# joesound212985/Deepfake-Detection-using-CLIP-Based-SigLIP-2-Vision-Transformers

Measured on AMD Instinct MI355X. Metric: images/sec (train fwd+bwd) SigLIP-2-so400m@384 bf16, higher is better.
Workload: dtype bf16; 1 GPU; so400m-patch14-384 encoder+pool-head train fwd+bwd, 384x384, per-GPU batch 128, seeded random weights; global_batch=128, parallelism=dp1

## Files before the change

### deepfake-detection-using-clip-based-siglip-2-vision-transformers_amd/csrc/encoder.hip

```cpp
#include <hip/hip_runtime.h>
#include <string.h>

#include <algorithm>
#include <new>
#include <vector>

#include "kernels.h"
#include "siglip_hip.h"

using namespace sgl;

namespace {

inline size_t align256(size_t x) { return (x + 255) & ~(size_t)255; }
inline char* at(void* base, size_t off) { return reinterpret_cast<char*>(base) + off; }
inline const char* at(const void* base, size_t off) { return reinterpret_cast<const char*>(base) + off; }
inline bool mfma16(int dt) { return dt == DT_BF16 || dt == DT_F16; }
inline int round_up(int x, int m) { return (x + m - 1) / m * m; }

struct Bump {
  size_t off = 0;
  size_t take(size_t bytes) {
    const size_t o = off;
    off += align256(bytes);
// ... 148 lines not shown

#define CK(expr)                        \
  do {                                  \
    hipError_t e_ = (expr);             \
    if (e_ != hipSuccess) {             \
      ctx->last_hip = (int)e_;          \
      return SGL_ERR_HIP;               \
    }                                   \
  } while (0)

#define RET(expr)                 \
  do {                            \
    int r_ = (expr);              \
    if (r_ != SGL_OK) return r_;  \
  } while (0)

EpiParams epi_store(void* out, int ldo) {
  EpiParams p;
  p.out = out;
  p.ldo = ldo;
  return p;
}
EpiParams epi_f32(float* out, int ldo, const float* bias = nullptr) {
  EpiParams p;
  p.out = out;
  p.ldo = ldo;
  p.bias = bias;
  return p;
}
EpiParams epi_f32_acc(float* out, int ldo, int accumulate) {
  EpiParams p;
  p.out = out;
  p.ldo = ldo;
  p.accumulate = accumulate;
  return p;
}
EpiParams epi_res_f32(float* out, const float* bias, const float* res, int ld) {
  EpiParams p;
  p.out = out;
  p.ldo = ld;
  p.bias = bias;
  p.res = res;
  p.ldr = ld;
  return p;
}
EpiParams epi_pos_f32(float* out, int ldo, const float* bias, const float* pos, int pos_rows) {
  EpiParams p;
  p.out = out;
  p.ldo = ldo;
  p.bias = bias;
  p.pos = pos;
  p.pos_rows = pos_rows;
  return p;
}
EpiParams epi_bias_gelu(void* u, void* a, int ld, const float* bias, int grad_form) {
  EpiParams p;
  p.out = u;
  p.gelu_grad_form = grad_form;
  p.ldo = ld;
  p.out2 = a;
  p.ldo2 = ld;
  p.bias = bias;
  return p;
}
EpiParams epi_bias_gelu_mx(void* out, int ldo, const float* bias) {
  EpiParams p;
  p.out = out;
  p.ldo = ldo;
  p.bias = bias;
  return p;
}
EpiParams epi_gelu_bwd(void* out, const void* aux, int ld, int grad_form, float* colsum = nullptr) {
  EpiParams p;
  p.out = out;
  p.ldo = ld;
  p.aux = aux;
  p.ldaux = ld;
  p.gelu_grad_form = grad_form;
  if (colsum) {
    p.colsum = colsum;
    p.colsum_ld = ld;
  }
  return p;
}

int tn_splits(int N1, int N2, int rows) {
  const int tiles = ((N1 + 127) / 128) * ((N2 + 127) / 128);
  return std::min({(512 + tiles - 1) / tiles, std::max(rows / 512, 1), 16});
}

struct Call {
  sgl_ctx* ctx = nullptr;
  Layout lay;
  hipStream_t s = nullptr;
  const void* shadow = nullptr;
  char* act = nullptr;
  void* ws = nullptr;
  void* sp_a = nullptr;
  void* sp_b = nullptr;

  char* wsp(size_t off) const { return at(ws, off); }
  float* wsf(size_t off) const { return reinterpret_cast<float*>(at(ws, off)); }
  float* actf(size_t off) const { return reinterpret_cast<float*>(act + off); }
  const char* sh(size_t off) const { return at(shadow, off); }
  const float* shf(size_t off) const { return reinterpret_cast<const float*>(at(shadow, off)); }
  size_t head_bytes() const { return ::head_bytes(ctx, lay.B, lay.N); }
  char* block(int l) const { return lay.rc ? wsp(lay.w_blk) : act + lay.layer_base(l); }

  EpiParams epi_qkv(void* out, const float* bias) const {
    EpiParams p;
    p.out = out;
    p.bias = bias;
    p.tokens = lay.N;
    p.heads = ctx->H;
    p.head_dim = ctx->dh;
    p.head_dim_pad = ctx->DP;
    p.batch = lay.B;
    return p;
  }

  hipError_t gemm_nt(const void* A, int lda, const void* B, int ldb, int M, int N, int K, int epi, int out_dt,
                     const EpiParams& p) const {
    if (ctx->dt == DT_BF16) return gemm_nt_bf16(A, lda, B, ldb, M, N, K, epi, out_dt, p, s);
    if (ctx->dt == DT_F16) return gemm_nt_f16(A, lda, B, ldb, M, N, K, epi, out_dt, p, s);
    if (ctx->split && M > 0 && N > 0) {
      const int Ks = round_up(K, 8);
      hipError_t e = split3_rows((const float*)A, M, K, lda, sp_a, Ks, 0, s);
      if (e != hipSuccess) return e;
      e = split3_rows((const float*)B, N, K, ldb, sp_b, Ks, 1, s);
      if (e != hipSuccess) return e;
      return gemm_nt_bf16(sp_a, 3 * Ks, sp_b, 3 * Ks, M, N, 3 * Ks, epi, out_dt, p, s);
    }
    return gemm_f32_generic((const float*)A, lda, 1, (const float*)B, ldb, 1, M, N, K, epi, out_dt, p, s);
  }

  hipError_t gemm_tn(const void* A, int lda, const void* B, int ldb, int Mred, int N1, int N2, float* out, int ldo,
                     int accumulate, bool split_slabs) const {
    const EpiParams p = epi_f32_acc(out, ldo, accumulate);
    float* slabs = split_slabs ? wsf(lay.w_splitws) : nullptr;
    const size_t slab_bytes = split_slabs ? kSplitWsBytes : 0;
    if (ctx->dt == DT_F16)
      return gemm_tn_f16(A, lda, B, ldb, Mred, N1, N2, tn_splits(N1, N2, Mred), p, s, slabs, slab_bytes);
    if (ctx->dt == DT_BF16)
      return gemm_tn_bf16(A, lda, B, ldb, Mred, N1, N2, tn_splits(N1, N2, Mred), p, s, slabs, slab_bytes);
    if (ctx->split && Mred > 0 && N1 > 0 && N2 > 0) {
      const int l1 = round_up(N1, 8), l2 = round_up(N2, 8);
      hipError_t e = split3_stack((const float*)A, Mred, N1, lda, sp_a, l1, 0, s);
      if (e != hipSuccess) return e;
      e = split3_stack((const float*)B, Mred, N2, ldb, sp_b, l2, 1, s);
      if (e != hipSuccess) return e;
      return gemm_tn_bf16(sp_a, l1, sp_b, l2, 3 * Mred, N1, N2, tn_splits(N1, N2, 3 * Mred), p, s, slabs, slab_bytes);
    }
    return gemm_f32_generic((const float*)A, 1, lda, (const float*)B, 1, ldb, N1, N2, Mred, EPI_F32, DT_F32, p, s);
  }

  int bias_grad(const void* in, int ld, int M, int N, int n_out, float* out, int accumulate) const {
    if (!out) return SGL_OK;
    CK(colsum(in, ctx->dt, ld, M, N, n_out, wsf(lay.w_cspart), out, accumulate, s));
    return SGL_OK;
  }

  int ln_backward(const void* dy, int dy_dt, const float* x, const float* stats, int rows, const float* gamma,
                  const float* dres, float* dx, void* dx_lp, float* dgamma, float* dbeta, int accumulate,
                  float* colsum_out = nullptr) const {
    const int D = ctx->D;
    const bool want = dgamma || dbeta || colsum_out;
    const int nblk = layernorm_bwd_blocks(rows);
    float* part = wsf(lay.w_lnpart);
    CK(layernorm_bwd(dy, dy_dt, D, x, stats, stats + rows, gamma, dres, dx, dx_lp, ctx->dt, want ? part : nullptr, nblk,
                     rows, D, s));
    CK(reduce_partials3(part, nblk, 3 * D, dgamma, dbeta, colsum_out, D, accumulate, accumulate, 0, s));
    return SGL_OK;
  }
};

int mx_block(const Call& c, const sgl_layer_weights& lw, const ShadowLayer& sl, char* lb, const float* x, float* xo) {
  sgl_ctx* ctx = c.ctx;
  const Layout& lay = c.lay;
  hipStream_t s = c.s;
  const int D = ctx->D, Ip = ctx->Ip, Dp = ctx->Dp, M = lay.M;
  const float eps = ctx->cfg.layer_norm_eps;
  const size_t Mz = (size_t)M;
  char* h1 = lb + lay.r_h1;
  char* q = lb + lay.r_qkv;
  char* aq = lb + lay.r_attq;
  float* xmid = reinterpret_cast<float*>(lb + lay.r_xmid);
  char* h2 = lb + lay.r_h2;
  char* ua = lb + lay.r_a;
  CK(layernorm_fwd_mx(x, lw.ln1_w, lw.ln1_b, h1, h1 + Mz * Dp, M, D, Dp, eps, s));
  CK(gemm_nt_mx(h1, h1 + Mz * Dp, c.sh(sl.wqkv), c.sh(sl.wqkv_s), M, 3 * D, Dp, EPI_QKV, c.epi_qkv(q, c.shf(sl.bqkv)),
                nullptr, s));
  CK(attn_fwd(q, q + c.head_bytes(), q + 2 * c.head_bytes(), DT_BF16, lb + lay.r_attn,
              reinterpret_cast<float*>(lb + lay.r_lse), lay.B, ctx->H, lay.N, ctx->dh, ctx->DP, 0, s));
  CK(quantize_mx(lb + lay.r_attn, DT_BF16, D, M, D, Dp, aq, aq + Mz * Dp, s));
  CK(gemm_nt_mx(aq, aq + Mz * Dp, c.sh(sl.wo), c.sh(sl.wo_s), M, D, Dp, EPI_RES_F32, epi_res_f32(xmid, lw.o_b, x, D),
                nullptr, s));
  CK(layernorm_fwd_mx(xmid, lw.ln2_w, lw.ln2_b, h2, h2 + Mz * Dp, M, D, Dp, eps, s));
  CK(gemm_nt_mx(h2, h2 + Mz * Dp, c.sh(sl.w1), c.sh(sl.w1_s), M, Ip, Dp, EPI_BIAS_GELU,
                epi_bias_gelu_mx(ua, Ip, c.shf(sl.b1)), ua + Mz * Ip, s));
  CK(gemm_nt_mx(ua, ua + Mz * Ip, c.sh(sl.w2), c.sh(sl.w2_s), M, D, Ip, EPI_RES_F32, epi_res_f32(xo, lw.fc2_b, xmid, D),
                nullptr, s));
  return SGL_OK;
}

int block_to_fc1(const Call& c, const sgl_layer_weights& lw, const ShadowLayer& sl, char* lb, const float* x, bool want_u) {
  sgl_ctx* ctx = c.ctx;
  const Layout& lay = c.lay;
  hipStream_t s = c.s;
  const int D = ctx->D, Ip = ctx->Ip, M = lay.M, dt = ctx->dt;
  const float eps = ctx->cfg.layer_norm_eps;
  float* st1 = reinterpret_cast<float*>(lb + lay.r_stats1);
  float* st2 = reinterpret_cast<float*>(lb + lay.r_stats2);
  char* q = lb + lay.r_qkv;
  float* xmid = reinterpret_cast<float*>(lb + lay.r_xmid);
  CK(layernorm_fwd(x, lw.ln1_w, lw.ln1_b, lb + lay.r_h1, dt, D, st1, st1 + M, M, D, eps, s));
  CK(c.gemm_nt(lb + lay.r_h1, D, c.sh(sl.wqkv), D, M, 3 * D, D, EPI_QKV, dt, c.epi_qkv(q, c.shf(sl.bqkv))));
  CK(attn_fwd(q, q + c.head_bytes(), q + 2 * c.head_bytes(), ctx->split ? DT_F32_MFMA : dt, lb + lay.r_attn,
              reinterpret_cast<float*>(lb + lay.r_lse), lay.B, ctx->H, lay.N, ctx->dh, ctx->DP, 0, s));
  CK(c.gemm_nt(lb + lay.r_attn, D, c.sh(sl.wo), D, M, D, D, EPI_RES_F32, DT_F32, epi_res_f32(xmid, lw.o_b, x, D)));
  CK(layernorm_fwd(xmid, lw.ln2_w, lw.ln2_b, lb + lay.r_h2, dt, D, st2, st2 + M, M, D, eps, s));
  CK(c.gemm_nt(lb + lay.r_h2, D, c.sh(sl.w1), D, M, Ip, D, EPI_BIAS_GELU, dt,
               epi_bias_gelu(want_u ? lb + lay.r_u : nullptr, lb + lay.r_a, Ip, c.shf(sl.b1), mfma16(dt))));
  return SGL_OK;
}

int embed_forward(const Call& c, const sgl_weights* w, const float* pixels, int channels_last, int H, int W, float* out) {
  sgl_ctx* ctx = c.ctx;
  const Layout& lay = c.lay;
  hipStream_t s = c.s;
  const int D = ctx->D, Kp = ctx->Kp, M = lay.M;
  char* cols = c.act + lay.a_im2col;
  if (channels_last == 2) {
    CK(hipMemcpyAsync(cols, pixels, (size_t)M * Kp * ctx->es, hipMemcpyDeviceToDevice, s));
  } else {
    CK(im2col(pixels, channels_last, cols, ctx->dt, lay.B, H, W, ctx->P, Kp, s));
  }
  const float* pos = w->pos;
  if (!(lay.gh == ctx->g0 && lay.gw == ctx->g0)) {
    float* pr = c.actf(lay.a_pos);
    CK(pos_resize(w->pos, ctx->g0, pr, lay.gh, lay.gw, D, s));
    pos = pr;
  }
  CK(c.gemm_nt(cols, Kp, c.sh(ctx->sh_wpatch), Kp, M, D, Kp, EPI_POS_F32, DT_F32,
               epi_pos_f32(out, D, w->patch_b, pos, lay.N)));
  return SGL_OK;
}

int head_forward(const Call& c, const sgl_weights* w, const float* last_hidden, float* pooled) {
  sgl_ctx* ctx = c.ctx;
  const Layout& lay = c.lay;
  hipStream_t s = c.s;
  const int D = ctx->D, Ip = ctx->Ip, M = lay.M, B = lay.B, dt = ctx->dt;
  char* act = c.act;
  char* kv = act + lay.a_kvh;
  float* qp = c.actf(lay.a_qp);
  float* h0 = c.actf(lay.a_h0);
  float* hst = c.actf(lay.a_hstats);
  CK(cast_f32(last_hidden, act + lay.a_lastlp, dt, (size_t)M * D, s));
  CK(c.gemm_nt(act + lay.a_lastlp, D, c.sh(ctx->sh_hwkv), D, M, 2 * D, D, EPI_QKV, dt, c.epi_qkv(kv, w->in_proj_b + D)));
  CK(gemm_f32_generic(w->probe, D, 1, w->in_proj_w, D, 1, 1, D, D, EPI_F32, DT_F32, epi_f32(qp, D, w->in_proj_b), s));
  CK(pool_attn_fwd(qp, kv, kv + c.head_bytes(), dt, act + lay.a_ao, c.actf(lay.a_probs), B, ctx->H, lay.N, ctx->dh,
                   ctx->DP, s));
  CK(c.gemm_nt(act + lay.a_ao, D, c.sh(ctx->sh_hwo), D, B, D, D, EPI_F32, DT_F32, epi_f32(h0, D, w->out_proj_b)));
  CK(layernorm_fwd(h0, w->head_ln_w, w->head_ln_b, act + lay.a_hl, dt, D, hst, hst + B, B, D, ctx->cfg.layer_norm_eps, s));
  CK(c.gemm_nt(act + lay.a_hl, D, c.sh(ctx->sh_hw1), D, B, Ip, D, EPI_BIAS_GELU, dt,
               epi_bias_gelu(act + lay.a_hu, act + lay.a_ha, Ip, c.shf(ctx->sh_hb1), 0)));
  CK(c.gemm_nt(act + lay.a_ha, Ip, c.sh(ctx->sh_hw2), Ip, B, D, Ip, EPI_RES_F32, DT_F32,
               epi_res_f32(pooled, w->head_fc2_b, h0, D)));
  return SGL_OK;
}

long rc_max_tokens(const sgl_ctx* c) {
  long w = c->Ip;
  if (3l * c->D > w) w = 3l * c->D;
  if ((long)c->Kp > w) w = c->Kp;
  const long row_bytes = c->split ? 3 * (long)round_up((int)w, 8) * 2 : w * (long)c->es;
  const long m = ((1l << 32) - 1) / row_bytes;
  return m < (1l << 22) - 1 ? m : (1l << 22) - 1;
}

bool shape_ok(const sgl_ctx* c, int B, int H, int W) {
  if (B <= 0 || H <= 0 || W <= 0) return false;
  if (H < c->P || W < c->P) return false;
  const long N = (long)(H / c->P) * (W / c->P);
  if ((long)B * N > (1l << 24)) return false;
  if (c->cfg.use_head && N > pool_attn_max_tokens(c->DP, 0)) return false;
  return true;
}

bool train_shape_ok(const sgl_ctx* c, int B, int H, int W) {
  if (!shape_ok(c, B, H, W)) return false;
  const long N = (long)(H / c->P) * (W / c->P);
  if (c->cfg.use_head && N > pool_attn_max_tokens(c->DP, 1)) return false;
  return !c->recompute || (long)B * N <= rc_max_tokens(c);
}

enum Pass { FORWARD, BACKWARD };
int begin_call(Call& c, Pass pass, sgl_ctx* ctx, const void* shadow, int B, int H, int W, const void* saved,
               size_t saved_bytes, void* ws, size_t ws_bytes, sgl_stream stream) {
  const bool train = pass == BACKWARD || saved != nullptr;
  if (!(train ? train_shape_ok(ctx, B, H, W) : shape_ok(ctx, B, H, W))) return SGL_ERR_BAD_SHAPE;
  if (train && ctx->mx) return SGL_ERR_UNSUPPORTED;
  c.lay = Layout(ctx, B, H, W, train);
  const Layout& lay = c.lay;
  if (pass == BACKWARD) {
    if (!saved || !ws) return SGL_ERR_NULL;
// ... 295 lines not shown
  float* slots[kMaxLayers + 1];
  for (int l = 0; l <= ctx->L; ++l) slots[l] = hidden_states + (size_t)(l % hs_slots) * hs_stride;
  return sgl_forward_slots(ctx, w, shadow, pixels, channels_last, B, H, W, interpolate_pos, slots, last_hidden,
                           pooled, saved, saved_bytes, ws, ws_bytes, first_trainable_block, stream);
}

int sgl_forward_slots(sgl_ctx* ctx, const sgl_weights* w, const void* shadow, const float* pixels, int channels_last,
                      int B, int H, int W, int interpolate_pos, float* const* hs_slots, float* last_hidden,
                      float* pooled, void* saved, size_t saved_bytes, void* ws, size_t ws_bytes,
                      int first_trainable_block, sgl_stream stream) {
  if (!ctx || !w || !shadow || !pixels || !hs_slots || !last_hidden || (ctx->L > 0 && !w->layers))
    return SGL_ERR_NULL;
  if (!shape_ok(ctx, B, H, W)) return SGL_ERR_BAD_SHAPE;
  for (int l = 0; l <= ctx->L; ++l)
    if (!hs_slots[l]) return SGL_ERR_NULL;
  const bool train = saved != nullptr;
  if (train && ctx->mx) return SGL_ERR_UNSUPPORTED;
  if (train)
    for (int l = 0; l < ctx->L; ++l)
      for (int k = l + 1; k <= ctx->L; ++k)
        if (hs_slots[l] == hs_slots[k]) return SGL_ERR_BAD_SHAPE;
  Call c;
  RET(begin_call(c, FORWARD, ctx, shadow, B, H, W, saved, saved_bytes, ws, ws_bytes, stream));
  const Layout& lay = c.lay;
  if (!(lay.gh == ctx->g0 && lay.gw == ctx->g0) && !interpolate_pos) return SGL_ERR_BAD_SHAPE;

  RET(embed_forward(c, w, pixels, channels_last, H, W, hs_slots[0]));
  for (int l = 0; l < ctx->L; ++l) {
    const sgl_layer_weights& lw = w->layers[l];
    const ShadowLayer& sl = ctx->sh_layers[l];
    char* lb = c.block(l);
    if (ctx->mx) {
      RET(mx_block(c, lw, sl, lb, hs_slots[l], hs_slots[l + 1]));
      continue;
    }
    RET(block_to_fc1(c, lw, sl, lb, hs_slots[l], train && !lay.rc && l >= first_trainable_block));
    CK(c.gemm_nt(lb + lay.r_a, ctx->Ip, c.sh(sl.w2), ctx->Ip, lay.M, ctx->D, ctx->Ip, EPI_RES_F32, DT_F32,
                 epi_res_f32(hs_slots[l + 1], lw.fc2_b, reinterpret_cast<const float*>(lb + lay.r_xmid), ctx->D)));
  }
  float* pst = c.actf(lay.a_pstats);
  CK(layernorm_fwd(hs_slots[ctx->L], w->post_ln_w, w->post_ln_b, last_hidden, DT_F32, ctx->D, pst, pst + lay.M, lay.M,
                   ctx->D, ctx->cfg.layer_norm_eps, c.s));
  if (ctx->cfg.use_head && pooled) RET(head_forward(c, w, last_hidden, pooled));
  return SGL_OK;
}

namespace {

int head_backward(const Call& c, const sgl_weights* w, const sgl_grads* g, const float* d_pooled,
                  const float* d_last_hidden, float* dlast) {
  sgl_ctx* ctx = c.ctx;
  const Layout& lay = c.lay;
  hipStream_t s = c.s;
  const int D = ctx->D, I = ctx->I, Ip = ctx->Ip, M = lay.M, B = lay.B, dt = ctx->dt;
  const int acc = g->accumulate;
  const char* act = c.act;
  const char* kv = act + lay.a_kvh;
  const float* qp = c.actf(lay.a_qp);
  void* hg = c.wsp(lay.w_hg);
  void* hdu = c.wsp(lay.w_hdu);
  void* hdh = c.wsp(lay.w_hdh);
  float* hdao = c.wsf(lay.w_hdao);
  CK(cast_f32(d_pooled, hg, dt, (size_t)B * D, s));
  CK(c.gemm_nt(hg, D, c.sh(ctx->sh_hw2_t), D, B, Ip, D, EPI_GELU_BWD, dt, epi_gelu_bwd(hdu, act + lay.a_hu, Ip, 0)));
  if (g->head_fc2_w) CK(c.gemm_tn(hg, D, act + lay.a_ha, Ip, B, D, I, g->head_fc2_w, I, acc, false));
  RET(c.bias_grad(hg, D, B, D, D, g->head_fc2_b, acc));
  CK(c.gemm_nt(hdu, Ip, c.sh(ctx->sh_hw1_t), Ip, B, D, Ip, EPI_STORE, dt, epi_store(hdh, D)));
  if (g->head_fc1_w) CK(c.gemm_tn(hdu, Ip, act + lay.a_hl, D, B, I, D, g->head_fc1_w, D, acc, false));
  RET(c.bias_grad(hdu, Ip, B, Ip, I, g->head_fc1_b, acc));
  RET(c.ln_backward(hdh, dt, c.actf(lay.a_h0), c.actf(lay.a_hstats), B, w->head_ln_w, d_pooled, c.wsf(lay.w_hdh0), hg,
                    g->head_ln_w, g->head_ln_b, acc));
  CK(c.gemm_nt(hg, D, c.sh(ctx->sh_hwo_t), D, B, D, D, EPI_F32, DT_F32, epi_f32(hdao, D)));
  if (g->out_proj_w) CK(c.gemm_tn(hg, D, act + lay.a_ao, D, B, D, D, g->out_proj_w, D, acc, false));
  RET(c.bias_grad(hg, D, B, D, D, g->out_proj_b, acc));
  void* dkv = c.wsp(lay.w_dqkv);
  float* dqpart = c.wsf(lay.w_hdqpart);
  float* dqp = c.wsf(lay.w_hdqp);
  CK(pool_attn_bwd(qp, kv, kv + c.head_bytes(), dt, c.actf(lay.a_probs), hdao, dkv, dqpart, B, ctx->H, lay.N, ctx->dh,
                   ctx->DP, s));
  if (g->probe || g->in_proj_w || g->in_proj_b) {
    CK(batch_sum(dqpart, B, (size_t)D, dqp, 0, s));
    if (g->in_proj_w)
      CK(gemm_f32_generic(dqp, 1, 1, w->probe, 1, 1, D, D, 1, EPI_F32, DT_F32, epi_f32_acc(g->in_proj_w, D, acc), s));
    if (g->in_proj_b) CK(batch_sum(dqp, 1, (size_t)D, g->in_proj_b, acc, s));
    if (g->probe)
      CK(gemm_f32_generic(dqp, D, 1, w->in_proj_w, 1, D, 1, D, D, EPI_F32, DT_F32, epi_f32_acc(g->probe, D, acc), s));
  }
  if (d_last_hidden) CK(copy_f32(d_last_hidden, dlast, (size_t)M * D, s));
  CK(c.gemm_nt(dkv, 2 * D, c.sh(ctx->sh_hwkv_t), 2 * D, M, D, 2 * D, EPI_F32, DT_F32,
               epi_f32_acc(dlast, D, d_last_hidden ? 1 : 0)));
  if (g->in_proj_w)
    CK(c.gemm_tn(dkv, 2 * D, act + lay.a_lastlp, D, M, 2 * D, D, g->in_proj_w + (size_t)D * D, D, acc, true));
  if (g->in_proj_b) RET(c.bias_grad(dkv, 2 * D, M, 2 * D, 2 * D, g->in_proj_b + D, acc));
  return SGL_OK;
}

int zero_dead_grads(const Call& c, const sgl_grads* g, bool no_head_grad, bool no_post_ln_grad) {
  sgl_ctx* ctx = c.ctx;
  hipStream_t s = c.s;
  if (g->accumulate) return SGL_OK;
  auto zero = [&](float* p, size_t n) { return p ? hipMemsetAsync(p, 0, n * 4, s) : hipSuccess; };
  const size_t Dz = (size_t)ctx->D, Iz = (size_t)ctx->I;
  if (ctx->cfg.use_head && no_head_grad) {
    CK(zero(g->probe, Dz));
    CK(zero(g->in_proj_w, 3 * Dz * Dz));
    CK(zero(g->in_proj_b, 3 * Dz));
    CK(zero(g->out_proj_w, Dz * Dz));
    CK(zero(g->out_proj_b, Dz));
    CK(zero(g->head_ln_w, Dz));
    CK(zero(g->head_ln_b, Dz));
    CK(zero(g->head_fc1_w, Iz * Dz));
    CK(zero(g->head_fc1_b, Iz));
    CK(zero(g->head_fc2_w, Dz * Iz));
    CK(zero(g->head_fc2_b, Dz));
  }
  if (no_post_ln_grad) {
    CK(zero(g->post_ln_w, Dz));
    CK(zero(g->post_ln_b, Dz));
  }
  return SGL_OK;
}

int mlp_backward(const Call& c, const sgl_layer_weights& lw, const sgl_layer_grads& lg, const ShadowLayer& sl,
                 const char* lb, int acc) {
  sgl_ctx* ctx = c.ctx;
  const Layout& lay = c.lay;
  hipStream_t s = c.s;
  const int D = ctx->D, I = ctx->I, Ip = ctx->Ip, M = lay.M, dt = ctx->dt;
  float* dx = c.wsf(lay.w_dx);
  void* gbuf = c.wsp(lay.w_g);
  void* du = c.wsp(lay.w_du);
  void* dhb = c.wsp(lay.w_dh);
  float* gsum = c.wsf(lay.w_gsum);
  float* csum = c.wsf(lay.w_csum);
  const bool fuse_cs = mfma16(dt) && lg.fc1_b;
  if (fuse_cs) CK(hipMemsetAsync(csum, 0, (size_t)((M + 127) / 128) * Ip * 4, s));
  CK(c.gemm_nt(gbuf, D, c.sh(sl.w2_t), D, M, Ip, D, EPI_GELU_BWD, dt,
               epi_gelu_bwd(du, lb + lay.r_u, Ip, mfma16(dt), fuse_cs ? csum : nullptr)));
  if (lg.fc2_w) CK(c.gemm_tn(gbuf, D, lb + lay.r_a, Ip, M, D, I, lg.fc2_w, I, acc, true));
  if (lg.fc2_b) CK(batch_sum(gsum, 1, (size_t)D, lg.fc2_b, acc, s));
  CK(c.gemm_nt(du, Ip, c.sh(sl.w1_t), Ip, M, D, Ip, EPI_STORE, dt, epi_store(dhb, D)));
  if (lg.fc1_w) CK(c.gemm_tn(du, Ip, lb + lay.r_h2, D, M, I, D, lg.fc1_w, D, acc, true));
  if (fuse_cs)
    CK(reduce_partials(csum, (M + 127) / 128, Ip, lg.fc1_b, I, acc, s));
  else
    RET(c.bias_grad(du, Ip, M, Ip, I, lg.fc1_b, acc));
  RET(c.ln_backward(dhb, dt, reinterpret_cast<const float*>(lb + lay.r_xmid),
                    reinterpret_cast<const float*>(lb + lay.r_stats2), M, lw.ln2_w, dx, dx, gbuf, lg.ln2_w, lg.ln2_b, acc,
                    (lg.o_b || lg.v_b) ? gsum : nullptr));
  if (lg.o_b) CK(batch_sum(gsum, 1, (size_t)D, lg.o_b, acc, s));
  return SGL_OK;
}

int attn_backward(const Call& c, const sgl_layer_weights& lw, const sgl_layer_grads& lg, const ShadowLayer& sl,
                  const char* lb, int acc) {
  sgl_ctx* ctx = c.ctx;
  const Layout& lay = c.lay;
  hipStream_t s = c.s;
  const int D = ctx->D, M = lay.M, dt = ctx->dt;
  void* gbuf = c.wsp(lay.w_g);
  void* dattn = c.wsp(lay.w_dh);
  void* dqkv = c.wsp(lay.w_dqkv);
  float* gsum = c.wsf(lay.w_gsum);
  const char* q = lb + lay.r_qkv;
  CK(c.gemm_nt(gbuf, D, c.sh(sl.wo_t), D, M, D, D, EPI_STORE, dt, epi_store(dattn, D)));
  if (lg.o_w) CK(c.gemm_tn(gbuf, D, lb + lay.r_attn, D, M, D, D, lg.o_w, D, acc, true));
  CK(attn_bwd(q, q + c.head_bytes(), q + 2 * c.head_bytes(), lb + lay.r_attn, dattn,
              reinterpret_cast<const float*>(lb + lay.r_lse), ctx->split ? DT_F32_MFMA : dt, dqkv, c.wsf(lay.w_delta),
              nullptr, lay.B, ctx->H, lay.N, ctx->dh, ctx->DP, 0, s));
  float* gw[3] = {lg.q_w, lg.k_w, lg.v_w};
  float* gb[3] = {lg.q_b, lg.k_b, lg.v_b};
  const bool w_adj = gw[0] && gw[1] == gw[0] + (size_t)D * D && gw[2] == gw[1] + (size_t)D * D;
  if (w_adj) CK(c.gemm_tn(dqkv, 3 * D, lb + lay.r_h1, D, M, 3 * D, D, gw[0], D, acc, true));
  for (int j = 0; j < 3; ++j) {
    const char* aj = reinterpret_cast<const char*>(dqkv) + (size_t)j * D * ctx->es;
    if (!w_adj && gw[j]) CK(c.gemm_tn(aj, 3 * D, lb + lay.r_h1, D, M, D, D, gw[j], D, acc, true));
  }
  if (gb[0]) RET(c.bias_grad(dqkv, 3 * D, M, D, D, gb[0], acc));
  if (gb[1] && !acc) CK(hipMemsetAsync(gb[1], 0, (size_t)D * 4, s));
  if (gb[2]) CK(vecmat_f32(gsum, lw.o_w, D, D, c.wsf(lay.w_cspart), gb[2], acc, s));
  return SGL_OK;
}

int ln1_backward(const Call& c, const sgl_layer_weights& lw, const sgl_layer_grads& lg, const ShadowLayer& sl,
                 const char* lb, const float* x_in, int acc) {
  sgl_ctx* ctx = c.ctx;
  const Layout& lay = c.lay;
  const int D = ctx->D, M = lay.M, dt = ctx->dt;
  float* dx = c.wsf(lay.w_dx);
  void* dh1 = c.wsp(lay.w_dh);
  CK(c.gemm_nt(c.wsp(lay.w_dqkv), 3 * D, c.sh(sl.wqkv_t), 3 * D, M, D, 3 * D, EPI_STORE, dt, epi_store(dh1, D)));
  RET(c.ln_backward(dh1, dt, x_in, reinterpret_cast<const float*>(lb + lay.r_stats1), M, lw.ln1_w, dx, dx,
                    c.wsp(lay.w_g), lg.ln1_w, lg.ln1_b, acc, c.wsf(lay.w_gsum)));
  return SGL_OK;
}

}

int sgl_backward_begin(sgl_ctx* ctx, const sgl_weights* w, const void* shadow, const sgl_grads* g, int B, int H, int W,
                       const float* hidden_states, const float* d_last_hidden, const float* d_pooled,
                       const float* d_tap_last, const void* saved, size_t saved_bytes, void* ws, size_t ws_bytes,
                       sgl_stream stream) {
  if (!ctx || !hidden_states) return SGL_ERR_NULL;
  if (!train_shape_ok(ctx, B, H, W)) return SGL_ERR_BAD_SHAPE;
  const size_t stride = (size_t)B * (H / ctx->P) * (W / ctx->P) * ctx->D;
  return sgl_backward_begin_p(ctx, w, shadow, g, B, H, W, hidden_states + (size_t)ctx->L * stride, d_last_hidden, d_pooled,
                              d_tap_last, saved, saved_bytes, ws, ws_bytes, stream);
}

int sgl_backward_begin_p(sgl_ctx* ctx, const sgl_weights* w, const void* shadow, const sgl_grads* g, int B, int H, int W,
                         const float* hs_last, const float* d_last_hidden, const float* d_pooled,
                         const float* d_tap_last, const void* saved, size_t saved_bytes, void* ws, size_t ws_bytes,
                         sgl_stream stream) {
  if (!ctx || !w || !shadow || !g || !hs_last) return SGL_ERR_NULL;
  Call c;
  RET(begin_call(c, BACKWARD, ctx, shadow, B, H, W, saved, saved_bytes, ws, ws_bytes, stream));
  const Layout& lay = c.lay;
  hipStream_t s = c.s;
  const int D = ctx->D, M = lay.M;
  float* dx = c.wsf(lay.w_dx);
  void* gbuf = c.wsp(lay.w_g);
  float* gsum = c.wsf(lay.w_gsum);
  const float* dlast = d_last_hidden;
  if (ctx->cfg.use_head && d_pooled) {
    float* dlast_buf = c.wsf(lay.w_dlast);
    RET(head_backward(c, w, g, d_pooled, d_last_hidden, dlast_buf));
    dlast = dlast_buf;
  }
  RET(zero_dead_grads(c, g, !d_pooled, !dlast));
  if (dlast) {
    RET(c.ln_backward(dlast, DT_F32, hs_last, c.actf(lay.a_pstats), M, w->post_ln_w, d_tap_last, dx, gbuf, g->post_ln_w,
                      g->post_ln_b, g->accumulate, gsum));
  } else if (d_tap_last) {
    CK(copy_f32(d_tap_last, dx, (size_t)M * D, s));
    CK(cast_f32(d_tap_last, gbuf, ctx->dt, (size_t)M * D, s));
    CK(colsum(gbuf, ctx->dt, D, M, D, D, c.wsf(lay.w_cspart), gsum, 0, s));
  } else {
    CK(hipMemsetAsync(dx, 0, (size_t)M * D * 4, s));
    CK(hipMemsetAsync(gbuf, 0, (size_t)M * D * ctx->es, s));
    CK(hipMemsetAsync(gsum, 0, (size_t)D * 4, s));
  }
  return SGL_OK;
}

int sgl_backward_layer(sgl_ctx* ctx, const sgl_weights* w, const void* shadow, const sgl_grads* g, int layer, int B,
                       int H, int W, const float* hidden_states, const float* d_tap, int need_dx, const void* saved,
                       size_t saved_bytes, void* ws, size_t ws_bytes, sgl_stream stream) {
  if (!ctx || !hidden_states) return SGL_ERR_NULL;
  if (layer < 0 || layer >= ctx->L || !train_shape_ok(ctx, B, H, W)) return SGL_ERR_BAD_SHAPE;
  const size_t stride = (size_t)B * (H / ctx->P) * (W / ctx->P) * ctx->D;
  return sgl_backward_layer_p(ctx, w, shadow, g, layer, B, H, W, hidden_states + (size_t)layer * stride, d_tap, need_dx,
                              saved, saved_bytes, ws, ws_bytes, stream);
}

int sgl_backward_layer_p(sgl_ctx* ctx, const sgl_weights* w, const void* shadow, const sgl_grads* g, int layer, int B,
                         int H, int W, const float* hs_in, const float* d_tap, int need_dx, const void* saved,
                         size_t saved_bytes, void* ws, size_t ws_bytes, sgl_stream stream) {
  if (!ctx || !w || !shadow || !g || !hs_in || !g->layers || !w->layers) return SGL_ERR_NULL;
  if (layer < 0 || layer >= ctx->L) return SGL_ERR_BAD_SHAPE;
  Call c;
  RET(begin_call(c, BACKWARD, ctx, shadow, B, H, W, saved, saved_bytes, ws, ws_bytes, stream));
  const int acc = g->accumulate;
  const sgl_layer_weights& lw = w->layers[layer];
  const sgl_layer_grads& lg = g->layers[layer];
  const ShadowLayer& sl = ctx->sh_layers[layer];
  char* lb = c.block(layer);
  if (c.lay.rc) RET(block_to_fc1(c, lw, sl, lb, hs_in, true));
  RET(mlp_backward(c, lw, lg, sl, lb, acc));
  RET(attn_backward(c, lw, lg, sl, lb, acc));
  float* dx = c.wsf(c.lay.w_dx);
  if (d_tap) CK(add_f32(dx, d_tap, dx, (size_t)c.lay.M * ctx->D, c.s));
  if (need_dx || lg.ln1_w || lg.ln1_b) RET(ln1_backward(c, lw, lg, sl, lb, hs_in, acc));
  return SGL_OK;
}

namespace {

int embed_param_backward(const Call& c, const sgl_grads* g) {
  sgl_ctx* ctx = c.ctx;
  const Layout& lay = c.lay;
  hipStream_t s = c.s;
  const int D = ctx->D, M = lay.M, N = lay.N;
  const int acc = g->accumulate;
  float* dx = c.wsf(lay.w_dx);
  void* gbuf = c.wsp(lay.w_g);
  if (g->patch_w)
    CK(c.gemm_tn(gbuf, D, c.act + lay.a_im2col, ctx->Kp, M, D, ctx->K0, g->patch_w, ctx->K0, acc, true));
  if (g->patch_b) CK(batch_sum(c.wsf(lay.w_gsum), 1, (size_t)D, g->patch_b, acc, s));
  if (g->pos) {
    if (lay.gh == ctx->g0 && lay.gw == ctx->g0) {
      CK(batch_sum(dx, lay.B, (size_t)N * D, g->pos, acc, s));
    } else {
      float* dpos = c.wsf(lay.w_dlast);
      CK(batch_sum(dx, lay.B, (size_t)N * D, dpos, 0, s));
      if (!acc) CK(hipMemsetAsync(g->pos, 0, (size_t)ctx->g0 * ctx->g0 * D * 4, s));
      CK(pos_resize_bwd(dpos, lay.gh, lay.gw, g->pos, ctx->g0, D, s));
    }
  }
  return SGL_OK;
}

struct PxLayout {
  size_t dcols = 0, wpt = 0, total = 0;
  PxLayout(const sgl_ctx* c, int M) {
    Bump b;
    dcols = b.take((size_t)M * c->Kp * 4);
    wpt = b.take((size_t)c->Kp * c->D * c->es);
    total = b.off;
  }
};

}

int sgl_backward_embed(sgl_ctx* ctx, const sgl_weights* w, const sgl_grads* g, int B, int H, int W, int interpolate_pos,
                       const void* saved, size_t saved_bytes, void* ws, size_t ws_bytes, sgl_stream stream) {
  if (!ctx || !w || !g) return SGL_ERR_NULL;
  Call c;
  RET(begin_call(c, BACKWARD, ctx, nullptr, B, H, W, saved, saved_bytes, ws, ws_bytes, stream));
  (void)interpolate_pos;
  return embed_param_backward(c, g);
}

int sgl_query_input_grad_bytes(const sgl_ctx* ctx, int B, int H, int W, size_t* scratch_bytes) {
  if (!ctx || !scratch_bytes) return SGL_ERR_NULL;
  if (!train_shape_ok(ctx, B, H, W)) return SGL_ERR_BAD_SHAPE;
  if (ctx->mx) return SGL_ERR_UNSUPPORTED;
  *scratch_bytes = PxLayout(ctx, B * (H / ctx->P) * (W / ctx->P)).total;
  return SGL_OK;
}

int sgl_backward_embed_px(sgl_ctx* ctx, const sgl_weights* w, const sgl_grads* g, int B, int H, int W,
                          int interpolate_pos, float* d_pixels, int channels_last, void* px_scratch,
                          size_t px_scratch_bytes, const void* saved, size_t saved_bytes, void* ws, size_t ws_bytes,
                          sgl_stream stream) {
  if (!ctx || !w || !g || !w->patch_w) return SGL_ERR_NULL;
  if (!d_pixels || !px_scratch) return SGL_ERR_NULL;
  if (channels_last != 0 && channels_last != 1) return SGL_ERR_UNSUPPORTED;
  Call c;
  RET(begin_call(c, BACKWARD, ctx, nullptr, B, H, W, saved, saved_bytes, ws, ws_bytes, stream));
  const Layout& lay = c.lay;
  const PxLayout px(ctx, lay.M);
  if (px_scratch_bytes < px.total) return SGL_ERR_WORKSPACE;
  (void)interpolate_pos;
  RET(embed_param_backward(c, g));
  const int D = ctx->D, Kp = ctx->Kp;
  float* dcols = reinterpret_cast<float*>(at(px_scratch, px.dcols));
  void* wpt = at(px_scratch, px.wpt);
  CastJob job;
  cast_job_add(job, w->patch_w, D, ctx->K0, ctx->K0, nullptr, D, Kp, Kp, wpt, D);
  CK(cast_job_run(job, ctx->dt, c.s));
  CK(c.gemm_nt(c.wsp(lay.w_g), D, wpt, D, lay.M, Kp, D, EPI_F32, DT_F32, epi_f32(dcols, Kp)));
  CK(col2im(dcols, lay.B, H, W, ctx->P, Kp, d_pixels, channels_last, c.s));
  return SGL_OK;
}

int sgl_backward(sgl_ctx* ctx, const sgl_weights* w, const void* shadow, const sgl_grads* g, int B, int H, int W,
                 int interpolate_pos, const float* hidden_states, const float* const* d_taps,
                 const float* d_last_hidden, const float* d_pooled, int first_trainable_block, int train_embeddings,
                 const void* saved, size_t saved_bytes, void* ws, size_t ws_bytes, sgl_stream stream) {
  if (!ctx) return SGL_ERR_NULL;
  const int L = ctx->L;
  int stop = train_embeddings ? 0 : first_trainable_block;
  if (stop < 0) stop = 0;
  if (stop < L && w && g && (!w->layers || !g->layers)) return SGL_ERR_NULL;
  RET(sgl_backward_begin(ctx, w, shadow, g, B, H, W, hidden_states, d_last_hidden, d_pooled,
                         d_taps ? d_taps[L] : nullptr, saved, saved_bytes, ws, ws_bytes, stream));
  for (int l = L - 1; l >= stop; --l) {
    const int need_dx = (l > stop) || train_embeddings;
    RET(sgl_backward_layer(ctx, w, shadow, g, l, B, H, W, hidden_states, d_taps ? d_taps[l] : nullptr, need_dx, saved,
                           saved_bytes, ws, ws_bytes, stream));
  }
  if (train_embeddings)
    RET(sgl_backward_embed(ctx, w, g, B, H, W, interpolate_pos, saved, saved_bytes, ws, ws_bytes, stream));
  return SGL_OK;
}

#define CKV(expr)                                   \
  do {                                              \
    hipError_t e_ = (expr);                         \
    if (e_ == hipErrorInvalidValue) return SGL_ERR_UNSUPPORTED; \
    if (e_ != hipSuccess) return SGL_ERR_HIP;       \
  } while (0)

int sgl_op_layernorm_fwd(const float* x, const float* gamma, const float* beta, void* y, int y_dtype, float* mean,
                         float* rstd, int M, int D, float eps, sgl_stream stream) {
  CKV(layernorm_fwd(x, gamma, beta, y, y_dtype, D, mean, rstd, M, D, eps, (hipStream_t)stream));
  return SGL_OK;
}

int sgl_op_quantize_mxfp8(const void* x, int x_dtype, int ldx, int M, int K, int Kp, void* q, void* scales,
                          sgl_stream stream) {
  if (!x || !q || !scales) return SGL_ERR_NULL;
  CKV(quantize_mx(x, x_dtype, ldx, M, K, Kp, q, scales, (hipStream_t)stream));
  return SGL_OK;
}

int sgl_op_layernorm_fwd_mx(const float* x, const float* gamma, const float* beta, void* q, void* scales, int M, int D,
                            int Kp, float eps, sgl_stream stream) {
  if (!x || !gamma || !beta || !q || !scales) return SGL_ERR_NULL;
  CKV(layernorm_fwd_mx(x, gamma, beta, q, scales, M, D, Kp, eps, (hipStream_t)stream));
  return SGL_OK;
}

int sgl_op_gemm_nt_mx(const void* A, const void* As, const void* B, const void* Bs, int M, int N, int Kp, int epi,
                      void* out, int ldo, void* out_scales, const float* bias, const float* res, int ldr, int tokens,
                      int heads, int head_dim, int head_dim_pad, int batch, sgl_stream stream) {
  if (!A || !As || !B || !Bs || !out || !bias) return SGL_ERR_NULL;
  EpiParams p;
  p.out = out; p.ldo = ldo; p.bias = bias; p.res = res; p.ldr = ldr;
  p.tokens = tokens > 0 ? tokens : 1; p.heads = heads > 0 ? heads : 1; p.head_dim = head_dim > 0 ? head_dim : 8;
  p.head_dim_pad = head_dim_pad > 0 ? head_dim_pad : 8; p.batch = batch > 0 ? batch : 1;
  CKV(gemm_nt_mx(A, As, B, Bs, M, N, Kp, epi, p, out_scales, (hipStream_t)stream));
  return SGL_OK;
}

int sgl_op_layernorm_bwd(const void* dy, int dy_dtype, const float* x, const float* mean, const float* rstd,
                         const float* gamma, const float* dres, float* dx, void* dx_lp, int lp_dtype, float* dgamma,
                         float* dbeta, float* scratch, size_t scratch_bytes, int M, int D, sgl_stream stream) {
  const int nblk = layernorm_bwd_blocks(M);
  if (scratch_bytes < (size_t)nblk * 3 * D * 4) return SGL_ERR_WORKSPACE;
  hipStream_t s = (hipStream_t)stream;
  CKV(layernorm_bwd(dy, dy_dtype, D, x, mean, rstd, gamma, dres, dx, dx_lp, lp_dtype, scratch, nblk, M, D, s));
  if (dgamma) CKV(reduce_partials(scratch, nblk, 3 * D, dgamma, D, 0, s));
  if (dbeta) CKV(reduce_partials(scratch + D, nblk, 3 * D, dbeta, D, 0, s));
  return SGL_OK;
}

int sgl_op_gemm_nt(int dtype, const void* A, int lda, const void* B, int ldb, int M, int N, int K, int epi, void* out,
                   int ldo, void* out2, int ldo2, const float* bias, const float* res, int ldr, const void* aux,
                   int ldaux, const float* pos, int pos_rows, int tokens, int heads, int head_dim, int head_dim_pad,
                   int batch, sgl_stream stream) {
  EpiParams p;
  p.out = out; p.ldo = ldo; p.out2 = out2; p.ldo2 = ldo2; p.bias = bias; p.res = res; p.ldr = ldr;
  p.aux = aux; p.ldaux = ldaux; p.pos = pos; p.pos_rows = pos_rows > 0 ? pos_rows : 1;
  p.tokens = tokens > 0 ? tokens : 1; p.heads = heads > 0 ? heads : 1; p.head_dim = head_dim > 0 ? head_dim : 8;
  p.head_dim_pad = head_dim_pad > 0 ? head_dim_pad : 8; p.batch = batch > 0 ? batch : 1;
  const bool f32_out = (epi == EPI_RES_F32 || epi == EPI_POS_F32 || epi == EPI_F32);
  const int out_dt = f32_out ? DT_F32 : dtype;
  if (dtype == DT_BF16)
    CKV(gemm_nt_bf16(A, lda, B, ldb, M, N, K, epi, out_dt, p, (hipStream_t)stream));
  else if (dtype == DT_F16)
    CKV(gemm_nt_f16(A, lda, B, ldb, M, N, K, epi, out_dt, p, (hipStream_t)stream));
  else
    CKV(gemm_f32_generic((const float*)A, lda, 1, (const float*)B, ldb, 1, M, N, K, epi, out_dt, p,
                         (hipStream_t)stream));
  return SGL_OK;
}

int sgl_op_gemm_tn(int dtype, const void* A, int lda, const void* B, int ldb, int Mred, int N1, int N2, int splits,
                   float* out, int ldo, int accumulate, sgl_stream stream) {
  return sgl_op_gemm_tn_ws(dtype, A, lda, B, ldb, Mred, N1, N2, splits, out, ldo, accumulate, nullptr, 0, stream);
}

int sgl_op_gemm_tn_ws(int dtype, const void* A, int lda, const void* B, int ldb, int Mred, int N1, int N2, int splits,
                      float* out, int ldo, int accumulate, float* scratch, size_t scratch_bytes, sgl_stream stream) {
  EpiParams p;
  p.out = out; p.ldo = ldo; p.accumulate = accumulate;
  if (dtype == DT_BF16)
    CKV(gemm_tn_bf16(A, lda, B, ldb, Mred, N1, N2, splits, p, (hipStream_t)stream, scratch, scratch_bytes));
  else if (dtype == DT_F16)
    CKV(gemm_tn_f16(A, lda, B, ldb, Mred, N1, N2, splits, p, (hipStream_t)stream, scratch, scratch_bytes));
  else
    CKV(gemm_f32_generic((const float*)A, 1, lda, (const float*)B, 1, ldb, N1, N2, Mred, EPI_F32, DT_F32, p,
                         (hipStream_t)stream));
  return SGL_OK;
}

int sgl_op_attn_fwd(int dtype, const void* q, const void* k, const void* v, void* out, float* lse, int B, int H, int N,
                    int head_dim, int head_dim_pad, int ld_qkv, sgl_stream stream) {
  CKV(attn_fwd(q, k, v, dtype, out, lse, B, H, N, head_dim, head_dim_pad, ld_qkv, (hipStream_t)stream));
  return SGL_OK;
}

int sgl_op_attn_bwd(int dtype, const void* q, const void* k, const void* v, const void* out, const void* dout,
                    const float* lse, void* dqkv, float* delta_scratch, int B, int H, int N, int head_dim,
                    int head_dim_pad, int ld_qkv, sgl_stream stream) {
  CKV(attn_bwd(q, k, v, out, dout, lse, dtype, dqkv, delta_scratch, nullptr, B, H, N, head_dim, head_dim_pad, ld_qkv,
               (hipStream_t)stream));
  return SGL_OK;
}

int sgl_op_colsum(int dtype, const void* in, int ld, int M, int N, float* out, int accumulate, float* scratch,
                  size_t scratch_bytes, sgl_stream stream) {
  if (scratch_bytes < (size_t)colsum_chunks(M) * N * 4) return SGL_ERR_WORKSPACE;
  CKV(colsum(in, dtype, ld, M, N, N, scratch, out, accumulate, (hipStream_t)stream));
  return SGL_OK;
}

int sgl_op_im2col(const float* pixels, int channels_last, void* out, int out_dtype, int B, int H, int W, int P, int Kp,
                  sgl_stream stream) {
  CKV(im2col(pixels, channels_last, out, out_dtype, B, H, W, P, Kp, (hipStream_t)stream));
  return SGL_OK;
}

int sgl_op_col2im(const float* d_cols, int B, int H, int W, int P, int Kp, float* d_pixels, int channels_last,
                  sgl_stream stream) {
  if (!d_cols || !d_pixels) return SGL_ERR_NULL;
  CKV(col2im(d_cols, B, H, W, P, Kp, d_pixels, channels_last, (hipStream_t)stream));
  return SGL_OK;
}

int sgl_op_pos_resize(const float* table, int native_grid, float* out, int gh, int gw, int D, sgl_stream stream) {
  CKV(pos_resize(table, native_grid, out, gh, gw, D, (hipStream_t)stream));
  return SGL_OK;
}

static bool lo_dtype_ok(int dt) { return dt == DT_F32 || dt == DT_BF16 || dt == DT_F16; }
static bool aligned16(const void* p) { return (((uintptr_t)p) & 15) == 0; }

int sgl_op_pool_attn_fwd(int dtype, const float* q, const void* K, const void* V, void* out, float* probs, int B, int H,
                         int N, int head_dim, int head_dim_pad, sgl_stream stream) {
  if (!q || !K || !V || !out || !probs) return SGL_ERR_NULL;
  if (B <= 0 || H <= 0 || N <= 0 || head_dim <= 0 || head_dim % 8 || head_dim_pad % 8 || head_dim > head_dim_pad)
    return SGL_ERR_BAD_SHAPE;
  if (!lo_dtype_ok(dtype) || !aligned16(K) || !aligned16(V)) return SGL_ERR_UNSUPPORTED;
  CKV(pool_attn_fwd(q, K, V, dtype, out, probs, B, H, N, head_dim, head_dim_pad, (hipStream_t)stream));
  return SGL_OK;
}

int sgl_op_pool_attn_bwd(int dtype, const float* q, const void* K, const void* V, const float* probs, const float* dout,
                         void* dkv, float* dq_partial, int B, int H, int N, int head_dim, int head_dim_pad,
                         sgl_stream stream) {
  if (!q || !K || !V || !probs || !dout || !dkv || !dq_partial) return SGL_ERR_NULL;
  if (B <= 0 || H <= 0 || N <= 0 || head_dim <= 0 || head_dim % 8 || head_dim_pad % 8 || head_dim > head_dim_pad)
    return SGL_ERR_BAD_SHAPE;
  if (!lo_dtype_ok(dtype) || !aligned16(K) || !aligned16(V) || !aligned16(dkv)) return SGL_ERR_UNSUPPORTED;
  CKV(pool_attn_bwd(q, K, V, dtype, probs, dout, dkv, dq_partial, B, H, N, head_dim, head_dim_pad, (hipStream_t)stream));
  return SGL_OK;
}

int sgl_op_pos_resize_bwd(const float* dout, int gh, int gw, float* dtable, int native_grid, int D, sgl_stream stream) {
  if (!dout || !dtable) return SGL_ERR_NULL;
  if (gh <= 0 || gw <= 0 || native_grid <= 0 || D <= 0) return SGL_ERR_BAD_SHAPE;
  CKV(pos_resize_bwd(dout, gh, gw, dtable, native_grid, D, (hipStream_t)stream));
  return SGL_OK;
}

int sgl_op_cast_pad(const float* src, int R, int C, int lds, void* dst, int dst_dtype, int Rp, int Cp, int ldd,
                    sgl_stream stream) {
  if (!src || !dst) return SGL_ERR_NULL;
  if (R < 0 || C < 0 || Rp < R || Cp < C || lds < C || ldd < Cp) return SGL_ERR_BAD_SHAPE;
  if (!lo_dtype_ok(dst_dtype)) return SGL_ERR_UNSUPPORTED;
  CKV(cast_pad(src, R, C, lds, dst, dst_dtype, Rp, Cp, ldd, (hipStream_t)stream));
  return SGL_OK;
}

int sgl_op_cast_job(const sgl_cast_mat* mats, int nmat, const sgl_cast_vec* vecs, int nvec, int dst_dtype,
                    sgl_stream stream) {
  if ((nmat > 0 && !mats) || (nvec > 0 && !vecs)) return SGL_ERR_NULL;
  if (nmat < 0 || nmat > 6 || nvec < 0 || nvec > 4) return SGL_ERR_BAD_SHAPE;
  for (int k = 0; k < nmat; ++k)
    if (!mats[k].src || (!mats[k].dst && !mats[k].dst_t)) return SGL_ERR_NULL;
  for (int k = 0; k < nvec; ++k)
    if (!vecs[k].src || !vecs[k].dst) return SGL_ERR_NULL;
  for (int k = 0; k < nmat; ++k) {
    const sgl_cast_mat& m = mats[k];
    if (m.R <= 0 || m.C <= 0 || m.Rp < m.R || m.Cp < m.C || m.lds < m.C || (m.dst && m.ldd < m.Cp) ||
        (m.dst_t && m.ldt < m.Rp))
      return SGL_ERR_BAD_SHAPE;
  }
  for (int k = 0; k < nvec; ++k)
    if (vecs[k].n < 0 || vecs[k].np < vecs[k].n) return SGL_ERR_BAD_SHAPE;
  if (!lo_dtype_ok(dst_dtype)) return SGL_ERR_UNSUPPORTED;
  CastJob job;
  for (int k = 0; k < nmat; ++k) {
    const sgl_cast_mat& m = mats[k];
    cast_job_add(job, m.src, m.R, m.C, m.lds, m.dst, m.Rp, m.Cp, m.ldd, m.dst_t, m.ldt);
  }
  for (int k = 0; k < nvec; ++k) cast_job_add_vec(job, vecs[k].src, vecs[k].n, vecs[k].dst, vecs[k].np);
  CKV(cast_job_run(job, dst_dtype, (hipStream_t)stream));
  return SGL_OK;
}

int sgl_op_split3(const float* src, int R, int C, int ld, void* dst, int Cs, int b_side, int stacked, sgl_stream stream) {
  if (!src || !dst) return SGL_ERR_NULL;
  if (R <= 0 || C <= 0 || ld < C || Cs != round_up(C, 8)) return SGL_ERR_BAD_SHAPE;
  if (!aligned16(dst)) return SGL_ERR_UNSUPPORTED;
  if (stacked)
    CKV(split3_stack(src, R, C, ld, dst, Cs, b_side ? 1 : 0, (hipStream_t)stream));
  else
    CKV(split3_rows(src, R, C, ld, dst, Cs, b_side ? 1 : 0, (hipStream_t)stream));
  return SGL_OK;
}

int sgl_op_batch_sum(const float* in, int B, size_t n, float* out, int accumulate, sgl_stream stream) {
  if (!in || !out) return SGL_ERR_NULL;
  if (B <= 0 || n >= ((size_t)1 << 31) * 256) return SGL_ERR_BAD_SHAPE;
  CKV(batch_sum(in, B, n, out, accumulate, (hipStream_t)stream));
  return SGL_OK;
}

int sgl_op_vecmat(const float* v, const float* W, int rows, int cols, float* scratch, size_t scratch_bytes, float* out,
                  int accumulate, sgl_stream stream) {
  if (!v || !W || !scratch || !out) return SGL_ERR_NULL;
  if (rows <= 0 || cols <= 0) return SGL_ERR_BAD_SHAPE;
  if (scratch_bytes < (size_t)16 * cols * 4) return SGL_ERR_WORKSPACE;
  CKV(vecmat_f32(v, W, rows, cols, scratch, out, accumulate, (hipStream_t)stream));
  return SGL_OK;
}

int sgl_op_reduce_partials(const float* partial, int nblk, int stride, float* out, int n, int accumulate,
                           sgl_stream stream) {
  if (!partial || !out) return SGL_ERR_NULL;
  if (nblk <= 0 || n <= 0 || stride < n) return SGL_ERR_BAD_SHAPE;
  CKV(reduce_partials(partial, nblk, stride, out, n, accumulate, (hipStream_t)stream));
  return SGL_OK;
}

int sgl_op_reduce_partials3(const float* partial, int nblk, int stride, float* out0, float* out1, float* out2, int n,
                            int accumulate0, int accumulate1, int accumulate2, sgl_stream stream) {
  if (!partial) return SGL_ERR_NULL;
  if (nblk <= 0 || n <= 0 || stride < 3 * (long)n) return SGL_ERR_BAD_SHAPE;
  CKV(reduce_partials3(partial, nblk, stride, out0, out1, out2, n, accumulate0, accumulate1, accumulate2,
                       (hipStream_t)stream));
  return SGL_OK;
}

int sgl_op_reduce_splits(const float* ws, int splits, size_t stride, int N1, int N2, float* out, int ldo, int accumulate,
                         sgl_stream stream) {
  if (!ws || !out) return SGL_ERR_NULL;
// ... 21 lines not shown
```

### deepfake-detection-using-clip-based-siglip-2-vision-transformers_amd/csrc/gemm_bf16.hip

```cpp
#include <stdlib.h>

#include "common.hip.h"
#include "epilogue.hip.h"
#include "kernels.h"

namespace sgl {

constexpr int G_BM = 128, G_BN = 128, G_BK = 64;
constexpr int G_STAGE = (G_BM + G_BN) * G_BK * 2;
constexpr int G_CT_LD = 132;
constexpr int G_LDS = (2 * G_STAGE > G_BM * G_CT_LD * 4) ? 2 * G_STAGE : G_BM * G_CT_LD * 4;

__device__ __forceinline__ u32x4 ldg128(__amdgpu_buffer_rsrc_t r, uint32_t voff) {
  return __builtin_amdgcn_raw_buffer_load_b128(r, voff, 0, 0);
}

template <int EPI, typename TOut>
__device__ __forceinline__ void store_tile(char* smem, f32x4 (&acc)[4][4], int wr, int wc, int lane, int t, int m0,
                                           int n0, int M, int N, const EpiParams& p) {
  float* ct = reinterpret_cast<float*>(smem);
  __syncthreads();
  const int g = lane >> 4, c16 = lane & 15;
#pragma unroll
  for (int i = 0; i < 4; ++i)
// ... 193 lines not shown
    }
  };

  load_tile(0);
  store_stage(0);
  __syncthreads();
  for (int kt = 0; kt < nk; ++kt) {
    const int cur = kt & 1;
    if (kt + 1 < nk) load_tile(kt + 1);
    const char* base = smem + cur * G_STAGE;
#pragma unroll
    for (int s = 0; s < 2; ++s) {
      const char* ba = base + s * 32 * 256 + frow;
      const char* bb = ba + OPB;
      lo_x8<TIn> af[4], bfr[4];
#pragma unroll
      for (int i = 0; i < 4; ++i) {
        const lo_x4<TIn> alo = lds_read_tr16<TIn>(ba + fa_col[i]);
        const lo_x4<TIn> ahi = lds_read_tr16<TIn>(ba + 4 * 256 + fa_col[i]);
        const lo_x4<TIn> blo = lds_read_tr16<TIn>(bb + fb_col[i]);
        const lo_x4<TIn> bhi = lds_read_tr16<TIn>(bb + 4 * 256 + fb_col[i]);
        af[i] = __builtin_shufflevector(alo, ahi, 0, 1, 2, 3, 4, 5, 6, 7);
        bfr[i] = __builtin_shufflevector(blo, bhi, 0, 1, 2, 3, 4, 5, 6, 7);
      }
#pragma unroll
      for (int i = 0; i < 4; ++i)
#pragma unroll
        for (int j = 0; j < 4; ++j)
          acc[i][j] = mfma_16x16x32(af[i], bfr[j], acc[i][j]);
    }
    if (kt + 1 < nk) store_stage(cur ^ 1);
    __syncthreads();
  }
  EpiParams pq = p;
  if (p.split_stride) pq.out = reinterpret_cast<float*>(p.out) + (size_t)blockIdx.y * p.split_stride;
  store_tile<EPI_F32, float>(smem, acc, wr, wc, lane, t, n1_0, n2_0, N1, N2, pq);
}

template <int EPI, typename TOut, typename TIn>
static hipError_t launch_nt(const TIn* A, int lda, const TIn* B, int ldb, int M, int N, int K, const EpiParams& p,
                            hipStream_t s) {
  const hipError_t e = set_max_dynamic_lds_once<&gemm_nt_kernel<EPI, TOut, TIn>>(G_LDS);
  if (e != hipSuccess) return e;
  const int tiles = ((M + G_BM - 1) / G_BM) * ((N + G_BN - 1) / G_BN);
  hipLaunchKernelGGL((gemm_nt_kernel<EPI, TOut, TIn>), dim3(tiles), dim3(256), G_LDS, s, A, lda, B, ldb, M, N, K, p);
  return hipGetLastError();
}

template <typename TIn>
static hipError_t gemm_nt_mfma(const void* A, int lda, const void* B, int ldb, int M, int N, int K, int epi,
                               int out_dtype, const EpiParams& p, hipStream_t s) {
  if (M == 0 || N == 0) return hipSuccess;
  if ((lda % 8) || (ldb % 8) || (K % 8) || K <= 0) return hipErrorInvalidValue;
  if (epi != EPI_F32 && (N % 8)) return hipErrorInvalidValue;
  if ((size_t)M * lda * 2 >= (1ull << 32) || (size_t)N * ldb * 2 >= (1ull << 32)) return hipErrorInvalidValue;
  if (M >= 2048 && N >= 256) {
    static const int tile_env = getenv("SGL_NT_TILE") ? atoi(getenv("SGL_NT_TILE")) : 0;
    const bool can384 = epi == EPI_STORE || epi == EPI_RES_F32;
    const bool pays384 = N % 192 == 0 && N % 256 != 0 && (epi == EPI_STORE || K >= 2048);
    const bool want384 = tile_env == 384 || (tile_env != 256 && pays384);
    if (can384 && want384) return gemm_nt384<TIn>(A, lda, B, ldb, M, N, K, epi, out_dtype, p, s);
    return gemm_nt256<TIn>(A, lda, B, ldb, M, N, K, epi, out_dtype, p, s);
  }
  return dispatch_epilogue<TIn>(epi, out_dtype, [&](auto tag) {
    using T = decltype(tag);
    return launch_nt<T::epi, typename T::out, TIn>((const TIn*)A, lda, (const TIn*)B, ldb, M, N, K, p, s);
  });
}
hipError_t gemm_nt_bf16(const void* A, int lda, const void* B, int ldb, int M, int N, int K, int epi, int out_dtype,
                        const EpiParams& p, hipStream_t s) {
  return gemm_nt_mfma<bf16>(A, lda, B, ldb, M, N, K, epi, out_dtype, p, s);
}
hipError_t gemm_nt_f16(const void* A, int lda, const void* B, int ldb, int M, int N, int K, int epi, int out_dtype,
                       const EpiParams& p, hipStream_t s) {
  return gemm_nt_mfma<f16>(A, lda, B, ldb, M, N, K, epi, out_dtype, p, s);
}

static bool tn_slabs_ok(const EpiParams& p, int N2, const float* split_ws) {
  return p.alpha == 1.0f && !p.bias && (N2 % 4 == 0) && (p.ldo % 4 == 0) &&
         ((((uintptr_t)p.out) | ((uintptr_t)split_ws)) & 15) == 0;
}

template <typename Launch>
static hipError_t tn_split_k(int Mred, int N1, int N2, int splits, const EpiParams& p_, hipStream_t s, float* split_ws,
                             size_t split_ws_bytes, Launch&& launch) {
  EpiParams p = p_;
  float* out = reinterpret_cast<float*>(p.out);
  if (splits < 1) splits = 1;
  int m_per = (Mred + splits - 1) / splits;
  m_per = ((m_per + G_BK - 1) / G_BK) * G_BK;
  splits = (Mred + m_per - 1) / m_per;
  if (splits > 1) {
    const size_t slab = (size_t)N1 * N2;
    if (split_ws && (size_t)splits * slab * sizeof(float) <= split_ws_bytes && tn_slabs_ok(p, N2, split_ws)) {
      EpiParams q = p;
      q.out = split_ws;
      q.ldo = N2;
      q.accumulate = 0;
      q.atomic = 0;
      q.split_stride = slab;
      const hipError_t e = launch(m_per, splits, q);
      if (e != hipSuccess) return e;
      return reduce_splits(split_ws, splits, slab, N1, N2, out, p.ldo, p.accumulate, s);
    }
    if (!p.accumulate) {
      const hipError_t e = hipMemset2DAsync(out, (size_t)p.ldo * sizeof(float), 0, (size_t)N2 * sizeof(float), N1, s);
      if (e != hipSuccess) return e;
    }
    p.atomic = 1;
  }
  return launch(m_per, splits, p);
}

template <typename TIn>
static hipError_t gemm_tn_mfma(const void* A, int lda, const void* B, int ldb, int Mred, int N1, int N2, int splits,
                               const EpiParams& p, hipStream_t s, float* split_ws, size_t split_ws_bytes) {
  if (N1 == 0 || N2 == 0) return hipSuccess;
  if ((lda % 8) || (ldb % 8)) return hipErrorInvalidValue;
  if ((size_t)Mred * lda * 2 >= (1ull << 32) || (size_t)Mred * ldb * 2 >= (1ull << 32)) return hipErrorInvalidValue;
  if (Mred <= 0) {
    if (!p.accumulate)
      return hipMemset2DAsync(p.out, (size_t)p.ldo * sizeof(float), 0, (size_t)N2 * sizeof(float), N1, s);
    return hipSuccess;
  }
  if (N1 >= 512 && N2 >= 512 && Mred >= 2048) {
    static const int tile_env = getenv("SGL_TN_TILE") ? atoi(getenv("SGL_TN_TILE")) : 0;
    const int tile = (tile_env == 256 || tile_env == 384) ? tile_env : 0;
    const bool slabs_ok = split_ws && tn_slabs_ok(p, N2, split_ws);
    TnPlan plan = tn_plan(Mred, N1, N2, slabs_ok ? split_ws_bytes : 0, tile);
    if (plan.splits == 1) plan = tn_plan(Mred, N1, N2, ~(size_t)0, tile);
    return tn_split_k(Mred, N1, N2, plan.splits, p, s, split_ws, split_ws_bytes, [&](int m_per, int nsplit, const EpiParams& q) {
      if (plan.tile == 384) return gemm_tn384<TIn>(A, lda, B, ldb, Mred, N1, N2, m_per, nsplit, q, s);
      return gemm_tn256<TIn>(A, lda, B, ldb, Mred, N1, N2, m_per, nsplit, q, s);
    });
  }
  return tn_split_k(Mred, N1, N2, splits, p, s, split_ws, split_ws_bytes, [&](int m_per, int nsplit, const EpiParams& q) {
    const hipError_t e = set_max_dynamic_lds_once<&gemm_tn_kernel<TIn>>(G_LDS);
    if (e != hipSuccess) return e;
    const int tiles = ((N1 + G_BM - 1) / G_BM) * ((N2 + G_BN - 1) / G_BN);
    hipLaunchKernelGGL(gemm_tn_kernel<TIn>, dim3(tiles, nsplit), dim3(256), G_LDS, s, (const TIn*)A, lda, (const TIn*)B,
                       ldb, Mred, N1, N2, m_per, q);
    return hipGetLastError();
  });
}
hipError_t gemm_tn_bf16(const void* A, int lda, const void* B, int ldb, int Mred, int N1, int N2, int splits,
                        const EpiParams& p, hipStream_t s, float* split_ws, size_t split_ws_bytes) {
  return gemm_tn_mfma<bf16>(A, lda, B, ldb, Mred, N1, N2, splits, p, s, split_ws, split_ws_bytes);
}
hipError_t gemm_tn_f16(const void* A, int lda, const void* B, int ldb, int Mred, int N1, int N2, int splits,
                       const EpiParams& p, hipStream_t s, float* split_ws, size_t split_ws_bytes) {
  return gemm_tn_mfma<f16>(A, lda, B, ldb, Mred, N1, N2, splits, p, s, split_ws, split_ws_bytes);
}

}
```

### deepfake-detection-using-clip-based-siglip-2-vision-transformers_amd/csrc/gemm_bf16_v2.hip

```cpp
#include <stdlib.h>
#ifdef SGL_TIMELINE
#include <stdio.h>
#include <string.h>
#endif

#include "common.hip.h"
#include "epilogue.hip.h"
#include "kernels.h"

namespace sgl {

constexpr int T_BK = 64;

template <int BM_, int BN_, int MI_, int MJ_>
struct NtTileShape {
  static constexpr int BM = BM_, BN = BN_, MI = MI_, MJ = MJ_;
  static constexpr int WM = 16 * MI, WN = 16 * MJ;
  static constexpr int NWR = BM / WM, NWC = BN / WN;
  static constexpr int OPA = BM * T_BK * 2;
  static constexpr int STAGE = (BM + BN) * T_BK * 2;
  static constexpr int LDS = 2 * STAGE;
  static constexpr int PA = BM / 128, PB = BN / 64, NI = 2 * PA + PB;
  static constexpr int CT_LD = BN + 4;
  static_assert(NWR * WM == BM && NWC * WN == BN && NWR * NWC == 8, "8 waves = 512 threads cover the tile");
  static_assert(MI % 2 == 0 && BM % 128 == 0 && BN % 64 == 0 && 64 % NWR == 0 && (64 / NWR) % 16 == 0, "halves, pieces, passes");
  static_assert(LDS <= 160 * 1024 && 64 * CT_LD * 4 <= LDS, "two stages, and the epilogue image, in 160 KiB of LDS");
};

struct NtTile256 : NtTileShape<256, 256, 8, 4> {
  static __device__ __forceinline__ int wr(int w) { return (w >> 1) & 1; }
  static __device__ __forceinline__ int wc(int w) { return (w & 1) + 2 * (w >> 2); }
  static __device__ __forceinline__ int b_row(int w, int q) {
    const int ul = 16 * w + 8 * (q & 1);
    return (ul >> 5) * 64 + (ul & 31) + 32 * (q >> 1);
  }
  static constexpr bool takes(int epi) { return true; }
};

struct NtTile384 : NtTileShape<384, 192, 6, 6> {
  static __device__ __forceinline__ int wr(int w) { return w & 3; }
  static __device__ __forceinline__ int wc(int w) { return w >> 2; }
  static __device__ __forceinline__ int b_row(int w, int q) { return 8 * (3 * w + q); }
  static constexpr bool takes(int epi) { return epi == EPI_STORE || epi == EPI_RES_F32 || epi == EPI_F32; }
};

constexpr int gcd_of(int a, int b) { return b == 0 ? a : gcd_of(b, a % b); }

template <typename G, int EPI, typename TOut>
__device__ __forceinline__ void store_tile_pp(char* smem, f32x4 (&acc)[G::MI][G::MJ], int wr, int wc, int lane, int t,
                                              int m0, int n0, int M, int N, const EpiParams& p) {
  static_assert(G::takes(EPI), "this tile geometry is not dispatched with this epilogue");
  float* ct = reinterpret_cast<float*>(smem);
  const int g = lane >> 4, c16 = lane & 15;
  constexpr int NV = (sizeof(TOut) == 4) ? 4 : 8;
  constexpr int CT_LD = G::CT_LD;
  constexpr int CPR = G::BN / NV;
  constexpr int WR_ROWS = 64 / G::NWR;
  constexpr int BLK = WR_ROWS / 16;
  constexpr int NPASS = G::BM / 64;
  constexpr int QN = (64 * CPR) / 512;
  constexpr int P = CPR / gcd_of(CPR, 512);
  static_assert(NPASS * BLK == G::MI && (64 * CPR) % 512 == 0 && (512 * P) % CPR == 0, "staging image and chunk walk");
  auto grow_of = [&](int pass, int row) { return m0 + (row / WR_ROWS) * G::WM + pass * WR_ROWS + row % WR_ROWS; };
  constexpr bool HAS_BIAS = (EPI == EPI_BIAS_GELU || EPI == EPI_RES_F32 || EPI == EPI_QKV);
  int tcol[P], gcol[P];
  bool col_ok[P];
  float bias[P][NV];
  size_t qkv_c0[P];
  int qkv_pad[P];
#pragma unroll
  for (int h = 0; h < P; ++h) {
    tcol[h] = ((t + 512 * h) % CPR) * NV;
    gcol[h] = n0 + tcol[h];
    col_ok[h] = gcol[h] < N;
#pragma unroll
    for (int j = 0; j < NV; ++j) bias[h][j] = 0.f;
    if constexpr (HAS_BIAS) {
      if (col_ok[h]) Vec<float, NV>::ld(p.bias + gcol[h], bias[h]);
    }
    qkv_c0[h] = 0;
    qkv_pad[h] = 0;
    if constexpr (EPI == EPI_QKV) {
      const int dm = p.heads * p.head_dim;
      const int which = gcol[h] / dm;
      const int hc = gcol[h] - which * dm;
      const int hd = hc / p.head_dim;
      const int d = hc - hd * p.head_dim;
      qkv_c0[h] = ((size_t)which * p.batch * p.heads + hd) * (size_t)p.tokens * p.head_dim_pad + d;
      qkv_pad[h] = (d + NV == p.head_dim) ? (p.head_dim_pad - p.head_dim) / NV : 0;
    }
  }
  float csum[NV];
#pragma unroll
  for (int j = 0; j < NV; ++j) csum[j] = 0.f;
  using PreT = u32x4;
  constexpr bool HAS_PRE = (EPI == EPI_RES_F32 || EPI == EPI_GELU_BWD);
  PreT pre[2][QN];
  auto load_pre = [&](int pass, PreT (&dst)[QN]) {
    if constexpr (HAS_PRE) {
#pragma unroll
      for (int q = 0; q < QN; ++q) {
        const int h = q % P;
        const int grow = grow_of(pass, (t + 512 * q) / CPR);
        const void* src = (EPI == EPI_RES_F32)
                              ? (const void*)(p.res + (size_t)grow * p.ldr + gcol[h])
                              : (const void*)(reinterpret_cast<const TOut*>(p.aux) + (size_t)grow * p.ldaux + gcol[h]);
        dst[q] = (grow < M && col_ok[h]) ? *reinterpret_cast<const PreT*>(src) : PreT{0u, 0u, 0u, 0u};
      }
    }
  };
  load_pre(0, pre[0]);
#pragma unroll
  for (int pass = 0; pass < NPASS; ++pass) {
    if (pass + 1 < NPASS) load_pre(pass + 1, pre[(pass + 1) & 1]);
    lds_barrier();
#pragma unroll
    for (int i2 = 0; i2 < BLK; ++i2)
#pragma unroll
      for (int j = 0; j < G::MJ; ++j)
#pragma unroll
        for (int r = 0; r < 4; ++r)
          ct[(wr * WR_ROWS + i2 * 16 + g * 4 + r) * CT_LD + wc * G::WN + j * 16 + c16] = acc[BLK * pass + i2][j][r];
    lds_barrier();
    if constexpr (EPI == EPI_F32) {
      if (p.atomic) {
        float* outp = reinterpret_cast<float*>(p.out);
        const int w = t >> 6;
#pragma unroll 2
        for (int rr = 0; rr < 8; ++rr) {
          const int row = w + rr * 8;
          const int grow = grow_of(pass, row);
          if (grow >= M) continue;
#pragma unroll
          for (int h = 0; h < G::BN / 64; ++h) {
            const int col = lane + 64 * h;
            if (n0 + col < N) atomicAdd(outp + (size_t)grow * p.ldo + n0 + col, ct[row * CT_LD + col] * p.alpha);
          }
        }
        continue;
      }
    }
#pragma unroll
    for (int q = 0; q < QN; ++q) {
      const int h = q % P;
      const int row = (t + 512 * q) / CPR;
      const int grow = grow_of(pass, row);
      if (grow < M && col_ok[h]) {
        float v[NV];
        Vec<float, NV>::ld(ct + row * CT_LD + tcol[h], v);
        if constexpr (EPI == EPI_RES_F32) {
          const f32x4 r = __builtin_bit_cast(f32x4, pre[pass & 1][q]);
          float rf[NV];
#pragma unroll
          for (int j = 0; j < NV; ++j) rf[j] = r[j];
          epi_res_f32<NV>(v, bias[h], rf, reinterpret_cast<float*>(p.out) + (size_t)grow * p.ldo + gcol[h]);
        } else if constexpr (EPI == EPI_BIAS_GELU) {
          epi_bias_gelu<TOut, NV>(p, v, bias[h], reinterpret_cast<TOut*>(p.out) + (size_t)grow * p.ldo + gcol[h],
                                  reinterpret_cast<TOut*>(p.out2) + (size_t)grow * p.ldo2 + gcol[h]);
        } else if constexpr (EPI == EPI_QKV) {
          int b, n;
          qkv_split_row(grow, p.tokens, b, n);
// ... 63 lines not shown
               (uint32_t)__builtin_amdgcn_readfirstlane((int)d[2]), (uint32_t)__builtin_amdgcn_readfirstlane((int)d[3])};
}
template <int NI>
__device__ __forceinline__ void pp_end_read() {
  asm volatile("s_waitcnt vmcnt(%0) lgkmcnt(0)" :: "n"(NI) : "memory");
  __builtin_amdgcn_sched_barrier(0);
  __builtin_amdgcn_s_barrier();
  __builtin_amdgcn_sched_barrier(0);
}
#define SGL_PP_END_MFMA()                 \
  do {                                    \
    __builtin_amdgcn_sched_barrier(0);    \
    __builtin_amdgcn_s_barrier();         \
    __builtin_amdgcn_sched_barrier(0);    \
  } while (0)

#ifdef SGL_TIMELINE
__device__ unsigned long long g_nt6_tl[4];
__device__ unsigned long long g_tn6_tl[12];
#define SGL_TL_STAMP(v) const unsigned long long v = __builtin_readcyclecounter()
#else
#define SGL_TL_STAMP(v)
#endif

template <typename G, int EPI, typename TOut, typename TIn>
__global__ __launch_bounds__(512, 2) void gemm_nt6_kernel(const TIn* __restrict__ A, int lda,
                                                          const TIn* __restrict__ B, int ldb, int M, int N, int K,
                                                          int tiles_m, int tiles_n, int band_h, EpiParams p) {
  extern __shared__ __attribute__((aligned(16))) char smem[];
  SGL_TL_STAMP(tl0);
  const int ntiles = tiles_m * tiles_n;
  int tile_m, tile_n;
  if (band_h < 0) {
    if (!tile_of_local(blockIdx.x & 7, blockIdx.x >> 3, tiles_m, tiles_n, -band_h, tile_m, tile_n)) return;
  } else {
    const int unit = unit_of_block(blockIdx.x, (ntiles + 7) >> 3);
    if (unit >= ntiles) return;
    tile_of_unit(unit, tiles_m, tiles_n, tile_m, tile_n, band_h);
  }
  constexpr int MI = G::MI, MJ = G::MJ, HI = MI / 2, PA = G::PA, PB = G::PB, NI = G::NI;
  const int t = threadIdx.x, lane = t & 63;
  const int w = __builtin_amdgcn_readfirstlane(t >> 6);
  const int wr = G::wr(w), wc = G::wc(w), grp = w >> 2;
  const int m0 = tile_m * G::BM, n0 = tile_n * G::BN;
  const int rows_a = (M - m0 < G::BM) ? M - m0 : G::BM;
  const int rows_b = (N - n0 < G::BN) ? N - n0 : G::BN;
  const u32x4 da = pp_desc(A + (size_t)m0 * lda, (uint32_t)(((size_t)(rows_a - 1) * lda + K) * 2));
  const u32x4 db = pp_desc(B + (size_t)n0 * ldb, (uint32_t)(((size_t)(rows_b - 1) * ldb + K) * 2));
  const uint32_t lds0 = (uint32_t)(size_t)((SGL_LDS char*)smem);

  enum { U_A0 = 0, U_B = 1, U_A1 = 2 };
  constexpr int PMAX = PA > PB ? PA : PB;
  const int drow = lane >> 3, dchunk = (lane & 7) ^ drow;
  uint32_t voff[3][PMAX], ldst[3][PMAX];
#pragma unroll
  for (int u = 0; u < 3; ++u)
#pragma unroll
    for (int q = 0; q < (u == U_B ? PB : PA); ++q) {
      const bool isA = u != U_B;
      constexpr int ppw = G::WM / 16;
      const int piece = PA * w + q;
      const int r0 = isA ? G::WM * (piece / ppw) + 8 * (piece % ppw) + (u == U_A1 ? G::WM / 2 : 0) : G::b_row(w, q);
      const int row = r0 + drow;
      voff[u][q] = (row < (isA ? rows_a : rows_b)) ? (uint32_t)(row * (isA ? lda : ldb) + dchunk * 8) * 2u : SGL_OOB;
      ldst[u][q] = lds0 + (isA ? 0 : G::OPA) + (uint32_t)r0 * 128u;
    }
  const int nk = (K + T_BK - 1) / T_BK;
  auto issue = [&](int u, int kt) {
    const int k0 = kt * T_BK;
    const bool kok = (kt < nk) && (k0 + dchunk * 8 < K);
    const uint32_t sb = (uint32_t)((kt & 1) * G::STAGE);
#pragma unroll
    for (int q = 0; q < (u == U_B ? PB : PA); ++q)
      pp_dma16(u == U_B ? db : da, ldst[u][q] + sb, (kok && voff[u][q] != SGL_OOB) ? voff[u][q] + (uint32_t)k0 * 2u : SGL_OOB);
  };

  const int frow = lane & 15, fg = lane >> 4, fsw = frow & 7;
  const uint32_t fa_base = (uint32_t)((wr * G::WM + frow) * 128);
  const uint32_t fb_base = (uint32_t)(G::OPA + (wc * G::WN + frow) * 128);
  const uint32_t c0 = (uint32_t)(((0 + fg) ^ fsw) << 4), c1 = (uint32_t)(((4 + fg) ^ fsw) << 4);
  const bool active = (n0 + wc * G::WN < N) && (m0 + wr * G::WM < M);

  f32x4 acc[MI][MJ];
#pragma unroll
  for (int i = 0; i < MI; ++i)
#pragma unroll
    for (int j = 0; j < MJ; ++j) acc[i][j] = f32x4{0.f, 0.f, 0.f, 0.f};

  issue(U_A0, 0); issue(U_B, 0); issue(U_A1, 0);
  issue(U_A0, 1); issue(U_B, 1);
  pp_end_read<NI>();
  if (grp == 1) SGL_PP_END_MFMA();

  lo_x8<TIn> fa[2 * HI], fb[2 * MJ];
  auto mfma_slot = [&](int i0) {
    if (active) {
      __builtin_amdgcn_s_setprio(1);
#pragma unroll
      for (int h = 0; h < 2; ++h)
#pragma unroll
        for (int i = 0; i < HI; ++i)
#pragma unroll
          for (int j = 0; j < MJ; ++j)
            acc[i0 + i][j] = mfma_16x16x32(fa[HI * h + i], fb[MJ * h + j], acc[i0 + i][j]);
      __builtin_amdgcn_s_setprio(0);
    }
    SGL_PP_END_MFMA();
  };
  for (int kt = 0; kt < nk; ++kt) {
    const char* base = smem + (kt & 1) * G::STAGE;
    const char* pa = base + fa_base;
    const char* pb = base + fb_base;
    if (active) {
#pragma unroll
      for (int f = 0; f < 2 * MJ; ++f) fb[f] = *reinterpret_cast<const lo_x8<TIn>*>(pb + (f % MJ) * 2048 + ((f / MJ) ? c1 : c0));
#pragma unroll
      for (int f = 0; f < 2 * HI; ++f) fa[f] = *reinterpret_cast<const lo_x8<TIn>*>(pa + (f % HI) * 2048 + ((f / HI) ? c1 : c0));
    }
    issue(U_A1, kt + 1);
    pp_end_read<NI>();
    mfma_slot(0);
    if (active) {
#pragma unroll
      for (int f = 0; f < 2 * HI; ++f) fa[f] = *reinterpret_cast<const lo_x8<TIn>*>(pa + (HI + f % HI) * 2048 + ((f / HI) ? c1 : c0));
    }
    issue(U_A0, kt + 2); issue(U_B, kt + 2);
    pp_end_read<NI>();
    mfma_slot(HI);
  }
  if (grp == 0) SGL_PP_END_MFMA();
  asm volatile("s_waitcnt vmcnt(0)" ::: "memory");
#ifdef SGL_TIMELINE
  if (p.atomic == 77) return;
#endif
  SGL_TL_STAMP(tl1);
  store_tile_pp<G, EPI, TOut>(smem, acc, wr, wc, lane, t, m0, n0, M, N, p);
#ifdef SGL_TIMELINE
  SGL_TL_STAMP(tl2);
  if (t == 0) {
    atomicAdd(&g_nt6_tl[0], tl1 - tl0);
    atomicAdd(&g_nt6_tl[1], tl2 - tl1);
    atomicAdd(&g_nt6_tl[2], 1ull);
  }
#endif
}

template <int ROWB>
__device__ __forceinline__ int tn_swz(int m) {
  static_assert(ROWB % 128 == 0, "the patterns are closed inside 256 / 128 bytes of a row");
  if constexpr (ROWB % 256 == 0) return 2 * (m & 3) + 8 * ((m >> 3) & 1);
  else return 2 * ((m >> 1) & 1) + 4 * ((m >> 3) & 1);
}

template <typename G, typename TIn>
__global__ __launch_bounds__(512, 2) void gemm_tn6_kernel(const TIn* __restrict__ A, int lda,
                                                          const TIn* __restrict__ B, int ldb, int Mred, int N1, int N2,
                                                          int m_per_split, int nsplits, int tiles_1, int tiles_2,
                                                          EpiParams p) {
  extern __shared__ __attribute__((aligned(16))) char smem[];
  constexpr int MI = G::MI, MJ = G::MJ;
  constexpr int RA = 2 * G::BM, RB = 2 * G::BN;
  constexpr int HA = G::BM / 16, HB = G::BN / 16;
  constexpr int PA = HA / 8, PB = HB / 8;
  constexpr bool BX = (HB % 8) != 0;
  constexpr int NI = 2 * PA + 2 * PB + (BX ? 1 : 0);
  static_assert(HA % 8 == 0 && (HB % 8 == 0 || HB % 8 == 4), "pieces of a k-half over 8 waves (+ one wave group)");
  const int ntiles = tiles_1 * tiles_2;
  const int nunits = ntiles * nsplits;
  const int unit = unit_of_block(blockIdx.x, (nunits + 7) >> 3);
  if (unit >= nunits) return;
  const int split = unit / ntiles, trem = unit - split * ntiles;
  const int tile1 = trem / tiles_2, tile2 = trem - tile1 * tiles_2;
  const int t = threadIdx.x, lane = t & 63;
  const int w = __builtin_amdgcn_readfirstlane(t >> 6);
  const int wr = G::wr(w), wc = G::wc(w), grp = w >> 2;
  const int n1_0 = tile1 * G::BM, n2_0 = tile2 * G::BN;
  const int m_begin = split * m_per_split;
  const int m_end = (m_begin + m_per_split < Mred) ? m_begin + m_per_split : Mred;
  const int rows = m_end - m_begin;
  const u32x4 da = pp_desc_sgpr(pp_desc(A + (size_t)m_begin * lda, (uint32_t)((size_t)rows * lda * 2)));
  const u32x4 db = pp_desc_sgpr(pp_desc(B + (size_t)m_begin * ldb, (uint32_t)((size_t)rows * ldb * 2)));
  const uint32_t lds0 = (uint32_t)(size_t)((SGL_LDS char*)smem);

  uint32_t voffA[2][PA], ldsA[2][PA], voffB[2][PB + 1], ldsB[2][PB + 1];
#pragma unroll
  for (int h = 0; h < 2; ++h) {
#pragma unroll
    for (int q = 0; q < PA; ++q) {
      const int piece = PA * w + q, pos = 1024 * piece + 16 * lane;
      const int row = 32 * h + pos / RA, chunk = ((pos % RA) >> 4) ^ tn_swz<RA>(row);
      const int col = n1_0 + chunk * 8;
      voffA[h][q] = (col < N1) ? (uint32_t)(row * lda + col) * 2u : SGL_OOB;
      ldsA[h][q] = lds0 + (uint32_t)(h * 32 * RA + 1024 * piece);
    }
#pragma unroll
    for (int q = 0; q < PB + 1; ++q) {
      const int piece = (q < PB) ? PB * w + q : 8 * PB + (w & 3), pos = 1024 * piece + 16 * lane;
      const int row = 32 * h + pos / RB, chunk = ((pos % RB) >> 4) ^ tn_swz<RB>(row);
      const int col = n2_0 + chunk * 8;
      voffB[h][q] = (col < N2) ? (uint32_t)(row * ldb + col) * 2u : SGL_OOB;
      ldsB[h][q] = lds0 + (uint32_t)(G::OPA + h * 32 * RB + 1024 * piece);
    }
  }
  auto issue = [&](int h, int kt) {
    const uint32_t r0 = (uint32_t)kt * T_BK;
    const uint32_t sb = (uint32_t)((kt & 1) * G::STAGE);
    const uint32_t adva = r0 * (uint32_t)lda * 2u, advb = r0 * (uint32_t)ldb * 2u;
#pragma unroll
    for (int q = 0; q < PA; ++q) pp_dma16(da, ldsA[h][q] + sb, voffA[h][q] == SGL_OOB ? SGL_OOB : voffA[h][q] + adva);
#pragma unroll
    for (int q = 0; q < PB; ++q) pp_dma16(db, ldsB[h][q] + sb, voffB[h][q] == SGL_OOB ? SGL_OOB : voffB[h][q] + advb);
    if constexpr (BX) {
      if (grp == h) pp_dma16(db, ldsB[h][PB] + sb, voffB[h][PB] == SGL_OOB ? SGL_OOB : voffB[h][PB] + advb);
    }
  };

  const int fg = lane >> 4, fq = (lane >> 2) & 3, fp = lane & 3;
  const int fm = 8 * fg + fq;
  uint32_t fa_off[MI], fb_off[MJ];
#pragma unroll
  for (int i = 0; i < MI; ++i)
    fa_off[i] = (uint32_t)(fm * RA) + ((uint32_t)(wr * G::WM * 2 + i * 32 + 8 * fp) ^ (uint32_t)(16 * tn_swz<RA>(fm)));
#pragma unroll
  for (int j = 0; j < MJ; ++j)
    fb_off[j] = (uint32_t)(G::OPA + fm * RB) + ((uint32_t)(wc * G::WN * 2 + j * 32 + 8 * fp) ^ (uint32_t)(16 * tn_swz<RB>(fm)));
  const bool active = (n2_0 + wc * G::WN < N2) && (n1_0 + wr * G::WM < N1);

  f32x4 acc[MI][MJ];
#pragma unroll
  for (int i = 0; i < MI; ++i)
#pragma unroll
    for (int j = 0; j < MJ; ++j) acc[i][j] = f32x4{0.f, 0.f, 0.f, 0.f};

  const int nk = (rows + T_BK - 1) / T_BK;
  issue(0, 0); issue(1, 0);
  issue(0, 1);
  pp_end_read<NI>();
  if (grp == 1) SGL_PP_END_MFMA();

#define SGL_TR6(ptr, rowb) \
  __builtin_shufflevector(lds_read_tr16<TIn>(ptr), lds_read_tr16<TIn>((ptr) + 4 * (rowb)), 0, 1, 2, 3, 4, 5, 6, 7)
  lo_x8<TIn> fa[MI], fb[MJ];
#ifdef SGL_TIMELINE
  unsigned long long tlp[5] = {0, 0, 0, 0, 0};
#define SGL_TLP(i) do { const unsigned long long n_ = __builtin_readcyclecounter(); tlp[i] += n_ - tl_last; tl_last = n_; } while (0)
  unsigned long long tl_last = __builtin_readcyclecounter();
#else
#define SGL_TLP(i)
#endif
  for (int kt = 0; kt < nk; ++kt) {
    const char* base = smem + (kt & 1) * G::STAGE;
#pragma unroll
    for (int h = 0; h < 2; ++h) {
      if (active) {
#pragma unroll
        for (int j = 0; j < MJ; ++j) fb[j] = SGL_TR6(base + h * 32 * RB + fb_off[j], RB);
#pragma unroll
        for (int i = 0; i < MI; ++i) fa[i] = SGL_TR6(base + h * 32 * RA + fa_off[i], RA);
      }
      if (h == 0) issue(1, kt + 1);
      else issue(0, kt + 2);
#ifdef SGL_TIMELINE
      SGL_TLP(0);
      asm volatile("s_waitcnt vmcnt(%0) lgkmcnt(0)" :: "n"(NI) : "memory");
      SGL_TLP(1);
      __builtin_amdgcn_sched_barrier(0);
      __builtin_amdgcn_s_barrier();
      __builtin_amdgcn_sched_barrier(0);
      SGL_TLP(2);
#else
      pp_end_read<NI>();
#endif
      if (active) {
        __builtin_amdgcn_s_setprio(1);
#pragma unroll
        for (int i = 0; i < MI; ++i)
#pragma unroll
          for (int j = 0; j < MJ; ++j)
            acc[i][j] = mfma_16x16x32(fa[i], fb[j], acc[i][j]);
        __builtin_amdgcn_s_setprio(0);
      }
#ifdef SGL_TIMELINE
      asm volatile("s_nop 0" ::"v"(acc[0][0]), "v"(acc[MI - 1][MJ - 1]));
      SGL_TLP(3);
#endif
      SGL_PP_END_MFMA();
      SGL_TLP(4);
    }
  }
#ifdef SGL_TIMELINE
  if (lane == 0 && active && (w == 0 || w == 4)) {
    for (int i = 0; i < 5; ++i) atomicAdd(&g_tn6_tl[(w >> 2) * 6 + i], tlp[i]);
    atomicAdd(&g_tn6_tl[(w >> 2) * 6 + 5], (unsigned long long)(2 * nk));
  }
#endif
#undef SGL_TR6
  if (grp == 0) SGL_PP_END_MFMA();
  asm volatile("s_waitcnt vmcnt(0)" ::: "memory");
  EpiParams pq = p;
  if (p.split_stride) pq.out = reinterpret_cast<float*>(p.out) + (size_t)split * p.split_stride;
  store_tile_pp<G, EPI_F32, float>(smem, acc, wr, wc, lane, t, n1_0, n2_0, N1, N2, pq);
}

#ifdef SGL_TIMELINE
template <int NC, typename Print>
static void timeline_report(hipStream_t s, unsigned long long (&counters)[NC], Print&& print) {
  if (!getenv("SGL_TIMELINE")) return;
  unsigned long long h[NC];
  (void)hipStreamSynchronize(s);
  (void)hipMemcpyFromSymbol(h, HIP_SYMBOL(counters), sizeof(h));
  print(h);
  memset(h, 0, sizeof(h));
  (void)hipMemcpyToSymbol(HIP_SYMBOL(counters), h, sizeof(h));
}
#endif

template <typename G, int EPI, typename TOut, typename TIn>
static hipError_t launch_nt_pp(const TIn* A, int lda, const TIn* B, int ldb, int M, int N, int K, const EpiParams& p,
                               hipStream_t s) {
  const hipError_t e = set_max_dynamic_lds_once<&gemm_nt6_kernel<G, EPI, TOut, TIn>>(G::LDS);
  if (e != hipSuccess) return e;
  const int tiles_m = (M + G::BM - 1) / G::BM, tiles_n = (N + G::BN - 1) / G::BN;
  static const int band_env = getenv("SGL_BAND") ? atoi(getenv("SGL_BAND")) : 0;
  const int band_h = band_env != 0 ? band_env : -8;
  const int grid = band_h < 0 ? 8 * (((tiles_m + 7) / 8) * tiles_n)
                              : ((tiles_m * tiles_n + 7) / 8) * 8;
  EpiParams pp = p;
#ifdef SGL_TIMELINE
  static const bool skip_epi = getenv("SGL_NT6_SKIP_EPI") != nullptr;
  if (skip_epi && EPI != EPI_F32) pp.atomic = 77;
#endif
  hipLaunchKernelGGL((gemm_nt6_kernel<G, EPI, TOut, TIn>), dim3(grid), dim3(512), G::LDS, s, A, lda, B, ldb, M, N, K,
                     tiles_m, tiles_n, band_h, pp);
#ifdef SGL_TIMELINE
  timeline_report(s, g_nt6_tl, [&](const unsigned long long* h) {
    if (h[2])
      fprintf(stderr, "[timeline] gemm_nt6 %dx%d EPI %d M=%d N=%d K=%d: %llu tiles, main loop %.0f, epilogue %.0f cycles per tile\n",
              G::BM, G::BN, EPI, M, N, K, h[2], (double)h[0] / h[2], (double)h[1] / h[2]);
  });
#endif
  return hipGetLastError();
}

template <typename G, typename TIn>
static hipError_t gemm_nt_pp(const void* A, int lda, const void* B, int ldb, int M, int N, int K, int epi, int out_dtype,
                             const EpiParams& p, hipStream_t s) {
  return dispatch_epilogue<TIn>(epi, out_dtype, [&](auto tag) {
    using T = decltype(tag);
    if constexpr (G::takes(T::epi))
      return launch_nt_pp<G, T::epi, typename T::out, TIn>((const TIn*)A, lda, (const TIn*)B, ldb, M, N, K, p, s);
    else
      return hipErrorInvalidValue;
  });
}
template <typename TIn>
hipError_t gemm_nt256(const void* A, int lda, const void* B, int ldb, int M, int N, int K, int epi, int out_dtype,
                      const EpiParams& p, hipStream_t s) {
  return gemm_nt_pp<NtTile256, TIn>(A, lda, B, ldb, M, N, K, epi, out_dtype, p, s);
}
template <typename TIn>
hipError_t gemm_nt384(const void* A, int lda, const void* B, int ldb, int M, int N, int K, int epi, int out_dtype,
                      const EpiParams& p, hipStream_t s) {
  return gemm_nt_pp<NtTile384, TIn>(A, lda, B, ldb, M, N, K, epi, out_dtype, p, s);
}

template <typename G, typename TIn>
static hipError_t launch_tn_pp(const void* A, int lda, const void* B, int ldb, int Mred, int N1, int N2, int m_per,
                               int splits, const EpiParams& p, hipStream_t s) {
  const hipError_t e = set_max_dynamic_lds_once<&gemm_tn6_kernel<G, TIn>>(G::LDS);
  if (e != hipSuccess) return e;
  const int tiles_1 = (N1 + G::BM - 1) / G::BM, tiles_2 = (N2 + G::BN - 1) / G::BN;
  const int grid = ((tiles_1 * tiles_2 * splits + 7) / 8) * 8;
  hipLaunchKernelGGL((gemm_tn6_kernel<G, TIn>), dim3(grid), dim3(512), G::LDS, s, (const TIn*)A, lda, (const TIn*)B, ldb,
                     Mred, N1, N2, m_per, splits, tiles_1, tiles_2, p);
#ifdef SGL_TIMELINE
  timeline_report(s, g_tn6_tl, [&](const unsigned long long* h) {
    for (int g = 0; g < 2; ++g)
      if (h[g * 6 + 5])
        fprintf(stderr, "[timeline] gemm_tn6 %dx%d N1=%d N2=%d Mred=%d splits=%d group %d, cycles per slot pair (read slot + MFMA slot): "
                "issue reads+DMA %.0f, wait %.0f, barrier %.0f, %d MFMAs %.0f, barrier %.0f\n", G::BM, G::BN, N1, N2, Mred, splits, g,
                (double)h[g * 6 + 0] / h[g * 6 + 5], (double)h[g * 6 + 1] / h[g * 6 + 5], (double)h[g * 6 + 2] / h[g * 6 + 5],
                G::MI * G::MJ, (double)h[g * 6 + 3] / h[g * 6 + 5], (double)h[g * 6 + 4] / h[g * 6 + 5]);
  });
#endif
  return hipGetLastError();
}
template <typename TIn>
hipError_t gemm_tn256(const void* A, int lda, const void* B, int ldb, int Mred, int N1, int N2, int m_per, int splits,
                      const EpiParams& p, hipStream_t s) {
  return launch_tn_pp<NtTile256, TIn>(A, lda, B, ldb, Mred, N1, N2, m_per, splits, p, s);
}
template <typename TIn>
hipError_t gemm_tn384(const void* A, int lda, const void* B, int ldb, int Mred, int N1, int N2, int m_per, int splits,
                      const EpiParams& p, hipStream_t s) {
  return launch_tn_pp<NtTile384, TIn>(A, lda, B, ldb, Mred, N1, N2, m_per, splits, p, s);
}

#define SGL_INSTANTIATE_PP(TIn)                                                                                        \
  template hipError_t gemm_nt256<TIn>(const void*, int, const void*, int, int, int, int, int, int, const EpiParams&,   \
                                      hipStream_t);                                                                    \
  template hipError_t gemm_nt384<TIn>(const void*, int, const void*, int, int, int, int, int, int, const EpiParams&,   \
                                      hipStream_t);                                                                    \
  template hipError_t gemm_tn256<TIn>(const void*, int, const void*, int, int, int, int, int, int, const EpiParams&,   \
                                      hipStream_t);                                                                    \
  template hipError_t gemm_tn384<TIn>(const void*, int, const void*, int, int, int, int, int, int, const EpiParams&,   \
                                      hipStream_t);
SGL_INSTANTIATE_PP(bf16)
SGL_INSTANTIATE_PP(f16)
#undef SGL_INSTANTIATE_PP

}
```

### deepfake-detection-using-clip-based-siglip-2-vision-transformers_amd/csrc/kernels.h

```cpp
#pragma once
#include <hip/hip_runtime.h>
#include <stddef.h>
#include <stdint.h>

#include "siglip_hip.h"

namespace sgl {

enum DType : int {
  DT_F32 = 0,
  DT_BF16 = 1,
  DT_F32_MFMA = 2,
  DT_F16 = 3,
};
static inline size_t dtype_size(int dt) { return (dt == DT_BF16 || dt == DT_F16) ? 2 : 4; }

template <auto Kernel>
hipError_t set_max_dynamic_lds_once(int bytes) {
  static bool done = false;
  if (done) return hipSuccess;
  const hipError_t e =
      hipFuncSetAttribute(reinterpret_cast<const void*>(Kernel), hipFuncAttributeMaxDynamicSharedMemorySize, bytes);
  done = e == hipSuccess;
  return e;
}

static inline bool view_box_ok(const sgl_view& r, int B, int Hs, int Ws) {
  return r.src >= 0 && r.src < B && r.x0 >= 0 && r.x0 < r.x1 && r.x1 <= Ws && r.y0 >= 0 && r.y0 < r.y1 && r.y1 <= Hs;
}

enum Epi : int {
  EPI_STORE = 0,
  EPI_BIAS_GELU = 1,
  EPI_RES_F32 = 2,
  EPI_QKV = 3,
  EPI_GELU_BWD = 4,
  EPI_POS_F32 = 5,
  EPI_F32 = 6,
};

struct EpiParams {
  void* out = nullptr;   int ldo = 0;
  void* out2 = nullptr;  int ldo2 = 0;
  const float* bias = nullptr;
  const float* res = nullptr;  int ldr = 0;
  const void* aux = nullptr;   int ldaux = 0;
  const float* pos = nullptr;  int pos_rows = 1;
  int tokens = 1, heads = 1, head_dim = 8, head_dim_pad = 8, batch = 1;
  float alpha = 1.0f;
  int accumulate = 0;
  int atomic = 0;
  float* colsum = nullptr;
  int colsum_ld = 0;
  int gelu_grad_form = 0;
  size_t split_stride = 0;
};

hipError_t quantize_mx(const void* x, int x_dtype, int ldx, int M, int K, int Kp, void* q, void* sc, hipStream_t s);
hipError_t layernorm_fwd_mx(const float* x, const float* gamma, const float* beta, void* q, void* sc, int M, int D, int Kp,
                            float eps, hipStream_t s);
hipError_t gemm_nt_mx(const void* A, const void* As, const void* B, const void* Bs, int M, int N, int Kp, int epi,
                      const EpiParams& p, void* out_sc, hipStream_t s);

hipError_t layernorm_fwd(const float* x, const float* gamma, const float* beta, void* y, int y_dtype, int ldy,
                         float* mean, float* rstd, int M, int D, float eps, hipStream_t s);
int layernorm_bwd_blocks(int M);
hipError_t layernorm_bwd(const void* dy, int dy_dtype, int lddy, const float* x, const float* mean,
                         const float* rstd, const float* gamma, const float* dres, float* dx, void* dx_lp,
                         int lp_dtype, float* partial, int nblk, int M, int D, hipStream_t s);
hipError_t reduce_partials(const float* partial, int nblk, int stride, float* out, int n, int accumulate,
                           hipStream_t s);
hipError_t reduce_partials3(const float* partial, int nblk, int stride, float* o0, float* o1, float* o2, int n, int a0,
                            int a1, int a2, hipStream_t s);

hipError_t im2col(const float* pix, int channels_last, void* out, int out_dtype, int B, int H, int W, int P,
                  int Kp, hipStream_t s);
hipError_t col2im(const float* d_cols, int B, int H, int W, int P, int Kp, float* d_pixels, int channels_last,
                  hipStream_t s);
hipError_t cast_pad(const float* src, int R, int C, int lds_, void* dst, int dst_dtype, int Rp, int Cp, int ldd,
                    hipStream_t s);
struct CastMat {
  const float* src;
  void* dst;
  void* dst_t;
  int R, C, lds, Rp, Cp, ldd, ldt, tiles_c, tile0;
};
struct CastJob {
  CastMat m[6];
  const float* vsrc[4];
  float* vdst[4];
  int vn[4], vnp[4];
  int nmat = 0, nvec = 0, ntiles = 0;
};
void cast_job_add(CastJob& job, const float* src, int R, int C, int lds_, void* dst, int Rp, int Cp, int ldd, void* dst_t,
                  int ldt);
void cast_job_add_vec(CastJob& job, const float* src, int n, float* dst, int np);
hipError_t cast_job_run(const CastJob& job, int dst_dtype, hipStream_t s);
hipError_t split3_rows(const float* src, int R, int C, int ld, void* dst, int Cs, int b_side, hipStream_t s);
hipError_t split3_stack(const float* src, int R, int C, int ld, void* dst, int Cs, int b_side, hipStream_t s);
int colsum_chunks(int M);
hipError_t colsum(const void* in, int dtype, int ld, int M, int N, int n_out, float* partial ,
                  float* out, int accumulate, hipStream_t s);
hipError_t batch_sum(const float* in, int B, size_t n, float* out, int accumulate, hipStream_t s);
hipError_t vecmat_f32(const float* v, const float* W, int rows, int cols, float* scratch, float* out, int accumulate,
                      hipStream_t s);
hipError_t pos_resize(const float* table, int g0, float* out, int gh, int gw, int D, hipStream_t s);
hipError_t pos_resize_bwd(const float* dout, int gh, int gw, float* dtable, int g0, int D, hipStream_t s);
hipError_t copy_f32(const float* src, float* dst, size_t n, hipStream_t s);
hipError_t cast_f32(const float* src, void* dst, int dst_dtype, size_t n, hipStream_t s);
hipError_t add_f32(const float* a, const float* b, float* out, size_t n, hipStream_t s);
static inline size_t pool_attn_lds_floats(int N, int DP, int backward) {
  const size_t part = (size_t)N * (DP / 8) > (size_t)256 * 8 ? (size_t)N * (DP / 8) : (size_t)256 * 8;
  return part + (backward ? 2 : 1) * (size_t)N + 8;
}
static inline int pool_attn_max_tokens(int DP, int backward) {
  return (int)((64 * 1024 / sizeof(float) - 8) / (size_t)(DP / 8 + (backward ? 2 : 1)));
}
hipError_t pool_attn_fwd(const float* q, const void* K, const void* V, int dtype, void* out ,
                         float* probs , int B, int H, int N, int dh, int DP, hipStream_t s);
hipError_t pool_attn_bwd(const float* q, const void* K, const void* V, int dtype, const float* probs,
                         const float* dout , void* dkv ,
                         float* dq_partial , int B, int H, int N, int dh, int DP, hipStream_t s);

hipError_t gemm_f32_generic(const float* A, long sam, long sak, const float* B, long sbn, long sbk, int M, int N,
                            int K, int epi, int out_dtype, const EpiParams& p, hipStream_t s);

hipError_t gemm_nt_bf16(const void* A, int lda, const void* B, int ldb, int M, int N, int K, int epi,
                        int out_dtype, const EpiParams& p, hipStream_t s);
hipError_t reduce_splits(const float* ws, int splits, size_t stride, int N1, int N2, float* out, int ldo, int accumulate,
                         hipStream_t s);
hipError_t gemm_tn_bf16(const void* A, int lda, const void* B, int ldb, int Mred, int N1, int N2, int splits,
                        const EpiParams& p, hipStream_t s, float* split_ws = nullptr, size_t split_ws_bytes = 0);
hipError_t gemm_nt_f16(const void* A, int lda, const void* B, int ldb, int M, int N, int K, int epi, int out_dtype,
                       const EpiParams& p, hipStream_t s);
hipError_t gemm_tn_f16(const void* A, int lda, const void* B, int ldb, int Mred, int N1, int N2, int splits,
                       const EpiParams& p, hipStream_t s, float* split_ws = nullptr, size_t split_ws_bytes = 0);
template <typename TIn>
hipError_t gemm_nt256(const void* A, int lda, const void* B, int ldb, int M, int N, int K, int epi, int out_dtype,
                      const EpiParams& p, hipStream_t s);
template <typename TIn>
hipError_t gemm_nt384(const void* A, int lda, const void* B, int ldb, int M, int N, int K, int epi, int out_dtype,
                      const EpiParams& p, hipStream_t s);
template <typename TIn>
hipError_t gemm_tn256(const void* A, int lda, const void* B, int ldb, int Mred, int N1, int N2, int m_per, int splits,
                      const EpiParams& p, hipStream_t s);
template <typename TIn>
hipError_t gemm_tn384(const void* A, int lda, const void* B, int ldb, int Mred, int N1, int N2, int m_per, int splits,
                      const EpiParams& p, hipStream_t s);

struct TnPlan {
  int tile, splits, m_per;
};
constexpr TnPlan tn_plan(int Mred, int N1, int N2, size_t ws_bytes, int tile = 0) {
  TnPlan best = {0, 0, 0};
  long best_cost = 0;
  for (int g = 0; g < 2; ++g) {
    const int bm = g ? 384 : 256, bn = g ? 192 : 256, area8 = g ? 9 : 8;
    if (tile != 0 && tile != bm) continue;
    const int tiles = ((N1 + bm - 1) / bm) * ((N2 + bn - 1) / bn);
    for (int sp = 1; sp == 1 || (tiles * sp <= 256 && Mred / sp >= 1024); ++sp) {
      if (sp > 1 && (size_t)sp * N1 * N2 * sizeof(float) > ws_bytes) break;
      const int m_per = ((Mred + sp - 1) / sp + 63) / 64 * 64;
      const long cost = (long)area8 * m_per;
      if (best.tile == 0 || cost < best_cost) {
        best = {bm, (Mred + m_per - 1) / m_per, m_per};
        best_cost = cost;
      }
    }
  }
  return best;
}
constexpr bool tn_plan_is(int Mred, int N1, int N2, size_t ws_bytes, int tile, int splits) {
  const TnPlan p = tn_plan(Mred, N1, N2, ws_bytes);
  return (tile == 0 || p.tile == tile) && p.splits == splits;
}
constexpr size_t kTnSlabBytes = (size_t)256 * 384 * 192 * 4;
static_assert(tn_plan_is(93312, 1152, 1152, kTnSlabBytes, 384, 14), "out_proj dW");
static_assert(tn_plan_is(93312, 3456, 1152, kTnSlabBytes, 384, 4), "QKV dW");
static_assert(tn_plan_is(93312, 4304, 1152, kTnSlabBytes, 256, 3), "fc1 dW");
static_assert(tn_plan_is(93312, 1152, 4304, kTnSlabBytes, 256, 3), "fc2 dW");
static_assert(tn_plan_is(4133, 520, 1152, kTnSlabBytes, 0, 4) && tn_plan(4133, 520, 1152, kTnSlabBytes).m_per == 1088, "digest case");
static_assert(tn_plan_is(2048, 512, 512, kTnSlabBytes, 256, 2) && tn_plan(2048, 512, 512, kTnSlabBytes).m_per == 1024, "digest case");

hipError_t attn_fwd(const void* q, const void* k, const void* v, int dtype, void* out, float* lse, int B, int H,
                    int N, int dh, int DP, int ld_qkv, hipStream_t s);
hipError_t attn_bwd(const void* q, const void* k, const void* v, const void* out, const void* dout,
                    const float* lse, int dtype, void* dqkv, float* delta, float* reserved, int B, int H, int N,
                    int dh, int DP, int ld_qkv, hipStream_t s);

}
```

### deepfake-detection-using-clip-based-siglip-2-vision-transformers_amd/csrc/layernorm.hip

```cpp
#include "common.hip.h"
#include "kernels.h"

namespace sgl {

constexpr int LN_MAXV_MAX = 8;

template <typename TOut, int LN_MAXV>
__global__ __launch_bounds__(256) void ln_fwd_kernel(const float* __restrict__ x, const float* __restrict__ gamma,
                                                     const float* __restrict__ beta, TOut* __restrict__ y, int ldy,
                                                     float* __restrict__ mean, float* __restrict__ rstd, int M, int D,
                                                     float eps) {
  const int lane = lane_id();
  const int nv = D >> 2;
  const int stride = gridDim.x * 4;
  int row = blockIdx.x * 4 + wave_id();
  if (row >= M) return;
  f32x4 v[LN_MAXV], nx[LN_MAXV];
#pragma unroll
  for (int i = 0; i < LN_MAXV; ++i) {
    const int c = lane + i * 64;
    const f32x4 z = {0.f, 0.f, 0.f, 0.f};
    v[i] = (c < nv) ? __builtin_nontemporal_load(reinterpret_cast<const f32x4*>(x + (size_t)row * D) + c) : z;
    nx[i] = z;
  }
  const float invD = 1.0f / (float)D;
  for (; row < M; row += stride) {
    const int nrow = row + stride;
    if (nrow < M) {
#pragma unroll
      for (int i = 0; i < LN_MAXV; ++i) {
        const int c = lane + i * 64;
        if (c < nv) nx[i] = __builtin_nontemporal_load(reinterpret_cast<const f32x4*>(x + (size_t)nrow * D) + c);
      }
    }
    float s = 0.f;
#pragma unroll
    for (int i = 0; i < LN_MAXV; ++i) s += (v[i][0] + v[i][1]) + (v[i][2] + v[i][3]);
    const float mu = wave_sum(s) * invD;
    float q = 0.f;
#pragma unroll
    for (int i = 0; i < LN_MAXV; ++i) {
      const int c = lane + i * 64;
      if (c < nv) {
#pragma unroll
        for (int j = 0; j < 4; ++j) {
          const float d = v[i][j] - mu;
          q += d * d;
        }
      }
    }
    const float rs = 1.0f / sqrtf(wave_sum(q) * invD + eps);
    TOut* yr = y + (size_t)row * ldy;
#pragma unroll
    for (int i = 0; i < LN_MAXV; ++i) {
      const int c = lane + i * 64;
      if (c < nv) {
        const f32x4 g = reinterpret_cast<const f32x4*>(gamma)[c];
        const f32x4 b = reinterpret_cast<const f32x4*>(beta)[c];
        float o[4];
#pragma unroll
        for (int j = 0; j < 4; ++j) o[j] = (v[i][j] - mu) * rs * g[j] + b[j];
        Vec<TOut, 4>::st_nt(yr + c * 4, o);
      }
    }
    if (lane == 0) {
      mean[row] = mu;
      rstd[row] = rs;
    }
#pragma unroll
    for (int i = 0; i < LN_MAXV; ++i) v[i] = nx[i];
  }
}

template <typename TOut>
static hipError_t ln_fwd_launch(const float* x, const float* gamma, const float* beta, TOut* y, int ldy, float* mean,
                                float* rstd, int M, int D, float eps, hipStream_t s) {
  int blocks = (M + 3) / 4;
  if (blocks > 16384) blocks = 16384;
  dim3 grid(blocks), block(256);
  if (D <= 512)
    hipLaunchKernelGGL((ln_fwd_kernel<TOut, 2>), grid, block, 0, s, x, gamma, beta, y, ldy, mean, rstd, M, D, eps);
  else if (D <= 1280)
    hipLaunchKernelGGL((ln_fwd_kernel<TOut, 5>), grid, block, 0, s, x, gamma, beta, y, ldy, mean, rstd, M, D, eps);
  else
    hipLaunchKernelGGL((ln_fwd_kernel<TOut, 8>), grid, block, 0, s, x, gamma, beta, y, ldy, mean, rstd, M, D, eps);
  return hipGetLastError();
}

hipError_t layernorm_fwd(const float* x, const float* gamma, const float* beta, void* y, int y_dtype, int ldy,
                         float* mean, float* rstd, int M, int D, float eps, hipStream_t s) {
  if (D % 4 || D > 64 * 4 * LN_MAXV_MAX || ldy % 4) return hipErrorInvalidValue;
  if (M == 0) return hipSuccess;
  if (y_dtype == DT_BF16) return ln_fwd_launch<bf16>(x, gamma, beta, (bf16*)y, ldy, mean, rstd, M, D, eps, s);
  if (y_dtype == DT_F16) return ln_fwd_launch<f16>(x, gamma, beta, (f16*)y, ldy, mean, rstd, M, D, eps, s);
  return ln_fwd_launch<float>(x, gamma, beta, (float*)y, ldy, mean, rstd, M, D, eps, s);
}

template <typename TDy, typename TLp, int LN_MAXV>
__global__ __launch_bounds__(256, (LN_MAXV <= 5 ? 3 : 1)) void ln_bwd_kernel(const TDy* __restrict__ dy, int lddy, const float* __restrict__ x,
                                                     const float* __restrict__ mean, const float* __restrict__ rstd,
                                                     const float* __restrict__ gamma, const float* __restrict__ dres,
                                                     float* __restrict__ dx, TLp* __restrict__ dx_lp,
                                                     float* __restrict__ partial, int M, int D) {
  extern __shared__ __attribute__((aligned(16))) float ln_smem[];
  const int lane = lane_id(), w = wave_id();
  const int nv = D >> 2;
  float* gsm = ln_smem + (size_t)4 * D;
  for (int j = threadIdx.x; j < D; j += 256) gsm[j] = gamma[j];
  __syncthreads();
  using DyVec = __attribute__((ext_vector_type(4))) TDy;
  f32x4 dg[LN_MAXV], db[LN_MAXV], ds[LN_MAXV];
#pragma unroll
  for (int i = 0; i < LN_MAXV; ++i) {
    const f32x4 z = {0.f, 0.f, 0.f, 0.f};
    dg[i] = z;
    db[i] = z;
    ds[i] = z;
  }
  const float invD = 1.0f / (float)D;
  for (int row = blockIdx.x * 4 + w; row < M; row += gridDim.x * 4) {
    const f32x4* xr = reinterpret_cast<const f32x4*>(x + (size_t)row * D);
    const TDy* dyr = dy + (size_t)row * lddy;
    const f32x4* rr = dres ? reinterpret_cast<const f32x4*>(dres + (size_t)row * D) : nullptr;
    f32x4 xv[LN_MAXV], rv[LN_MAXV];
    DyVec dv[LN_MAXV];
#pragma unroll
    for (int i = 0; i < LN_MAXV; ++i) {
      const int c = lane + i * 64;
      if (c < nv) {
        xv[i] = __builtin_nontemporal_load(xr + c);
        dv[i] = __builtin_nontemporal_load(reinterpret_cast<const DyVec*>(dyr + c * 4));
        if (rr) rv[i] = __builtin_nontemporal_load(rr + c);
      }
    }
    const float mu = mean[row], rs = rstd[row];
    float c1 = 0.f, c2 = 0.f;
#pragma unroll
    for (int i = 0; i < LN_MAXV; ++i) {
      const int c = lane + i * 64;
      if (c < nv) {
        const f32x4 gm = reinterpret_cast<const f32x4*>(gsm)[c];
#pragma unroll
        for (int j = 0; j < 4; ++j) {
          const float d = (float)dv[i][j];
          const float h = (xv[i][j] - mu) * rs;
          const float g = d * gm[j];
          c1 += g;
          c2 += g * h;
          dg[i][j] += d * h;
          db[i][j] += d;
        }
      }
    }
    c1 = wave_sum(c1) * invD;
    c2 = wave_sum(c2) * invD;
    float* dxr = dx + (size_t)row * D;
#pragma unroll
    for (int i = 0; i < LN_MAXV; ++i) {
      const int c = lane + i * 64;
      if (c < nv) {
        const f32x4 gm = reinterpret_cast<const f32x4*>(gsm)[c];
        float o[4];
#pragma unroll
        for (int j = 0; j < 4; ++j) {
          const float h = (xv[i][j] - mu) * rs;
          const float g = (float)dv[i][j] * gm[j];
          o[j] = rs * (g - c1 - h * c2);
        }
        if (rr) {
#pragma unroll
          for (int j = 0; j < 4; ++j) o[j] += rv[i][j];
        }
        Vec<float, 4>::st_nt(dxr + c * 4, o);
#pragma unroll
        for (int j = 0; j < 4; ++j) ds[i][j] += o[j];
        if (dx_lp) Vec<TLp, 4>::st_nt(dx_lp + (size_t)row * D + c * 4, o);
      }
    }
  }
  if (!partial) return;
  float* mine = ln_smem + (size_t)w * D;
  float* out = partial + (size_t)blockIdx.x * 3 * D;
#pragma unroll
  for (int ph = 0; ph < 3; ++ph) {
#pragma unroll
    for (int i = 0; i < LN_MAXV; ++i) {
      const int c = lane + i * 64;
      if (c < nv) reinterpret_cast<f32x4*>(mine)[c] = (ph == 0) ? dg[i] : ((ph == 1) ? db[i] : ds[i]);
    }
    __syncthreads();
    for (int j = threadIdx.x; j < D; j += 256)
      out[ph * D + j] = (ln_smem[j] + ln_smem[D + j]) + (ln_smem[2 * D + j] + ln_smem[3 * D + j]);
    __syncthreads();
  }
}

int layernorm_bwd_blocks(int M) {
  int b = (M + 3) / 4;
  return b < 1 ? 1 : (b > 768 ? 768 : b);
}

template <typename TDy, typename TLp>
static hipError_t ln_bwd_launch2(const void* dy, int lddy, const float* x, const float* mean, const float* rstd,
                                 const float* gamma, const float* dres, float* dx, void* dx_lp, float* partial,
                                 int nblk, int M, int D, hipStream_t s) {
  dim3 grid(nblk), block(256);
  const size_t smem = (size_t)5 * D * sizeof(float);
#define SGL_LNB(V)                                                                                                  \
  hipLaunchKernelGGL((ln_bwd_kernel<TDy, TLp, V>), grid, block, smem, s, (const TDy*)dy, lddy, x, mean, rstd, gamma, \
                     dres, dx, (TLp*)dx_lp, partial, M, D)
  if (D <= 512)
    SGL_LNB(2);
  else if (D <= 1280)
    SGL_LNB(5);
  else
    SGL_LNB(8);
#undef SGL_LNB
  return hipGetLastError();
}

template <typename TDy>
static hipError_t ln_bwd_launch(const void* dy, int lddy, const float* x, const float* mean, const float* rstd,
                                const float* gamma, const float* dres, float* dx, void* dx_lp, int lp_dtype,
                                float* partial, int nblk, int M, int D, hipStream_t s) {
  if (lp_dtype == DT_BF16)
    return ln_bwd_launch2<TDy, bf16>(dy, lddy, x, mean, rstd, gamma, dres, dx, dx_lp, partial, nblk, M, D, s);
  if (lp_dtype == DT_F16)
    return ln_bwd_launch2<TDy, f16>(dy, lddy, x, mean, rstd, gamma, dres, dx, dx_lp, partial, nblk, M, D, s);
  return ln_bwd_launch2<TDy, float>(dy, lddy, x, mean, rstd, gamma, dres, dx, dx_lp, partial, nblk, M, D, s);
}

hipError_t layernorm_bwd(const void* dy, int dy_dtype, int lddy, const float* x, const float* mean,
                         const float* rstd, const float* gamma, const float* dres, float* dx, void* dx_lp,
                         int lp_dtype, float* partial, int nblk, int M, int D, hipStream_t s) {
  if (D % 4 || D > 64 * 4 * LN_MAXV_MAX || lddy % 4) return hipErrorInvalidValue;
  if (M == 0) return hipSuccess;
  if (dy_dtype == DT_BF16)
    return ln_bwd_launch<bf16>(dy, lddy, x, mean, rstd, gamma, dres, dx, dx_lp, lp_dtype, partial, nblk, M, D, s);
  if (dy_dtype == DT_F16)
    return ln_bwd_launch<f16>(dy, lddy, x, mean, rstd, gamma, dres, dx, dx_lp, lp_dtype, partial, nblk, M, D, s);
  return ln_bwd_launch<float>(dy, lddy, x, mean, rstd, gamma, dres, dx, dx_lp, lp_dtype, partial, nblk, M, D, s);
}

__global__ __launch_bounds__(256) void reduce_partials_kernel(const float* __restrict__ partial, int nblk, int stride,
                                                              float* __restrict__ out, int n, int accumulate) {
  __shared__ float red[8][33];
  const int c = threadIdx.x & 31, g = threadIdx.x >> 5;
  const int j = blockIdx.x * 32 + c;
  float s0 = 0.f, s1 = 0.f;
  if (j < n) {
    int b = g;
    for (; b + 8 < nblk; b += 16) {
      s0 += partial[(size_t)b * stride + j];
      s1 += partial[(size_t)(b + 8) * stride + j];
    }
    if (b < nblk) s0 += partial[(size_t)b * stride + j];
  }
  red[g][c] = s0 + s1;
  __syncthreads();
  if (g == 0 && j < n) {
    float r = 0.f;
#pragma unroll
    for (int k = 0; k < 8; ++k) r += red[k][c];
    out[j] = accumulate ? out[j] + r : r;
  }
}

__global__ __launch_bounds__(256) void reduce_partials3_kernel(const float* __restrict__ partial, int nblk, int stride,
                                                               float* __restrict__ o0, float* __restrict__ o1,
                                                               float* __restrict__ o2, int n, int a0, int a1, int a2) {
  __shared__ float red[8][33];
  const int c = threadIdx.x & 31, g = threadIdx.x >> 5;
  const int j = blockIdx.x * 32 + c;
  const int which = j / n, jj = j - which * n;
  float* o = which == 0 ? o0 : (which == 1 ? o1 : o2);
  const int acc = which == 0 ? a0 : (which == 1 ? a1 : a2);
  const bool live = (j < 3 * n) && o;
  float s0 = 0.f, s1 = 0.f, s2 = 0.f, s3 = 0.f;
  if (live) {
    int b = g;
    for (; b + 24 < nblk; b += 32) {
      s0 += partial[(size_t)b * stride + j];
      s1 += partial[(size_t)(b + 8) * stride + j];
      s2 += partial[(size_t)(b + 16) * stride + j];
      s3 += partial[(size_t)(b + 24) * stride + j];
    }
    for (; b < nblk; b += 8) s0 += partial[(size_t)b * stride + j];
  }
  red[g][c] = (s0 + s1) + (s2 + s3);
  __syncthreads();
  if (g == 0 && live) {
    float r = 0.f;
#pragma unroll
    for (int k = 0; k < 8; ++k) r += red[k][c];
    o[jj] = acc ? o[jj] + r : r;
  }
}

hipError_t reduce_partials3(const float* partial, int nblk, int stride, float* o0, float* o1, float* o2, int n, int a0,
                            int a1, int a2, hipStream_t s) {
  if (n == 0 || (!o0 && !o1 && !o2)) return hipSuccess;
  hipLaunchKernelGGL(reduce_partials3_kernel, dim3((3 * n + 31) / 32), dim3(256), 0, s, partial, nblk, stride, o0, o1,
                     o2, n, a0, a1, a2);
  return hipGetLastError();
}

hipError_t reduce_partials(const float* partial, int nblk, int stride, float* out, int n, int accumulate,
                           hipStream_t s) {
  if (n == 0) return hipSuccess;
  hipLaunchKernelGGL(reduce_partials_kernel, dim3((n + 31) / 32), dim3(256), 0, s, partial, nblk, stride, out, n,
                     accumulate);
  return hipGetLastError();
}

}
```

### deepfake-detection-using-clip-based-siglip-2-vision-transformers_amd/lib.py

```python
from __future__ import annotations

import ctypes as C
import os
import re

_HERE = os.path.dirname(os.path.abspath(__file__))
LIB_PATH = os.environ.get("SGL_LIB_PATH") or os.path.join(_HERE, "libsiglip_hip.so")
HEADER_PATH = os.path.join(os.path.dirname(_HERE), "include", "siglip_hip.h")

SGL_DTYPE_F32, SGL_DTYPE_BF16, SGL_DTYPE_BF16X3, SGL_DTYPE_F16, SGL_DTYPE_MXFP8 = 0, 1, 2, 3, 5
SGL_DTYPE_U8 = 6
SEG_EVAL_AUC_BINS = 4096
SEG_TERM_FOCAL, SEG_TERM_BOUNDARY, SEG_TERM_TV = 1, 2, 4
SGL_RECOMPUTE_NONE, SGL_RECOMPUTE_BLOCKS = 0, 1
EPI_STORE, EPI_BIAS_GELU, EPI_RES_F32, EPI_QKV, EPI_GELU_BWD, EPI_POS_F32, EPI_F32 = range(7)
STATUS = {0: "ok", -1: "bad shape", -2: "unsupported configuration", -3: "buffer too small", -4: "HIP error",
          -5: "null pointer"}

_fp = C.c_void_p


class SglConfig(C.Structure):
    _fields_ = [("hidden_size", C.c_int), ("intermediate_size", C.c_int), ("num_layers", C.c_int),
                ("num_heads", C.c_int), ("patch_size", C.c_int), ("native_grid", C.c_int),
                ("layer_norm_eps", C.c_float), ("compute_dtype", C.c_int), ("use_head", C.c_int)]


LAYER_FIELDS = ["ln1_w", "ln1_b", "q_w", "q_b", "k_w", "k_b", "v_w", "v_b", "o_w", "o_b", "ln2_w", "ln2_b",
                "fc1_w", "fc1_b", "fc2_w", "fc2_b"]
HEAD_FIELDS = ["probe", "in_proj_w", "in_proj_b", "out_proj_w", "out_proj_b", "head_ln_w", "head_ln_b",
               "head_fc1_w", "head_fc1_b", "head_fc2_w", "head_fc2_b"]


class SglLayerPtrs(C.Structure):
    _fields_ = [(n, _fp) for n in LAYER_FIELDS]


class SglWeights(C.Structure):
    _fields_ = ([("patch_w", _fp), ("patch_b", _fp), ("pos", _fp), ("layers", C.POINTER(SglLayerPtrs)),
                 ("post_ln_w", _fp), ("post_ln_b", _fp)] + [(n, _fp) for n in HEAD_FIELDS])


class SglGrads(C.Structure):
    _fields_ = ([("patch_w", _fp), ("patch_b", _fp), ("pos", _fp), ("layers", C.POINTER(SglLayerPtrs)),
                 ("post_ln_w", _fp), ("post_ln_b", _fp)] + [(n, _fp) for n in HEAD_FIELDS] +
                [("accumulate", C.c_int)])


class SglAdamwTensor(C.Structure):
    _fields_ = [("p", _fp), ("g", _fp), ("m", _fp), ("v", _fp), ("n", C.c_uint64), ("lr", C.c_float),
                ("weight_decay", C.c_float)]


class SglAdamwAux(C.Structure):
    _fields_ = [("dst", _fp), ("dst_t", _fp), ("dst_f32", _fp), ("ema", _fp), ("ld", C.c_int), ("ld_t", C.c_int),
                ("rows", C.c_int), ("cols", C.c_int), ("row0", C.c_int), ("dtype", C.c_int), ("group", C.c_int),
                ("reserved", C.c_int)]


class SglCastMat(C.Structure):
    _fields_ = [("src", _fp), ("dst", _fp), ("dst_t", _fp)] + [(n, C.c_int) for n in ("R", "C", "lds", "Rp", "Cp", "ldd",
                                                                                    "ldt")]


class SglCastVec(C.Structure):
    _fields_ = [("src", _fp), ("dst", _fp), ("n", C.c_int), ("np", C.c_int)]


class SglView(C.Structure):
    _fields_ = [(n, C.c_int32) for n in ("src", "x0", "y0", "x1", "y1", "turns", "keep_canvas", "flip")]


_lib = None


def declared_symbols() -> list[str]:
    with open(HEADER_PATH) as f:
        text = f.read()
    text = re.sub(r"/\*.*?\*/", "", text, flags=re.S)
    return sorted(set(re.findall(r"\b(sgl_[a-z0-9_]+)\s*\(", text)))


def _sig(lib, name, restype, argtypes):
    fn = getattr(lib, name)
    fn.restype = restype
    fn.argtypes = argtypes
    return fn


def load():
    global _lib
    if _lib is not None:
        return _lib
    if not os.path.exists(LIB_PATH):
        raise RuntimeError(
            f"{LIB_PATH} not found: build it with `python -c 'import __graft_entry__ as g; g.build()'` "
            "(hipcc --offload-arch=gfx950).  There is no CPU fallback for the encoder path.")
    lib = C.CDLL(LIB_PATH)
    missing = [s for s in declared_symbols() if not hasattr(lib, s)]
    if missing:
        raise RuntimeError(f"{LIB_PATH} lacks symbols declared in siglip_hip.h: {missing}")
    i, sz, f = C.c_int, C.c_size_t, C.c_float
    psz = C.POINTER(C.c_size_t)
    _sig(lib, "sgl_abi_version", i, [])
    _sig(lib, "sgl_status_string", C.c_char_p, [i])
    _sig(lib, "sgl_create", C.c_void_p, [C.POINTER(SglConfig)])
    _sig(lib, "sgl_create_ex", C.c_void_p, [C.POINTER(SglConfig), i])
    _sig(lib, "sgl_destroy", None, [C.c_void_p])
    _sig(lib, "sgl_last_hip_error", i, [C.c_void_p])
    _sig(lib, "sgl_query_sizes", i, [C.c_void_p, i, i, i, i, psz, psz, psz])
    _sig(lib, "sgl_prepare_weights", i, [C.c_void_p, C.POINTER(SglWeights), _fp, sz, _fp])
    _sig(lib, "sgl_prepare_weights_dirty", i, [C.c_void_p, C.POINTER(SglWeights), _fp, sz, C.c_char_p, i, _fp])
    _sig(lib, "sgl_forward", i, [C.c_void_p, C.POINTER(SglWeights), _fp, _fp, i, i, i, i, i, _fp, i, _fp, _fp, _fp, sz,
                                 _fp, sz, _fp])
    _sig(lib, "sgl_forward_ex", i, [C.c_void_p, C.POINTER(SglWeights), _fp, _fp, i, i, i, i, i, _fp, i, _fp, _fp, _fp, sz,
                                    _fp, sz, i, _fp])
    _sig(lib, "sgl_forward_slots", i, [C.c_void_p, C.POINTER(SglWeights), _fp, _fp, i, i, i, i, i, C.POINTER(_fp), _fp, _fp,
                                       _fp, sz, _fp, sz, i, _fp])
    _sig(lib, "sgl_backward_begin_p", i, [C.c_void_p, C.POINTER(SglWeights), _fp, C.POINTER(SglGrads), i, i, i, _fp, _fp,
                                          _fp, _fp, _fp, sz, _fp, sz, _fp])
    _sig(lib, "sgl_backward_layer_p", i, [C.c_void_p, C.POINTER(SglWeights), _fp, C.POINTER(SglGrads), i, i, i, i, _fp,
                                          _fp, i, _fp, sz, _fp, sz, _fp])
    _sig(lib, "sgl_backward_begin", i, [C.c_void_p, C.POINTER(SglWeights), _fp, C.POINTER(SglGrads), i, i, i, _fp, _fp,
                                        _fp, _fp, _fp, sz, _fp, sz, _fp])
    _sig(lib, "sgl_backward_layer", i, [C.c_void_p, C.POINTER(SglWeights), _fp, C.POINTER(SglGrads), i, i, i, i, _fp,
                                        _fp, i, _fp, sz, _fp, sz, _fp])
    _sig(lib, "sgl_backward_embed", i, [C.c_void_p, C.POINTER(SglWeights), C.POINTER(SglGrads), i, i, i, i, _fp, sz,
                                        _fp, sz, _fp])
    _sig(lib, "sgl_query_input_grad_bytes", i, [C.c_void_p, i, i, i, psz])
    _sig(lib, "sgl_backward_embed_px", i, [C.c_void_p, C.POINTER(SglWeights), C.POINTER(SglGrads), i, i, i, i, _fp, i, _fp,
                                           sz, _fp, sz, _fp, sz, _fp])
    _sig(lib, "sgl_backward", i, [C.c_void_p, C.POINTER(SglWeights), _fp, C.POINTER(SglGrads), i, i, i, i, _fp,
                                  C.POINTER(_fp), _fp, _fp, i, i, _fp, sz, _fp, sz, _fp])
    _sig(lib, "sgl_op_layernorm_fwd", i, [_fp, _fp, _fp, _fp, i, _fp, _fp, i, i, f, _fp])
    _sig(lib, "sgl_op_layernorm_bwd", i, [_fp, i, _fp, _fp, _fp, _fp, _fp, _fp, _fp, i, _fp, _fp, _fp, sz, i, i, _fp])
    _sig(lib, "sgl_op_gemm_nt", i, [i, _fp, i, _fp, i, i, i, i, i, _fp, i, _fp, i, _fp, _fp, i, _fp, i, _fp, i, i, i,
                                    i, i, i, _fp])
    _sig(lib, "sgl_op_quantize_mxfp8", i, [_fp, i, i, i, i, i, _fp, _fp, _fp])
    _sig(lib, "sgl_op_layernorm_fwd_mx", i, [_fp, _fp, _fp, _fp, _fp, i, i, i, f, _fp])
    _sig(lib, "sgl_op_gemm_nt_mx", i, [_fp, _fp, _fp, _fp, i, i, i, i, _fp, i, _fp, _fp, _fp, i, i, i, i, i, i, _fp])
    _sig(lib, "sgl_op_gemm_tn", i, [i, _fp, i, _fp, i, i, i, i, i, _fp, i, i, _fp])
    _sig(lib, "sgl_op_gemm_tn_ws", i, [i, _fp, i, _fp, i, i, i, i, i, _fp, i, i, _fp, sz, _fp])
    _sig(lib, "sgl_op_attn_fwd", i, [i, _fp, _fp, _fp, _fp, _fp, i, i, i, i, i, i, _fp])
    _sig(lib, "sgl_op_attn_bwd", i, [i, _fp, _fp, _fp, _fp, _fp, _fp, _fp, _fp, i, i, i, i, i, i, _fp])
    _sig(lib, "sgl_op_colsum", i, [i, _fp, i, i, i, _fp, i, _fp, sz, _fp])
    _sig(lib, "sgl_op_im2col", i, [_fp, i, _fp, i, i, i, i, i, i, _fp])
    _sig(lib, "sgl_op_col2im", i, [_fp, i, i, i, i, i, _fp, i, _fp])
    _sig(lib, "sgl_op_pos_resize", i, [_fp, i, _fp, i, i, i, _fp])
    _sig(lib, "sgl_op_pool_attn_fwd", i, [i, _fp, _fp, _fp, _fp, _fp, i, i, i, i, i, _fp])
    _sig(lib, "sgl_op_pool_attn_bwd", i, [i, _fp, _fp, _fp, _fp, _fp, _fp, _fp, i, i, i, i, i, _fp])
    _sig(lib, "sgl_op_pos_resize_bwd", i, [_fp, i, i, _fp, i, i, _fp])
    _sig(lib, "sgl_op_cast_pad", i, [_fp, i, i, i, _fp, i, i, i, i, _fp])
    _sig(lib, "sgl_op_cast_job", i, [C.POINTER(SglCastMat), i, C.POINTER(SglCastVec), i, i, _fp])
    _sig(lib, "sgl_op_split3", i, [_fp, i, i, i, _fp, i, i, i, _fp])
    _sig(lib, "sgl_op_batch_sum", i, [_fp, i, sz, _fp, i, _fp])
    _sig(lib, "sgl_op_vecmat", i, [_fp, _fp, i, i, _fp, sz, _fp, i, _fp])
    _sig(lib, "sgl_op_reduce_partials", i, [_fp, i, i, _fp, i, i, _fp])
    _sig(lib, "sgl_op_reduce_partials3", i, [_fp, i, i, _fp, _fp, _fp, i, i, i, i, _fp])
    _sig(lib, "sgl_op_reduce_splits", i, [_fp, i, sz, i, i, _fp, i, i, _fp])
    _sig(lib, "sgl_op_add_f32", i, [_fp, _fp, _fp, sz, _fp])
    _sig(lib, "sgl_op_cast_f32", i, [_fp, _fp, i, sz, _fp])
    i64 = C.c_int64
    _sig(lib, "sgl_adamw_plan", i64, [C.POINTER(C.c_uint64), i, C.POINTER(C.c_int32), i64])
    _sig(lib, "sgl_op_grad_norm", i, [_fp, _fp, i64, f, _fp, _fp, _fp])
    _sig(lib, "sgl_op_adamw", i, [_fp, _fp, i64, C.c_double, C.c_double, C.c_double, i, _fp, _fp])
    _sig(lib, "sgl_op_ema", i, [_fp, _fp, i64, C.c_double, _fp])
    _sig(lib, "sgl_adamw_bind_shadows", i, [C.c_void_p, C.POINTER(SglWeights), _fp, C.POINTER(SglAdamwTensor),
                                            C.POINTER(SglAdamwAux), i])
    _sig(lib, "sgl_op_grad_norm_scaled", i, [_fp, _fp, i64, f, f, _fp, _fp, _fp])
    _sig(lib, "sgl_op_adamw_ex", i, [_fp, _fp, _fp, i64, C.c_double, C.c_double, C.c_double, i, _fp,
                                     C.POINTER(C.c_float), i, C.c_double, _fp])
    _sig(lib, "sgl_op_dwconv3x3", i, [_fp, i, _fp, _fp, _fp, i, i, i, i, i, _fp])
    _sig(lib, "sgl_op_dwconv3x3_wgrad_scratch_bytes", sz, [i, i, i, i])
    _sig(lib, "sgl_op_dwconv3x3_wgrad", i, [_fp, _fp, i, _fp, i, _fp, sz, i, i, i, i, _fp])
    _sig(lib, "sgl_op_preprocess", i, [_fp, i, i, i, i, _fp, i, i, i, i, i, f, f, _fp, f, _fp])
    _sig(lib, "sgl_op_preprocess_bwd_scratch_bytes", sz, [i, i, i, i])
    _sig(lib, "sgl_op_preprocess_bwd", i, [_fp, i, i, i, i, f, _fp, f, _fp, _fp, sz, _fp])
    _sig(lib, "sgl_op_preprocess_aug", i, [_fp, i, i, i, i, _fp, i, i, i, i, i, f, f, _fp, _fp, _fp])
    _sig(lib, "sgl_op_preprocess_aug_bwd_scratch_bytes", sz, [i, i, i, i])
    _sig(lib, "sgl_op_preprocess_aug_bwd", i, [_fp, _fp, i, i, i, i, i, f, _fp, _fp, _fp, sz, _fp])
    _sig(lib, "sgl_op_preprocess_views_scratch_bytes", sz, [i, i])
    _sig(lib, "sgl_op_preprocess_views", i, [_fp, i, i, i, i, C.POINTER(SglView), i, _fp, i, i, i, i, i, f, f, _fp, sz,
                                             _fp])
    _sig(lib, "sgl_op_preprocess_views_bwd_scratch_bytes", sz, [C.POINTER(SglView), i, i])
    _sig(lib, "sgl_op_preprocess_views_bwd", i, [_fp, i, i, i, C.POINTER(SglView), i, i, f, _fp, _fp, sz, _fp])
    _sig(lib, "sgl_op_freq_features_scratch_bytes", sz, [i, i, i])
    _sig(lib, "sgl_op_freq_features", i, [_fp, i, i, i, C.POINTER(SglView), i, _fp, _fp, i, _fp, _fp, sz, _fp])
    _sig(lib, "sgl_op_l2norm_tmean_fwd", i, [_fp, _fp, _fp, i, i, i, _fp])
    _sig(lib, "sgl_op_l2norm_tmean_bwd", i, [_fp, _fp, _fp, _fp, i, i, i, _fp])
    _sig(lib, "sgl_op_gate_mul", i, [_fp, _fp, _fp, sz, i, _fp])
    _sig(lib, "sgl_op_gate_mul_bwd", i, [_fp, _fp, _fp, _fp, _fp, sz, i, _fp])
    _sig(lib, "sgl_op_seg_loss_chunks", i, [i])
    _sig(lib, "sgl_op_seg_loss_fwd", i, [_fp, _fp, _fp, i, i, i, _fp])
    _sig(lib, "sgl_op_seg_loss_bwd", i, [_fp, _fp, _fp, _fp, _fp, i, i, i, f, _fp])
    _sig(lib, "sgl_op_seg_loss_ex_fwd", i, [_fp, _fp, _fp, i, i, i, i, f, _fp])
    _sig(lib, "sgl_op_seg_loss_ex_bwd", i, [_fp, _fp, _fp, _fp, _fp, i, i, i, i, f, f, f, _fp])
    _sig(lib, "sgl_op_seg_eval_auc_bins", i, [])
    _sig(lib, "sgl_op_seg_eval", i, [_fp, _fp, i, _fp, _fp, i, _fp, _fp, i, i, i, _fp])
    _lib = lib
    return lib


class SglError(RuntimeError):
    pass


def check(status: int, what: str, ctx=None):
    if status == 0:
        return
    msg = STATUS.get(status, f"status {status}")
    if status == -4 and ctx is not None and _lib is not None:
        msg += f" (hipError_t {_lib.sgl_last_hip_error(ctx)})"
    raise SglError(f"{what}: {msg}")


def ptr(t) -> int | None:
    return None if t is None else t.data_ptr()


def current_stream_handle(device) -> int:
    import torch
    return torch.cuda.current_stream(device).cuda_stream


def call(symbol: str, device, *args) -> None:
    import torch
    fn = getattr(load(), symbol)
    with torch.cuda.device(device):
        status = fn(*args, current_stream_handle(device))
    check(status, symbol)


def dtype_code(dtype) -> int:
    import torch
    codes = {torch.float32: SGL_DTYPE_F32, torch.bfloat16: SGL_DTYPE_BF16, torch.float16: SGL_DTYPE_F16}
    if dtype not in codes:
        raise ValueError(f"output dtype must be float32, bfloat16 or float16, not {dtype}")
    return codes[dtype]
```

### include/siglip_hip.h

```cpp
#ifndef SIGLIP_HIP_H
#define SIGLIP_HIP_H
#include <stddef.h>
#include <stdint.h>

#ifdef __cplusplus
extern "C" {
#endif

typedef struct sgl_ctx sgl_ctx;
typedef void* sgl_stream;

enum { SGL_DTYPE_F32 = 0, SGL_DTYPE_BF16 = 1, SGL_DTYPE_BF16X3 = 2, SGL_DTYPE_F16 = 3, SGL_DTYPE_MXFP8 = 5 };
enum { SGL_DTYPE_U8 = 6 };

typedef enum {
  SGL_OK = 0,
  SGL_ERR_BAD_SHAPE = -1,
  SGL_ERR_UNSUPPORTED = -2,
  SGL_ERR_WORKSPACE = -3,
  SGL_ERR_HIP = -4,
  SGL_ERR_NULL = -5
} sgl_status;

typedef struct {
  int hidden_size;
  int intermediate_size;
  int num_layers;
  int num_heads;
  int patch_size;
  int native_grid;
  float layer_norm_eps;
  int compute_dtype;
  int use_head;
} sgl_config;

typedef struct {
  const float *ln1_w, *ln1_b;
  const float *q_w, *q_b, *k_w, *k_b, *v_w, *v_b, *o_w, *o_b;
  const float *ln2_w, *ln2_b;
  const float *fc1_w, *fc1_b, *fc2_w, *fc2_b;
} sgl_layer_weights;

typedef struct {
  const float *patch_w, *patch_b;
  const float* pos;
  const sgl_layer_weights* layers;
  const float *post_ln_w, *post_ln_b;
  const float *probe;
  const float *in_proj_w, *in_proj_b;
  const float *out_proj_w, *out_proj_b;
  const float *head_ln_w, *head_ln_b;
  const float *head_fc1_w, *head_fc1_b, *head_fc2_w, *head_fc2_b;
} sgl_weights;

typedef struct {
  float *ln1_w, *ln1_b;
  float *q_w, *q_b, *k_w, *k_b, *v_w, *v_b, *o_w, *o_b;
  float *ln2_w, *ln2_b;
  float *fc1_w, *fc1_b, *fc2_w, *fc2_b;
} sgl_layer_grads;

typedef struct {
  float *patch_w, *patch_b, *pos;
  const sgl_layer_grads* layers;
  float *post_ln_w, *post_ln_b;
  float *probe, *in_proj_w, *in_proj_b, *out_proj_w, *out_proj_b, *head_ln_w, *head_ln_b;
  float *head_fc1_w, *head_fc1_b, *head_fc2_w, *head_fc2_b;
  int accumulate;
} sgl_grads;

sgl_ctx* sgl_create(const sgl_config* cfg);
enum { SGL_RECOMPUTE_NONE = 0, SGL_RECOMPUTE_BLOCKS = 1 };
sgl_ctx* sgl_create_ex(const sgl_config* cfg, int recompute);
void sgl_destroy(sgl_ctx* ctx);
int sgl_last_hip_error(const sgl_ctx* ctx);
const char* sgl_status_string(int status);
int sgl_abi_version(void);

int sgl_query_sizes(const sgl_ctx* ctx, int B, int H, int W, int train, size_t* shadow_bytes, size_t* saved_bytes,
                    size_t* ws_bytes);

int sgl_prepare_weights(sgl_ctx* ctx, const sgl_weights* w, void* shadow, size_t shadow_bytes, sgl_stream stream);
int sgl_prepare_weights_dirty(sgl_ctx* ctx, const sgl_weights* w, void* shadow, size_t shadow_bytes,
                              const unsigned char* layer_dirty, int globals_dirty, sgl_stream stream);

int sgl_forward(sgl_ctx* ctx, const sgl_weights* w, const void* shadow, const float* pixels, int channels_last, int B,
                int H, int W, int interpolate_pos, float* hidden_states, int hs_slots, float* last_hidden,
                float* pooled, void* saved, size_t saved_bytes, void* ws, size_t ws_bytes, sgl_stream stream);
int sgl_forward_ex(sgl_ctx* ctx, const sgl_weights* w, const void* shadow, const float* pixels, int channels_last, int B,
                   int H, int W, int interpolate_pos, float* hidden_states, int hs_slots, float* last_hidden,
                   float* pooled, void* saved, size_t saved_bytes, void* ws, size_t ws_bytes, int first_trainable_block,
                   sgl_stream stream);

int sgl_forward_slots(sgl_ctx* ctx, const sgl_weights* w, const void* shadow, const float* pixels, int channels_last,
                      int B, int H, int W, int interpolate_pos, float* const* hs_slots, float* last_hidden,
                      float* pooled, void* saved, size_t saved_bytes, void* ws, size_t ws_bytes,
                      int first_trainable_block, sgl_stream stream);

int sgl_backward_begin(sgl_ctx* ctx, const sgl_weights* w, const void* shadow, const sgl_grads* g, int B, int H, int W,
                       const float* hidden_states, const float* d_last_hidden, const float* d_pooled,
                       const float* d_tap_last, const void* saved, size_t saved_bytes, void* ws, size_t ws_bytes,
                       sgl_stream stream);
int sgl_backward_layer(sgl_ctx* ctx, const sgl_weights* w, const void* shadow, const sgl_grads* g, int layer, int B,
                       int H, int W, const float* hidden_states, const float* d_tap, int need_dx, const void* saved,
                       size_t saved_bytes, void* ws, size_t ws_bytes, sgl_stream stream);
int sgl_backward_begin_p(sgl_ctx* ctx, const sgl_weights* w, const void* shadow, const sgl_grads* g, int B, int H, int W,
                         const float* hs_last, const float* d_last_hidden, const float* d_pooled,
                         const float* d_tap_last, const void* saved, size_t saved_bytes, void* ws, size_t ws_bytes,
                         sgl_stream stream);
int sgl_backward_layer_p(sgl_ctx* ctx, const sgl_weights* w, const void* shadow, const sgl_grads* g, int layer, int B,
                         int H, int W, const float* hs_in, const float* d_tap, int need_dx, const void* saved,
                         size_t saved_bytes, void* ws, size_t ws_bytes, sgl_stream stream);
int sgl_backward_embed(sgl_ctx* ctx, const sgl_weights* w, const sgl_grads* g, int B, int H, int W, int interpolate_pos,
                       const void* saved, size_t saved_bytes, void* ws, size_t ws_bytes, sgl_stream stream);
int sgl_query_input_grad_bytes(const sgl_ctx* ctx, int B, int H, int W, size_t* scratch_bytes);
int sgl_backward_embed_px(sgl_ctx* ctx, const sgl_weights* w, const sgl_grads* g, int B, int H, int W,
                          int interpolate_pos, float* d_pixels, int channels_last, void* px_scratch,
                          size_t px_scratch_bytes, const void* saved, size_t saved_bytes, void* ws, size_t ws_bytes,
                          sgl_stream stream);
int sgl_backward(sgl_ctx* ctx, const sgl_weights* w, const void* shadow, const sgl_grads* g, int B, int H, int W,
                 int interpolate_pos, const float* hidden_states, const float* const* d_taps,
                 const float* d_last_hidden, const float* d_pooled, int first_trainable_block, int train_embeddings,
                 const void* saved, size_t saved_bytes, void* ws, size_t ws_bytes, sgl_stream stream);

int sgl_op_layernorm_fwd(const float* x, const float* gamma, const float* beta, void* y, int y_dtype, float* mean,
                         float* rstd, int M, int D, float eps, sgl_stream stream);
int sgl_op_layernorm_bwd(const void* dy, int dy_dtype, const float* x, const float* mean, const float* rstd,
                         const float* gamma, const float* dres, float* dx, void* dx_lp, int lp_dtype, float* dgamma,
                         float* dbeta, float* scratch, size_t scratch_bytes, int M, int D, sgl_stream stream);
enum { SGL_EPI_STORE = 0, SGL_EPI_BIAS_GELU = 1, SGL_EPI_RES_F32 = 2, SGL_EPI_QKV = 3, SGL_EPI_GELU_BWD = 4,
       SGL_EPI_POS_F32 = 5, SGL_EPI_F32 = 6 };
int sgl_op_gemm_nt(int dtype, const void* A, int lda, const void* B, int ldb, int M, int N, int K, int epi, void* out,
                   int ldo, void* out2, int ldo2, const float* bias, const float* res, int ldr, const void* aux,
                   int ldaux, const float* pos, int pos_rows, int tokens, int heads, int head_dim, int head_dim_pad,
                   int batch, sgl_stream stream);
int sgl_op_quantize_mxfp8(const void* x, int x_dtype, int ldx, int M, int K, int Kp, void* q, void* scales,
                          sgl_stream stream);
int sgl_op_layernorm_fwd_mx(const float* x, const float* gamma, const float* beta, void* q, void* scales, int M, int D,
                            int Kp, float eps, sgl_stream stream);
int sgl_op_gemm_nt_mx(const void* A, const void* As, const void* B, const void* Bs, int M, int N, int Kp, int epi,
                      void* out, int ldo, void* out_scales, const float* bias, const float* res, int ldr, int tokens,
                      int heads, int head_dim, int head_dim_pad, int batch, sgl_stream stream);
int sgl_op_gemm_tn(int dtype, const void* A, int lda, const void* B, int ldb, int Mred, int N1, int N2, int splits,
                   float* out, int ldo, int accumulate, sgl_stream stream);
int sgl_op_gemm_tn_ws(int dtype, const void* A, int lda, const void* B, int ldb, int Mred, int N1, int N2, int splits,
                      float* out, int ldo, int accumulate, float* scratch, size_t scratch_bytes, sgl_stream stream);
int sgl_op_attn_fwd(int dtype, const void* q, const void* k, const void* v, void* out, float* lse, int B, int H, int N,
                    int head_dim, int head_dim_pad, int ld_qkv, sgl_stream stream);
int sgl_op_attn_bwd(int dtype, const void* q, const void* k, const void* v, const void* out, const void* dout,
                    const float* lse, void* dqkv, float* delta_scratch, int B, int H, int N, int head_dim,
                    int head_dim_pad, int ld_qkv, sgl_stream stream);
int sgl_op_colsum(int dtype, const void* in, int ld, int M, int N, float* out, int accumulate, float* scratch,
                  size_t scratch_bytes, sgl_stream stream);
int sgl_op_im2col(const float* pixels, int channels_last, void* out, int out_dtype, int B, int H, int W, int P, int Kp,
                  sgl_stream stream);
int sgl_op_col2im(const float* d_cols, int B, int H, int W, int P, int Kp, float* d_pixels, int channels_last,
                  sgl_stream stream);
int sgl_op_pos_resize(const float* table, int native_grid, float* out, int gh, int gw, int D, sgl_stream stream);

int sgl_op_pool_attn_fwd(int dtype, const float* q, const void* K, const void* V, void* out, float* probs, int B, int H,
                         int N, int head_dim, int head_dim_pad, sgl_stream stream);
int sgl_op_pool_attn_bwd(int dtype, const float* q, const void* K, const void* V, const float* probs, const float* dout,
                         void* dkv, float* dq_partial, int B, int H, int N, int head_dim, int head_dim_pad,
                         sgl_stream stream);
int sgl_op_pos_resize_bwd(const float* dout, int gh, int gw, float* dtable, int native_grid, int D, sgl_stream stream);
int sgl_op_cast_pad(const float* src, int R, int C, int lds, void* dst, int dst_dtype, int Rp, int Cp, int ldd,
                    sgl_stream stream);
typedef struct {
  const float* src;
  void* dst;
  void* dst_t;
  int R, C, lds, Rp, Cp, ldd, ldt;
} sgl_cast_mat;
typedef struct {
  const float* src;
  float* dst;
  int n, np;
} sgl_cast_vec;
int sgl_op_cast_job(const sgl_cast_mat* mats, int nmat, const sgl_cast_vec* vecs, int nvec, int dst_dtype,
                    sgl_stream stream);
int sgl_op_split3(const float* src, int R, int C, int ld, void* dst, int Cs, int b_side, int stacked, sgl_stream stream);
int sgl_op_batch_sum(const float* in, int B, size_t n, float* out, int accumulate, sgl_stream stream);
int sgl_op_vecmat(const float* v, const float* W, int rows, int cols, float* scratch, size_t scratch_bytes, float* out,
                  int accumulate, sgl_stream stream);
int sgl_op_reduce_partials(const float* partial, int nblk, int stride, float* out, int n, int accumulate,
                           sgl_stream stream);
int sgl_op_reduce_partials3(const float* partial, int nblk, int stride, float* out0, float* out1, float* out2, int n,
                            int accumulate0, int accumulate1, int accumulate2, sgl_stream stream);
int sgl_op_reduce_splits(const float* ws, int splits, size_t stride, int N1, int N2, float* out, int ldo, int accumulate,
                         sgl_stream stream);
int sgl_op_add_f32(const float* a, const float* b, float* out, size_t n, sgl_stream stream);
int sgl_op_cast_f32(const float* src, void* dst, int dst_dtype, size_t n, sgl_stream stream);

int sgl_op_dwconv3x3(const void* x, int dtype, const float* w9, const float* bias, void* y, int B, int gh, int gw, int E,
                     int flip, sgl_stream stream);
size_t sgl_op_dwconv3x3_wgrad_scratch_bytes(int B, int gh, int gw, int E);
int sgl_op_dwconv3x3_wgrad(const void* x, const void* dy, int dtype, float* dw10, int accumulate, float* scratch,
                           size_t scratch_bytes, int B, int gh, int gw, int E, sgl_stream stream);

int sgl_op_preprocess(const void* src, int src_is_u8_nhwc, int B, int Hs, int Ws, void* out, int out_dtype, int S, int P,
                      int Kp, int patch_major, float mean, float std, const int* mix_index, float lam,
                      sgl_stream stream);
size_t sgl_op_preprocess_bwd_scratch_bytes(int B, int Hs, int Ws, int S);
int sgl_op_preprocess_bwd(const float* d_out, int B, int Hs, int Ws, int S, float std, const int* mix_index, float lam,
                          float* d_src, void* scratch, size_t scratch_bytes, sgl_stream stream);

typedef struct sgl_view {
  int32_t src, x0, y0, x1, y1, turns, keep_canvas, flip;
} sgl_view;
size_t sgl_op_preprocess_views_scratch_bytes(int V, int S);
int sgl_op_preprocess_views(const void* src, int src_is_u8_nhwc, int B, int Hs, int Ws, const sgl_view* views, int V,
                            void* out, int out_dtype, int S, int P, int Kp, int patch_major, float mean, float std,
                            void* scratch, size_t scratch_bytes, sgl_stream stream);
size_t sgl_op_preprocess_views_bwd_scratch_bytes(const sgl_view* views, int V, int S);
int sgl_op_preprocess_views_bwd(const float* d_out, int B, int Hs, int Ws, const sgl_view* views, int V, int S, float std,
                                float* d_src, void* scratch, size_t scratch_bytes, sgl_stream stream);

size_t sgl_op_freq_features_scratch_bytes(int V, int Hs, int Ws);
int sgl_op_freq_features(const void* src_u8_nhwc, int B, int Hs, int Ws, const sgl_view* views, int V,
                         const unsigned char* geometry, float* out , int standardize,
                         unsigned char* gray_out , void* scratch, size_t scratch_bytes,
                         sgl_stream stream);

typedef struct sgl_aug_sample {
  float flip, cos_a, sin_a, brightness, contrast, saturation, hue;
  int order[4];
  int reserved;
} sgl_aug_sample;
int sgl_op_preprocess_aug(const void* src, int src_is_u8_nhwc, int B, int Hs, int Ws, void* out, int out_dtype, int S,
                          int P, int Kp, int patch_major, float mean, float std, const sgl_aug_sample* aug,
                          float* grey_mean, sgl_stream stream);
size_t sgl_op_preprocess_aug_bwd_scratch_bytes(int B, int Hs, int Ws, int S);
int sgl_op_preprocess_aug_bwd(const float* d_out, const void* src, int src_is_u8_nhwc, int B, int Hs, int Ws, int S,
                              float std, const sgl_aug_sample* aug, float* d_src, void* scratch, size_t scratch_bytes,
                              sgl_stream stream);

int sgl_op_l2norm_tmean_fwd(const float* f, float* out, float* inv_norm, int B, int T, int D, sgl_stream stream);
int sgl_op_l2norm_tmean_bwd(const float* f, const float* inv_norm, const float* dout, float* df, int B, int T, int D,
                            sgl_stream stream);

int sgl_op_gate_mul(const void* g, const void* x, void* y, size_t n, int dtype, sgl_stream stream);
int sgl_op_gate_mul_bwd(const void* dy, const void* g, const void* x, void* dg, void* dx, size_t n, int dtype,
                        sgl_stream stream);
int sgl_op_seg_loss_chunks(int S);
int sgl_op_seg_loss_fwd(const float* logits_lr, const float* targets, float* partial, int B, int g, int S,
                        sgl_stream stream);
int sgl_op_seg_loss_bwd(const float* logits_lr, const float* targets, const float* sums, const float* coef,
                        float* dlogits_lr, int B, int g, int S, float eps, sgl_stream stream);

#define SGL_SEG_TERM_FOCAL 1
#define SGL_SEG_TERM_BOUNDARY 2
#define SGL_SEG_TERM_TV 4
int sgl_op_seg_loss_ex_fwd(const float* logits_lr, const float* targets, float* partial, int B, int g, int S, int terms,
                           float alpha, sgl_stream stream);
int sgl_op_seg_loss_ex_bwd(const float* logits_lr, const float* targets, const float* sums, const float* coef,
                           float* dlogits_lr, int B, int g, int S, int terms, float alpha, float eps, float smooth,
                           sgl_stream stream);

#define SGL_SEG_EVAL_AUC_BINS 4096
int sgl_op_seg_eval_auc_bins(void);
int sgl_op_seg_eval(const float* logits_lr, const void* targets, int target_dtype, const uint8_t* sel, const float* cuts,
                    int K, int32_t* hist, unsigned long long* auc_hist, int B, int g, int S, sgl_stream stream);

typedef struct {
  float* p;
  const float* g;
  float* m;
  float* v;
  uint64_t n;
  float lr, weight_decay;
} sgl_adamw_tensor;
int64_t sgl_adamw_plan(const uint64_t* numel, int ntensors, int32_t* blockmap, int64_t capacity_pairs);
int sgl_op_grad_norm(const sgl_adamw_tensor* table, const int32_t* blockmap, int64_t nblocks, float max_norm,
                     float* partials, float* norm_and_coef, sgl_stream stream);
int sgl_op_adamw(const sgl_adamw_tensor* table, const int32_t* blockmap, int64_t nblocks, double beta1, double beta2,
                 double eps, int step, const float* norm_and_coef, sgl_stream stream);
typedef struct {
  void* dst;
  void* dst_t;
  float* dst_f32;
  float* ema;
  int ld, ld_t, rows, cols, row0, dtype, group, reserved;
} sgl_adamw_aux;
int sgl_adamw_bind_shadows(const sgl_ctx* ctx, const sgl_weights* w, void* shadow, const sgl_adamw_tensor* table_host,
                           sgl_adamw_aux* aux_host, int ntensors);
int sgl_op_grad_norm_scaled(const sgl_adamw_tensor* table, const int32_t* blockmap, int64_t nblocks, float max_norm,
                            float grad_scale, float* partials, float* norm_and_coef, sgl_stream stream);
int sgl_op_adamw_ex(const sgl_adamw_tensor* table, const sgl_adamw_aux* aux, const int32_t* blockmap, int64_t nblocks,
                    double beta1, double beta2, double eps, int step, const float* norm_and_coef,
                    const float* group_lr_wd_host, int ngroups, double ema_decay, sgl_stream stream);
int sgl_op_ema(const sgl_adamw_tensor* table, const int32_t* blockmap, int64_t nblocks, double decay,
               sgl_stream stream);

#ifdef __cplusplus
}
#endif
#endif
```

Baseline: 438.7 images/sec.

## Run LN1 backward as passenger workgroups inside the QKV weight-grad split-K GEMM

Defers the fused QKV weight-gradient GEMM from attention backward into LN1 backward, and launches it with extra 'passenger' workgroups that run a share of the layernorm backward rows on CUs the split-K GEMM grid leaves idle. The remaining LN rows run in a range-limited layernorm kernel afterwards, followed by the usual partial reduction. This aims to fill under-occupied GPU capacity during the weight-grad GEMM and cut separate LN backward time, at the cost of a larger kernel, shared LDS budgeting, and new scheduling heuristics.

```diff
diff --git a/deepfake-detection-using-clip-based-siglip-2-vision-transformers_amd/csrc/encoder.hip b/deepfake-detection-using-clip-based-siglip-2-vision-transformers_amd/csrc/encoder.hip
--- a/deepfake-detection-using-clip-based-siglip-2-vision-transformers_amd/csrc/encoder.hip
+++ b/deepfake-detection-using-clip-based-siglip-2-vision-transformers_amd/csrc/encoder.hip
@@ -324,6 +324,24 @@
       return gemm_tn_bf16(sp_a, l1, sp_b, l2, 3 * Mred, N1, N2, tn_splits(N1, N2, 3 * Mred), p, s, slabs, slab_bytes);
     }
     return gemm_f32_generic((const float*)A, 1, lda, (const float*)B, 1, ldb, N1, N2, Mred, EPI_F32, DT_F32, p, s);
+  }
+
+  bool tn_carries_ln() const { return ctx->dt == DT_BF16 || ctx->dt == DT_F16; }
+
+  int gemm_tn_ln(const void* A, int lda, const void* B, int ldb, int Mred, int N1, int N2, float* out, int ldo,
+                 int accumulate, const void* dy, const float* x, const float* stats, int rows, const float* gamma,
+                 const float* dres, float* dx, void* dx_lp, float* dgamma, float* dbeta, float* colsum_out) const {
+    const int D = ctx->D;
+    const bool want = dgamma || dbeta || colsum_out;
+    float* part = wsf(lay.w_lnpart);
+    LnBwdArgs ln;
+    ln.dy = dy; ln.lddy = D; ln.x = x; ln.mean = stats; ln.rstd = stats + rows; ln.gamma = gamma; ln.dres = dres;
+    ln.dx = dx; ln.dx_lp = dx_lp; ln.partial = want ? part : nullptr;
+    ln.nblk = layernorm_bwd_blocks(rows); ln.M = rows; ln.D = D; ln.vb_split = -1;
+    CK(gemm_tn_ln_bwd(ctx->dt, A, lda, B, ldb, Mred, N1, N2, tn_splits(N1, N2, Mred), epi_f32_acc(out, ldo, accumulate), s,
+                      wsf(lay.w_splitws), kSplitWsBytes, ln));
+    CK(reduce_partials3(part, ln.nblk, 3 * D, dgamma, dbeta, colsum_out, D, accumulate, accumulate, 0, s));
+    return SGL_OK;
   }
 
   int bias_grad(const void* in, int ld, int M, int N, int n_out, float* out, int accumulate) const {
@@ -925,8 +943,12 @@
   return SGL_OK;
 }
 
+inline bool qkv_grads_adjacent(const sgl_layer_grads& lg, int D) {
+  return lg.q_w && lg.k_w == lg.q_w + (size_t)D * D && lg.v_w == lg.k_w + (size_t)D * D;
+}
+
 int attn_backward(const Call& c, const sgl_layer_weights& lw, const sgl_layer_grads& lg, const ShadowLayer& sl,
-                  const char* lb, int acc) {
+                  const char* lb, int acc, bool defer_qkv_dw) {
   sgl_ctx* ctx = c.ctx;
   const Layout& lay = c.lay;
   hipStream_t s = c.s;
@@ -943,8 +965,8 @@
               nullptr, lay.B, ctx->H, lay.N, ctx->dh, ctx->DP, 0, s));
   float* gw[3] = {lg.q_w, lg.k_w, lg.v_w};
   float* gb[3] = {lg.q_b, lg.k_b, lg.v_b};
-  const bool w_adj = gw[0] && gw[1] == gw[0] + (size_t)D * D && gw[2] == gw[1] + (size_t)D * D;
-  if (w_adj) CK(c.gemm_tn(dqkv, 3 * D, lb + lay.r_h1, D, M, 3 * D, D, gw[0], D, acc, true));
+  const bool w_adj = qkv_grads_adjacent(lg, D);
+  if (w_adj && !defer_qkv_dw) CK(c.gemm_tn(dqkv, 3 * D, lb + lay.r_h1, D, M, 3 * D, D, gw[0], D, acc, true));
   for (int j = 0; j < 3; ++j) {
     const char* aj = reinterpret_cast<const char*>(dqkv) + (size_t)j * D * ctx->es;
     if (!w_adj && gw[j]) CK(c.gemm_tn(aj, 3 * D, lb + lay.r_h1, D, M, D, D, gw[j], D, acc, true));
@@ -956,13 +978,17 @@
 }
 
 int ln1_backward(const Call& c, const sgl_layer_weights& lw, const sgl_layer_grads& lg, const ShadowLayer& sl,
-                 const char* lb, const float* x_in, int acc) {
+                 const char* lb, const float* x_in, int acc, bool qkv_dw) {
   sgl_ctx* ctx = c.ctx;
   const Layout& lay = c.lay;
   const int D = ctx->D, M = lay.M, dt = ctx->dt;
   float* dx = c.wsf(lay.w_dx);
   void* dh1 = c.wsp(lay.w_dh);
   CK(c.gemm_nt(c.wsp(lay.w_dqkv), 3 * D, c.sh(sl.wqkv_t), 3 * D, M, D, 3 * D, EPI_STORE, dt, epi_store(dh1, D)));
+  if (qkv_dw)
+    return c.gemm_tn_ln(c.wsp(lay.w_dqkv), 3 * D, lb + lay.r_h1, D, M, 3 * D, D, lg.q_w, D, acc, dh1, x_in,
+                        reinterpret_cast<const float*>(lb + lay.r_stats1), M, lw.ln1_w, dx, dx, c.wsp(lay.w_g), lg.ln1_w,
+                        lg.ln1_b, c.wsf(lay.w_gsum));
   RET(c.ln_backward(dh1, dt, x_in, reinterpret_cast<const float*>(lb + lay.r_stats1), M, lw.ln1_w, dx, dx,
                     c.wsp(lay.w_g), lg.ln1_w, lg.ln1_b, acc, c.wsf(lay.w_gsum)));
   return SGL_OK;
@@ -1040,10 +1066,12 @@
   char* lb = c.block(layer);
   if (c.lay.rc) RET(block_to_fc1(c, lw, sl, lb, hs_in, true));
   RET(mlp_backward(c, lw, lg, sl, lb, acc));
-  RET(attn_backward(c, lw, lg, sl, lb, acc));
+  const bool ln1 = need_dx || lg.ln1_w || lg.ln1_b;
+  const bool ride = ln1 && c.tn_carries_ln() && qkv_grads_adjacent(lg, ctx->D);
+  RET(attn_backward(c, lw, lg, sl, lb, acc, ride));
   float* dx = c.wsf(c.lay.w_dx);
   if (d_tap) CK(add_f32(dx, d_tap, dx, (size_t)c.lay.M * ctx->D, c.s));
-  if (need_dx || lg.ln1_w || lg.ln1_b) RET(ln1_backward(c, lw, lg, sl, lb, hs_in, acc));
+  if (ln1) RET(ln1_backward(c, lw, lg, sl, lb, hs_in, acc, ride));
   return SGL_OK;
 }
 
@@ -1239,6 +1267,25 @@
   return SGL_OK;
 }
 
+int sgl_op_gemm_tn_ws_ln_bwd(int dtype, const void* A, int lda, const void* B, int ldb, int Mred, int N1, int N2,
+                             int splits, float* out, int ldo, int accumulate, float* scratch, size_t scratch_bytes,
+                             const void* dy, const float* x, const float* mean, const float* rstd, const float* gamma,
+                             const float* dres, float* dx, void* dx_lp, float* partial, size_t partial_bytes, int M, int D,
+                             int vb_split, sgl_stream stream) {
+  if (!A || !B || !out || !dy || !x || !mean || !rstd || !gamma || !dx) return SGL_ERR_NULL;
+  if (dtype != DT_BF16 && dtype != DT_F16) return SGL_ERR_UNSUPPORTED;
+  const int nblk = layernorm_bwd_blocks(M);
+  if (M <= 0 || vb_split < 0 || vb_split > nblk) return SGL_ERR_BAD_SHAPE;
+  if (partial && partial_bytes < (size_t)nblk * 3 * D * 4) return SGL_ERR_WORKSPACE;
+  EpiParams p;
+  p.out = out; p.ldo = ldo; p.accumulate = accumulate;
+  LnBwdArgs ln;
+  ln.dy = dy; ln.lddy = D; ln.x = x; ln.mean = mean; ln.rstd = rstd; ln.gamma = gamma; ln.dres = dres;
+  ln.dx = dx; ln.dx_lp = dx_lp; ln.partial = partial; ln.nblk = nblk; ln.M = M; ln.D = D; ln.vb_split = vb_split;
+  CKV(gemm_tn_ln_bwd(dtype, A, lda, B, ldb, Mred, N1, N2, splits, p, (hipStream_t)stream, scratch, scratch_bytes, ln));
+  return SGL_OK;
+}
+
 int sgl_op_attn_fwd(int dtype, const void* q, const void* k, const void* v, void* out, float* lse, int B, int H, int N,
                     int head_dim, int head_dim_pad, int ld_qkv, sgl_stream stream) {
   CKV(attn_fwd(q, k, v, dtype, out, lse, B, H, N, head_dim, head_dim_pad, ld_qkv, (hipStream_t)stream));
diff --git a/deepfake-detection-using-clip-based-siglip-2-vision-transformers_amd/csrc/gemm_bf16.hip b/deepfake-detection-using-clip-based-siglip-2-vision-transformers_amd/csrc/gemm_bf16.hip
--- a/deepfake-detection-using-clip-based-siglip-2-vision-transformers_amd/csrc/gemm_bf16.hip
+++ b/deepfake-detection-using-clip-based-siglip-2-vision-transformers_amd/csrc/gemm_bf16.hip
@@ -369,4 +369,58 @@
   return gemm_tn_mfma<f16>(A, lda, B, ldb, Mred, N1, N2, splits, p, s, split_ws, split_ws_bytes);
 }
 
-}
+static int device_cus() {
+  static const int cus = [] {
+    int dev = 0, n = 0;
+    if (hipGetDevice(&dev) != hipSuccess) return 0;
+    if (hipDeviceGetAttribute(&n, hipDeviceAttributeMultiprocessorCount, dev) != hipSuccess) return 0;
+    return n;
+  }();
+  return cus;
+}
+
+template <typename TIn>
+static hipError_t gemm_tn_ln_mfma(int dtype, const void* A, int lda, const void* B, int ldb, int Mred, int N1, int N2,
+                                  int splits, const EpiParams& p, hipStream_t s, float* split_ws, size_t split_ws_bytes,
+                                  const LnBwdArgs& ln) {
+  static const bool ride_env = !(getenv("SGL_TN_PASSENGERS") && atoi(getenv("SGL_TN_PASSENGERS")) == 0);
+  static const int tile_env = getenv("SGL_TN_TILE") ? atoi(getenv("SGL_TN_TILE")) : 0;
+  const auto two_launches = [&]() {
+    const hipError_t e = gemm_tn_mfma<TIn>(A, lda, B, ldb, Mred, N1, N2, splits, p, s, split_ws, split_ws_bytes);
+    if (e != hipSuccess) return e;
+    return layernorm_bwd(ln.dy, dtype, ln.lddy, ln.x, ln.mean, ln.rstd, ln.gamma, ln.dres, ln.dx, ln.dx_lp, dtype,
+                         ln.partial, ln.nblk, ln.M, ln.D, s);
+  };
+  const bool lds_dma = N1 >= 512 && N2 >= 512 && Mred >= 2048 && !(lda % 8) && !(ldb % 8) &&
+                       (size_t)Mred * lda * 2 < (1ull << 32) && (size_t)Mred * ldb * 2 < (1ull << 32);
+  const bool ln_ok = ln.M > 0 && ln.D > 512 && ln.D <= 1280 && ln.D % 4 == 0 && ln.lddy % 4 == 0 && ln.vb_split != 0 &&
+                     ln.vb_split <= ln.nblk;
+  if (!ride_env || !lds_dma || !ln_ok || !split_ws || !tn_slabs_ok(p, N2, split_ws)) return two_launches();
+  const int tile = (tile_env == 256 || tile_env == 384) ? tile_env : 0;
+  const TnPlan plan = tn_plan(Mred, N1, N2, split_ws_bytes, tile);
+  const int P = tn_passengers(device_cus(), tn_wgs(plan, N1, N2));
+  if (plan.splits == 1 || P == 0) return two_launches();
+  LnBwdArgs lq = ln;
+  if (lq.vb_split < 0) lq.vb_split = ln_passenger_share(P, plan, ln.M, ln.nblk);
+  if (lq.vb_split == 0) return two_launches();
+  return tn_split_k(Mred, N1, N2, plan.splits, p, s, split_ws, split_ws_bytes, [&](int m_per, int nsplit, const EpiParams& q) {
+    if (!q.split_stride || nsplit != plan.splits || m_per != plan.m_per) return hipErrorInvalidValue;
+    const hipError_t e = plan.tile == 384 ? gemm_tn384_ln<TIn>(A, lda, B, ldb, Mred, N1, N2, m_per, nsplit, q, P, lq, s)
+                                          : gemm_tn256_ln<TIn>(A, lda, B, ldb, Mred, N1, N2, m_per, nsplit, q, P, lq, s);
+    if (e != hipSuccess) return e;
+    return layernorm_bwd_range(ln.dy, dtype, ln.lddy, ln.x, ln.mean, ln.rstd, ln.gamma, ln.dres, ln.dx, ln.dx_lp, dtype,
+                               ln.partial, lq.vb_split, ln.nblk, ln.M, ln.D, s);
+  });
+}
+
+hipError_t gemm_tn_ln_bwd(int dtype, const void* A, int lda, const void* B, int ldb, int Mred, int N1, int N2, int splits,
+                          const EpiParams& p, hipStream_t s, float* split_ws, size_t split_ws_bytes, const LnBwdArgs& ln) {
+  if (ln.nblk != layernorm_bwd_blocks(ln.M) || ln.vb_split > ln.nblk) return hipErrorInvalidValue;
+  if (dtype == DT_BF16)
+    return gemm_tn_ln_mfma<bf16>(dtype, A, lda, B, ldb, Mred, N1, N2, splits, p, s, split_ws, split_ws_bytes, ln);
+  if (dtype == DT_F16)
+    return gemm_tn_ln_mfma<f16>(dtype, A, lda, B, ldb, Mred, N1, N2, splits, p, s, split_ws, split_ws_bytes, ln);
+  return hipErrorInvalidValue;
+}
+
+}
diff --git a/deepfake-detection-using-clip-based-siglip-2-vision-transformers_amd/csrc/gemm_bf16_v2.hip b/deepfake-detection-using-clip-based-siglip-2-vision-transformers_amd/csrc/gemm_bf16_v2.hip
--- a/deepfake-detection-using-clip-based-siglip-2-vision-transformers_amd/csrc/gemm_bf16_v2.hip
+++ b/deepfake-detection-using-clip-based-siglip-2-vision-transformers_amd/csrc/gemm_bf16_v2.hip
@@ -7,6 +7,7 @@
 #include "common.hip.h"
 #include "epilogue.hip.h"
 #include "kernels.h"
+#include "ln_bwd.hip.h"
 
 namespace sgl {
 
@@ -376,12 +377,24 @@
   else return 2 * ((m >> 1) & 1) + 4 * ((m >> 3) & 1);
 }
 
-template <typename G, typename TIn>
+struct TnLnRider {
+  int gemm_wgs;
+  LnBwdArgs ln;
+};
+template <typename G, typename TIn, typename... Rider>
 __global__ __launch_bounds__(512, 2) void gemm_tn6_kernel(const TIn* __restrict__ A, int lda,
                                                           const TIn* __restrict__ B, int ldb, int Mred, int N1, int N2,
                                                           int m_per_split, int nsplits, int tiles_1, int tiles_2,
-                                                          EpiParams p) {
+                                                          EpiParams p, Rider... rider_) {
   extern __shared__ __attribute__((aligned(16))) char smem[];
+  if constexpr (sizeof...(Rider) > 0) {
+    static_assert(sizeof...(Rider) == 1, "one rider");
+    const TnLnRider& rider = (rider_, ...);
+    if ((int)blockIdx.x >= rider.gemm_wgs) {
+      ln_bwd_passenger<TIn>(rider.ln, (int)blockIdx.x - rider.gemm_wgs, (int)gridDim.x - rider.gemm_wgs, smem);
+      return;
+    }
+  }
   constexpr int MI = G::MI, MJ = G::MJ;
   constexpr int RA = 2 * G::BM, RB = 2 * G::BN;
   constexpr int HA = G::BM / 16, HB = G::BN / 16;
@@ -590,11 +603,21 @@
 
 template <typename G, typename TIn>
 static hipError_t launch_tn_pp(const void* A, int lda, const void* B, int ldb, int Mred, int N1, int N2, int m_per,
-                               int splits, const EpiParams& p, hipStream_t s) {
+                               int splits, const EpiParams& p, hipStream_t s, int P = 0, const LnBwdArgs* ln = nullptr) {
+  const int tiles_1 = (N1 + G::BM - 1) / G::BM, tiles_2 = (N2 + G::BN - 1) / G::BN;
+  const int grid = ((tiles_1 * tiles_2 * splits + 7) / 8) * 8;
+  if (P > 0) {
+    if (!ln || ln->D % 4 || ln->D <= 512 || ln->D > 1280 || ln->lddy % 4 || (size_t)10 * ln->D * 4 > (size_t)G::LDS ||
+        ln->vb_split < 0 || ln->vb_split > ln->nblk || ln->M <= 0)
+      return hipErrorInvalidValue;
+    const hipError_t e = set_max_dynamic_lds_once<&gemm_tn6_kernel<G, TIn, TnLnRider>>(G::LDS);
+    if (e != hipSuccess) return e;
+    hipLaunchKernelGGL((gemm_tn6_kernel<G, TIn, TnLnRider>), dim3(grid + P), dim3(512), G::LDS, s, (const TIn*)A, lda,
+                       (const TIn*)B, ldb, Mred, N1, N2, m_per, splits, tiles_1, tiles_2, p, TnLnRider{grid, *ln});
+    return hipGetLastError();
+  }
   const hipError_t e = set_max_dynamic_lds_once<&gemm_tn6_kernel<G, TIn>>(G::LDS);
   if (e != hipSuccess) return e;
-  const int tiles_1 = (N1 + G::BM - 1) / G::BM, tiles_2 = (N2 + G::BN - 1) / G::BN;
-  const int grid = ((tiles_1 * tiles_2 * splits + 7) / 8) * 8;
   hipLaunchKernelGGL((gemm_tn6_kernel<G, TIn>), dim3(grid), dim3(512), G::LDS, s, (const TIn*)A, lda, (const TIn*)B, ldb,
                      Mred, N1, N2, m_per, splits, tiles_1, tiles_2, p);
 #ifdef SGL_TIMELINE
@@ -620,6 +643,17 @@
   return launch_tn_pp<NtTile384, TIn>(A, lda, B, ldb, Mred, N1, N2, m_per, splits, p, s);
 }
 
+template <typename TIn>
+hipError_t gemm_tn256_ln(const void* A, int lda, const void* B, int ldb, int Mred, int N1, int N2, int m_per, int splits,
+                         const EpiParams& p, int P, const LnBwdArgs& ln, hipStream_t s) {
+  return launch_tn_pp<NtTile256, TIn>(A, lda, B, ldb, Mred, N1, N2, m_per, splits, p, s, P, &ln);
+}
+template <typename TIn>
+hipError_t gemm_tn384_ln(const void* A, int lda, const void* B, int ldb, int Mred, int N1, int N2, int m_per, int splits,
+                         const EpiParams& p, int P, const LnBwdArgs& ln, hipStream_t s) {
+  return launch_tn_pp<NtTile384, TIn>(A, lda, B, ldb, Mred, N1, N2, m_per, splits, p, s, P, &ln);
+}
+
 #define SGL_INSTANTIATE_PP(TIn)                                                                                        \
   template hipError_t gemm_nt256<TIn>(const void*, int, const void*, int, int, int, int, int, int, const EpiParams&,   \
                                       hipStream_t);                                                                    \
@@ -628,7 +662,11 @@
   template hipError_t gemm_tn256<TIn>(const void*, int, const void*, int, int, int, int, int, int, const EpiParams&,   \
                                       hipStream_t);                                                                    \
   template hipError_t gemm_tn384<TIn>(const void*, int, const void*, int, int, int, int, int, int, const EpiParams&,   \
-                                      hipStream_t);
+                                      hipStream_t);                                                                    \
+  template hipError_t gemm_tn256_ln<TIn>(const void*, int, const void*, int, int, int, int, int, int, const EpiParams&, \
+                                         int, const LnBwdArgs&, hipStream_t);                                          \
+  template hipError_t gemm_tn384_ln<TIn>(const void*, int, const void*, int, int, int, int, int, int, const EpiParams&, \
+                                         int, const LnBwdArgs&, hipStream_t);
 SGL_INSTANTIATE_PP(bf16)
 SGL_INSTANTIATE_PP(f16)
 #undef SGL_INSTANTIATE_PP
diff --git a/deepfake-detection-using-clip-based-siglip-2-vision-transformers_amd/csrc/kernels.h b/deepfake-detection-using-clip-based-siglip-2-vision-transformers_amd/csrc/kernels.h
--- a/deepfake-detection-using-clip-based-siglip-2-vision-transformers_amd/csrc/kernels.h
+++ b/deepfake-detection-using-clip-based-siglip-2-vision-transformers_amd/csrc/kernels.h
@@ -68,6 +68,22 @@
 hipError_t layernorm_bwd(const void* dy, int dy_dtype, int lddy, const float* x, const float* mean,
                          const float* rstd, const float* gamma, const float* dres, float* dx, void* dx_lp,
                          int lp_dtype, float* partial, int nblk, int M, int D, hipStream_t s);
+hipError_t layernorm_bwd_range(const void* dy, int dy_dtype, int lddy, const float* x, const float* mean,
+                               const float* rstd, const float* gamma, const float* dres, float* dx, void* dx_lp,
+                               int lp_dtype, float* partial, int vb0, int nblk, int M, int D, hipStream_t s);
+struct LnBwdArgs {
+  const void* dy = nullptr;  int lddy = 0;
+  const float* x = nullptr;
+  const float* mean = nullptr;
+  const float* rstd = nullptr;
+  const float* gamma = nullptr;
+  const float* dres = nullptr;
+  float* dx = nullptr;
+  void* dx_lp = nullptr;
+  float* partial = nullptr;
+  int nblk = 0, M = 0, D = 0;
+  int vb_split = 0;
+};
 hipError_t reduce_partials(const float* partial, int nblk, int stride, float* out, int n, int accumulate,
                            hipStream_t s);
 hipError_t reduce_partials3(const float* partial, int nblk, int stride, float* o0, float* o1, float* o2, int n, int a0,
@@ -182,6 +198,35 @@
 static_assert(tn_plan_is(4133, 520, 1152, kTnSlabBytes, 0, 4) && tn_plan(4133, 520, 1152, kTnSlabBytes).m_per == 1088, "digest case");
 static_assert(tn_plan_is(2048, 512, 512, kTnSlabBytes, 256, 2) && tn_plan(2048, 512, 512, kTnSlabBytes).m_per == 1024, "digest case");
 
+constexpr int tn_wgs(const TnPlan& p, int N1, int N2) {
+  const int bm = p.tile == 384 ? 384 : 256, bn = p.tile == 384 ? 192 : 256;
+  return (((N1 + bm - 1) / bm) * ((N2 + bn - 1) / bn) * p.splits + 7) / 8 * 8;
+}
+constexpr int tn_passengers(int cus, int gemm_wgs) { return cus - gemm_wgs >= 16 ? cus - gemm_wgs : 0; }
+static_assert(tn_passengers(256, tn_wgs(tn_plan(93312, 3456, 1152, kTnSlabBytes), 3456, 1152)) == 40, "QKV dW");
+static_assert(tn_passengers(256, tn_wgs(tn_plan(93312, 4304, 1152, kTnSlabBytes), 4304, 1152)) == 0, "fc1 dW");
+static_assert(tn_passengers(256, tn_wgs(tn_plan(93312, 1152, 4304, kTnSlabBytes), 1152, 4304)) == 0, "fc2 dW");
+static_assert(tn_passengers(256, 248) == 0 && tn_passengers(256, 240) == 16 && tn_passengers(256, 256) == 0 &&
+              tn_passengers(304, 216) == 88, "fewer than 16 idle CUs carry nothing");
+
+constexpr double kTnNsPerRow8 = 2.8;
+constexpr double kLnPassengerRowsPerUs = 1.8;
+constexpr int ln_passenger_share(int P, const TnPlan& p, int M, int nblk) {
+  const double gemm_us = kTnNsPerRow8 * 1e-3 * (p.tile == 384 ? 9 : 8) * p.m_per;
+  const double rows = kLnPassengerRowsPerUs * P * gemm_us;
+  const double share = rows * nblk / (M > 0 ? M : 1);
+  return share >= nblk ? nblk : (int)share;
+}
+
+hipError_t gemm_tn_ln_bwd(int dtype, const void* A, int lda, const void* B, int ldb, int Mred, int N1, int N2, int splits,
+                          const EpiParams& p, hipStream_t s, float* split_ws, size_t split_ws_bytes, const LnBwdArgs& ln);
+template <typename TIn>
+hipError_t gemm_tn256_ln(const void* A, int lda, const void* B, int ldb, int Mred, int N1, int N2, int m_per, int splits,
+                         const EpiParams& p, int P, const LnBwdArgs& ln, hipStream_t s);
+template <typename TIn>
+hipError_t gemm_tn384_ln(const void* A, int lda, const void* B, int ldb, int Mred, int N1, int N2, int m_per, int splits,
+                         const EpiParams& p, int P, const LnBwdArgs& ln, hipStream_t s);
+
 hipError_t attn_fwd(const void* q, const void* k, const void* v, int dtype, void* out, float* lse, int B, int H,
                     int N, int dh, int DP, int ld_qkv, hipStream_t s);
 hipError_t attn_bwd(const void* q, const void* k, const void* v, const void* out, const void* dout,
diff --git a/deepfake-detection-using-clip-based-siglip-2-vision-transformers_amd/csrc/layernorm.hip b/deepfake-detection-using-clip-based-siglip-2-vision-transformers_amd/csrc/layernorm.hip
--- a/deepfake-detection-using-clip-based-siglip-2-vision-transformers_amd/csrc/layernorm.hip
+++ b/deepfake-detection-using-clip-based-siglip-2-vision-transformers_amd/csrc/layernorm.hip
@@ -1,5 +1,6 @@
 #include "common.hip.h"
 #include "kernels.h"
+#include "ln_bwd.hip.h"
 
 namespace sgl {
 
@@ -101,14 +102,12 @@
                                                      const float* __restrict__ mean, const float* __restrict__ rstd,
                                                      const float* __restrict__ gamma, const float* __restrict__ dres,
                                                      float* __restrict__ dx, TLp* __restrict__ dx_lp,
-                                                     float* __restrict__ partial, int M, int D) {
+                                                     float* __restrict__ partial, int M, int D, int vb0, int nblk_total) {
   extern __shared__ __attribute__((aligned(16))) float ln_smem[];
   const int lane = lane_id(), w = wave_id();
-  const int nv = D >> 2;
   float* gsm = ln_smem + (size_t)4 * D;
   for (int j = threadIdx.x; j < D; j += 256) gsm[j] = gamma[j];
   __syncthreads();
-  using DyVec = __attribute__((ext_vector_type(4))) TDy;
   f32x4 dg[LN_MAXV], db[LN_MAXV], ds[LN_MAXV];
 #pragma unroll
   for (int i = 0; i < LN_MAXV; ++i) {
@@ -117,82 +116,15 @@
     db[i] = z;
     ds[i] = z;
   }
-  const float invD = 1.0f / (float)D;
-  for (int row = blockIdx.x * 4 + w; row < M; row += gridDim.x * 4) {
-    const f32x4* xr = reinterpret_cast<const f32x4*>(x + (size_t)row * D);
-    const TDy* dyr = dy + (size_t)row * lddy;
-    const f32x4* rr = dres ? reinterpret_cast<const f32x4*>(dres + (size_t)row * D) : nullptr;
-    f32x4 xv[LN_MAXV], rv[LN_MAXV];
-    DyVec dv[LN_MAXV];
-#pragma unroll
-    for (int i = 0; i < LN_MAXV; ++i) {
-      const int c = lane + i * 64;
-      if (c < nv) {
-        xv[i] = __builtin_nontemporal_load(xr + c);
-        dv[i] = __builtin_nontemporal_load(reinterpret_cast<const DyVec*>(dyr + c * 4));
-        if (rr) rv[i] = __builtin_nontemporal_load(rr + c);
-      }
-    }
+  const int vb = vb0 + blockIdx.x;
+  for (int row = vb * 4 + w; row < M; row += nblk_total * 4) {
+    LnRow<TDy, LN_MAXV> r;
+    ln_row_load<TDy, LN_MAXV>(r, dy, lddy, x, dres, row, D, lane);
     const float mu = mean[row], rs = rstd[row];
-    float c1 = 0.f, c2 = 0.f;
-#pragma unroll
-    for (int i = 0; i < LN_MAXV; ++i) {
-      const int c = lane + i * 64;
-      if (c < nv) {
-        const f32x4 gm = reinterpret_cast<const f32x4*>(gsm)[c];
-#pragma unroll
-        for (int j = 0; j < 4; ++j) {
-          const float d = (float)dv[i][j];
-          const float h = (xv[i][j] - mu) * rs;
-          const float g = d * gm[j];
-          c1 += g;
-          c2 += g * h;
-          dg[i][j] += d * h;
-          db[i][j] += d;
-        }
-      }
-    }
-    c1 = wave_sum(c1) * invD;
-    c2 = wave_sum(c2) * invD;
-    float* dxr = dx + (size_t)row * D;
-#pragma unroll
-    for (int i = 0; i < LN_MAXV; ++i) {
-      const int c = lane + i * 64;
-      if (c < nv) {
-        const f32x4 gm = reinterpret_cast<const f32x4*>(gsm)[c];
-        float o[4];
-#pragma unroll
-        for (int j = 0; j < 4; ++j) {
-          const float h = (xv[i][j] - mu) * rs;
-          const float g = (float)dv[i][j] * gm[j];
-          o[j] = rs * (g - c1 - h * c2);
-        }
-        if (rr) {
-#pragma unroll
-          for (int j = 0; j < 4; ++j) o[j] += rv[i][j];
-        }
-        Vec<float, 4>::st_nt(dxr + c * 4, o);
-#pragma unroll
-        for (int j = 0; j < 4; ++j) ds[i][j] += o[j];
-        if (dx_lp) Vec<TLp, 4>::st_nt(dx_lp + (size_t)row * D + c * 4, o);
-      }
-    }
+    ln_row_finish<TDy, TLp, LN_MAXV>(r, dres != nullptr, mu, rs, gsm, dx, dx_lp, row, D, lane, dg, db, ds);
   }
   if (!partial) return;
-  float* mine = ln_smem + (size_t)w * D;
-  float* out = partial + (size_t)blockIdx.x * 3 * D;
-#pragma unroll
-  for (int ph = 0; ph < 3; ++ph) {
-#pragma unroll
-    for (int i = 0; i < LN_MAXV; ++i) {
-      const int c = lane + i * 64;
-      if (c < nv) reinterpret_cast<f32x4*>(mine)[c] = (ph == 0) ? dg[i] : ((ph == 1) ? db[i] : ds[i]);
-    }
-    __syncthreads();
-    for (int j = threadIdx.x; j < D; j += 256)
-      out[ph * D + j] = (ln_smem[j] + ln_smem[D + j]) + (ln_smem[2 * D + j] + ln_smem[3 * D + j]);
-    __syncthreads();
-  }
+  ln_fold_partials<LN_MAXV>(ln_smem, partial + (size_t)vb * 3 * D, true, D, threadIdx.x, w, lane, dg, db, ds);
 }
 
 int layernorm_bwd_blocks(int M) {
@@ -203,12 +135,12 @@
 template <typename TDy, typename TLp>
 static hipError_t ln_bwd_launch2(const void* dy, int lddy, const float* x, const float* mean, const float* rstd,
                                  const float* gamma, const float* dres, float* dx, void* dx_lp, float* partial,
-                                 int nblk, int M, int D, hipStream_t s) {
-  dim3 grid(nblk), block(256);
+                                 int vb0, int nblk, int M, int D, hipStream_t s) {
+  dim3 grid(nblk - vb0), block(256);
   const size_t smem = (size_t)5 * D * sizeof(float);
 #define SGL_LNB(V)                                                                                                  \
   hipLaunchKernelGGL((ln_bwd_kernel<TDy, TLp, V>), grid, block, smem, s, (const TDy*)dy, lddy, x, mean, rstd, gamma, \
-                     dres, dx, (TLp*)dx_lp, partial, M, D)
+                     dres, dx, (TLp*)dx_lp, partial, M, D, vb0, nblk)
   if (D <= 512)
     SGL_LNB(2);
   else if (D <= 1280)
@@ -222,24 +154,30 @@
 template <typename TDy>
 static hipError_t ln_bwd_launch(const void* dy, int lddy, const float* x, const float* mean, const float* rstd,
                                 const float* gamma, const float* dres, float* dx, void* dx_lp, int lp_dtype,
-                                float* partial, int nblk, int M, int D, hipStream_t s) {
+                                float* partial, int vb0, int nblk, int M, int D, hipStream_t s) {
   if (lp_dtype == DT_BF16)
-    return ln_bwd_launch2<TDy, bf16>(dy, lddy, x, mean, rstd, gamma, dres, dx, dx_lp, partial, nblk, M, D, s);
+    return ln_bwd_launch2<TDy, bf16>(dy, lddy, x, mean, rstd, gamma, dres, dx, dx_lp, partial, vb0, nblk, M, D, s);
   if (lp_dtype == DT_F16)
-    return ln_bwd_launch2<TDy, f16>(dy, lddy, x, mean, rstd, gamma, dres, dx, dx_lp, partial, nblk, M, D, s);
-  return ln_bwd_launch2<TDy, float>(dy, lddy, x, mean, rstd, gamma, dres, dx, dx_lp, partial, nblk, M, D, s);
+    return ln_bwd_launch2<TDy, f16>(dy, lddy, x, mean, rstd, gamma, dres, dx, dx_lp, partial, vb0, nblk, M, D, s);
+  return ln_bwd_launch2<TDy, float>(dy, lddy, x, mean, rstd, gamma, dres, dx, dx_lp, partial, vb0, nblk, M, D, s);
+}
+
+hipError_t layernorm_bwd_range(const void* dy, int dy_dtype, int lddy, const float* x, const float* mean,
+                               const float* rstd, const float* gamma, const float* dres, float* dx, void* dx_lp,
+                               int lp_dtype, float* partial, int vb0, int nblk, int M, int D, hipStream_t s) {
+  if (D % 4 || D > 64 * 4 * LN_MAXV_MAX || lddy % 4 || vb0 < 0 || vb0 > nblk) return hipErrorInvalidValue;
+  if (M == 0 || vb0 == nblk) return hipSuccess;
+  if (dy_dtype == DT_BF16)
+    return ln_bwd_launch<bf16>(dy, lddy, x, mean, rstd, gamma, dres, dx, dx_lp, lp_dtype, partial, vb0, nblk, M, D, s);
+  if (dy_dtype == DT_F16)
+    return ln_bwd_launch<f16>(dy, lddy, x, mean, rstd, gamma, dres, dx, dx_lp, lp_dtype, partial, vb0, nblk, M, D, s);
+  return ln_bwd_launch<float>(dy, lddy, x, mean, rstd, gamma, dres, dx, dx_lp, lp_dtype, partial, vb0, nblk, M, D, s);
 }
 
 hipError_t layernorm_bwd(const void* dy, int dy_dtype, int lddy, const float* x, const float* mean,
                          const float* rstd, const float* gamma, const float* dres, float* dx, void* dx_lp,
                          int lp_dtype, float* partial, int nblk, int M, int D, hipStream_t s) {
-  if (D % 4 || D > 64 * 4 * LN_MAXV_MAX || lddy % 4) return hipErrorInvalidValue;
-  if (M == 0) return hipSuccess;
-  if (dy_dtype == DT_BF16)
-    return ln_bwd_launch<bf16>(dy, lddy, x, mean, rstd, gamma, dres, dx, dx_lp, lp_dtype, partial, nblk, M, D, s);
-  if (dy_dtype == DT_F16)
-    return ln_bwd_launch<f16>(dy, lddy, x, mean, rstd, gamma, dres, dx, dx_lp, lp_dtype, partial, nblk, M, D, s);
-  return ln_bwd_launch<float>(dy, lddy, x, mean, rstd, gamma, dres, dx, dx_lp, lp_dtype, partial, nblk, M, D, s);
+  return layernorm_bwd_range(dy, dy_dtype, lddy, x, mean, rstd, gamma, dres, dx, dx_lp, lp_dtype, partial, 0, nblk, M, D, s);
 }
 
 __global__ __launch_bounds__(256) void reduce_partials_kernel(const float* __restrict__ partial, int nblk, int stride,
diff --git a/deepfake-detection-using-clip-based-siglip-2-vision-transformers_amd/csrc/ln_bwd.hip.h b/deepfake-detection-using-clip-based-siglip-2-vision-transformers_amd/csrc/ln_bwd.hip.h
--- /dev/null
+++ b/deepfake-detection-using-clip-based-siglip-2-vision-transformers_amd/csrc/ln_bwd.hip.h
@@ -0,0 +1,188 @@
+#pragma once
+#include "common.hip.h"
+#include "kernels.h"
+
+namespace sgl {
+
+template <typename TDy, int LN_MAXV>
+struct LnRow {
+  using DyVec = __attribute__((ext_vector_type(4))) TDy;
+  f32x4 xv[LN_MAXV], rv[LN_MAXV];
+  DyVec dv[LN_MAXV];
+};
+
+template <typename TDy, int LN_MAXV>
+__device__ __forceinline__ void ln_row_load(LnRow<TDy, LN_MAXV>& r, const TDy* __restrict__ dy, int lddy,
+                                            const float* __restrict__ x, const float* __restrict__ dres, int row, int D,
+                                            int lane) {
+  using DyVec = typename LnRow<TDy, LN_MAXV>::DyVec;
+  const int nv = D >> 2;
+  const f32x4* xr = reinterpret_cast<const f32x4*>(x + (size_t)row * D);
+  const TDy* dyr = dy + (size_t)row * lddy;
+  const f32x4* rr = dres ? reinterpret_cast<const f32x4*>(dres + (size_t)row * D) : nullptr;
+#pragma unroll
+  for (int i = 0; i < LN_MAXV; ++i) {
+    const int c = lane + i * 64;
+    if (c < nv) {
+      r.xv[i] = __builtin_nontemporal_load(xr + c);
+      r.dv[i] = __builtin_nontemporal_load(reinterpret_cast<const DyVec*>(dyr + c * 4));
+      if (rr) r.rv[i] = __builtin_nontemporal_load(rr + c);
+    }
+  }
+}
+
+template <typename TDy, int LN_MAXV, bool RES>
+__device__ __forceinline__ void ln_row_load_all(LnRow<TDy, LN_MAXV>& r, const TDy* __restrict__ dy, int lddy,
+                                                const float* __restrict__ x, const float* __restrict__ dres, int row, int D,
+                                                int lane) {
+  using DyVec = typename LnRow<TDy, LN_MAXV>::DyVec;
+  const int nv = D >> 2;
+  const f32x4* xr = reinterpret_cast<const f32x4*>(x + (size_t)row * D);
+  const TDy* dyr = dy + (size_t)row * lddy;
+  const f32x4* rr = reinterpret_cast<const f32x4*>(dres + (size_t)(RES ? row : 0) * D);
+#pragma unroll
+  for (int i = 0; i < LN_MAXV; ++i) {
+    const int c = (lane + i * 64 < nv) ? lane + i * 64 : nv - 1;
+    r.xv[i] = __builtin_nontemporal_load(xr + c);
+    r.dv[i] = __builtin_nontemporal_load(reinterpret_cast<const DyVec*>(dyr + c * 4));
+    if constexpr (RES) r.rv[i] = __builtin_nontemporal_load(rr + c);
+  }
+}
+
+template <typename TDy, typename TLp, int LN_MAXV>
+__device__ __forceinline__ void ln_row_finish(const LnRow<TDy, LN_MAXV>& r, bool has_res, float mu, float rs,
+                                              const float* gsm, float* __restrict__ dx, TLp* __restrict__ dx_lp, int row,
+                                              int D, int lane, f32x4 (&dg)[LN_MAXV], f32x4 (&db)[LN_MAXV],
+                                              f32x4 (&ds)[LN_MAXV]) {
+#pragma clang fp contract(off)
+  const int nv = D >> 2;
+  const float invD = 1.0f / (float)D;
+  float c1 = 0.f, c2 = 0.f;
+#pragma unroll
+  for (int i = 0; i < LN_MAXV; ++i) {
+    const int c = lane + i * 64;
+    if (c < nv) {
+      const f32x4 gm = reinterpret_cast<const f32x4*>(gsm)[c];
+#pragma unroll
+      for (int j = 0; j < 4; ++j) {
+        const float d = (float)r.dv[i][j];
+        const float h = (r.xv[i][j] - mu) * rs;
+        const float g = d * gm[j];
+        const float gh = g * h;
+        c1 += g;
+        c2 += gh;
+        dg[i][j] = __builtin_fmaf(d, h, dg[i][j]);
+        db[i][j] += d;
+      }
+    }
+  }
+  c1 = wave_sum(c1) * invD;
+  c2 = wave_sum(c2) * invD;
+  float* dxr = dx + (size_t)row * D;
+#pragma unroll
+  for (int i = 0; i < LN_MAXV; ++i) {
+    const int c = lane + i * 64;
+    if (c < nv) {
+      const f32x4 gm = reinterpret_cast<const f32x4*>(gsm)[c];
+      float o[4];
+#pragma unroll
+      for (int j = 0; j < 4; ++j) {
+        const float h = (r.xv[i][j] - mu) * rs;
+        const float u = __builtin_fmaf(-h, c2, __builtin_fmaf((float)r.dv[i][j], gm[j], -c1));
+        o[j] = has_res ? __builtin_fmaf(rs, u, r.rv[i][j]) : rs * u;
+      }
+      Vec<float, 4>::st_nt(dxr + c * 4, o);
+#pragma unroll
+      for (int j = 0; j < 4; ++j) ds[i][j] += o[j];
+      if (dx_lp) Vec<TLp, 4>::st_nt(dx_lp + (size_t)row * D + c * 4, o);
+    }
+  }
+}
+
+template <int LN_MAXV>
+__device__ __forceinline__ void ln_fold_partials(float* fold, float* __restrict__ out, bool live, int D, int t, int w,
+                                                 int lane, const f32x4 (&dg)[LN_MAXV], const f32x4 (&db)[LN_MAXV],
+                                                 const f32x4 (&ds)[LN_MAXV]) {
+  const int nv = D >> 2;
+  float* mine = fold + (size_t)w * D;
+#pragma unroll
+  for (int ph = 0; ph < 3; ++ph) {
+#pragma unroll
+    for (int i = 0; i < LN_MAXV; ++i) {
+      const int c = lane + i * 64;
+      if (c < nv) reinterpret_cast<f32x4*>(mine)[c] = (ph == 0) ? dg[i] : ((ph == 1) ? db[i] : ds[i]);
+    }
+    __syncthreads();
+    if (live) {
+      for (int j = t; j < D; j += 256)
+        out[ph * D + j] = (fold[j] + fold[D + j]) + (fold[2 * D + j] + fold[3 * D + j]);
+    }
+    __syncthreads();
+  }
+}
+
+template <typename T, bool RES>
+__device__ __forceinline__ void ln_passenger_rows(const LnBwdArgs& a, const T* __restrict__ dy, T* __restrict__ dx_lp, int row0,
+                                                  int stride, const float* gsm, int lane, f32x4 (&dg)[5], f32x4 (&db)[5],
+                                                  f32x4 (&ds)[5]) {
+  constexpr int V = 5;
+  const int M = a.M, D = a.D;
+  LnRow<T, V> ra, rb;
+  int row = row0;
+  ln_row_load_all<T, V, RES>(ra, dy, a.lddy, a.x, a.dres, row, D, lane);
+  float mua = a.mean[row], rsa = a.rstd[row];
+  for (;;) {
+    const int r1 = row + stride, r1c = r1 < M ? r1 : row;
+    ln_row_load_all<T, V, RES>(rb, dy, a.lddy, a.x, a.dres, r1c, D, lane);
+    const float mub = a.mean[r1c], rsb = a.rstd[r1c];
+    ln_row_finish<T, T, V>(ra, RES, mua, rsa, gsm, a.dx, dx_lp, row, D, lane, dg, db, ds);
+    if (r1 >= M) break;
+    const int r2 = r1 + stride, r2c = r2 < M ? r2 : r1;
+    ln_row_load_all<T, V, RES>(ra, dy, a.lddy, a.x, a.dres, r2c, D, lane);
+    mua = a.mean[r2c];
+    rsa = a.rstd[r2c];
+    ln_row_finish<T, T, V>(rb, RES, mub, rsb, gsm, a.dx, dx_lp, r1, D, lane, dg, db, ds);
+    if (r2 >= M) break;
+    row = r2;
+  }
+}
+
+template <typename T>
+__device__ __forceinline__ void ln_bwd_passenger(const LnBwdArgs& a, int pi, int P, char* smem) {
+  constexpr int V = 5;
+  const int lane = threadIdx.x & 63;
+  const int w8 = __builtin_amdgcn_readfirstlane(threadIdx.x >> 6);
+  const int half = w8 >> 2, w = w8 & 3, t = threadIdx.x & 255;
+  const int D = a.D, M = a.M;
+  float* fold = reinterpret_cast<float*>(smem) + (size_t)half * 5 * D;
+  float* gsm = fold + (size_t)4 * D;
+  for (int j = t; j < D; j += 256) gsm[j] = a.gamma[j];
+  __syncthreads();
+  const T* dy = reinterpret_cast<const T*>(a.dy);
+  T* dx_lp = reinterpret_cast<T*>(a.dx_lp);
+  const bool has_res = a.dres != nullptr;
+  const int stride = a.nblk * 4;
+  const int npairs = (a.vb_split + 1) >> 1;
+  for (int q = pi; q < npairs; q += P) {
+    const int vb = 2 * q + half;
+    const bool live = vb < a.vb_split;
+    f32x4 dg[V], db[V], ds[V];
+#pragma unroll
+    for (int i = 0; i < V; ++i) {
+      const f32x4 z = {0.f, 0.f, 0.f, 0.f};
+      dg[i] = z;
+      db[i] = z;
+      ds[i] = z;
+    }
+    const int row = vb * 4 + w;
+    if (live && row < M) {
+      if (has_res)
+        ln_passenger_rows<T, true>(a, dy, dx_lp, row, stride, gsm, lane, dg, db, ds);
+      else
+        ln_passenger_rows<T, false>(a, dy, dx_lp, row, stride, gsm, lane, dg, db, ds);
+    }
+    if (a.partial) ln_fold_partials<V>(fold, a.partial + (size_t)vb * 3 * D, live, D, t, w, lane, dg, db, ds);
+  }
+}
+
+}
diff --git a/deepfake-detection-using-clip-based-siglip-2-vision-transformers_amd/lib.py b/deepfake-detection-using-clip-based-siglip-2-vision-transformers_amd/lib.py
--- a/deepfake-detection-using-clip-based-siglip-2-vision-transformers_amd/lib.py
+++ b/deepfake-detection-using-clip-based-siglip-2-vision-transformers_amd/lib.py
@@ -141,6 +141,8 @@
     _sig(lib, "sgl_op_gemm_nt_mx", i, [_fp, _fp, _fp, _fp, i, i, i, i, _fp, i, _fp, _fp, _fp, i, i, i, i, i, i, _fp])
     _sig(lib, "sgl_op_gemm_tn", i, [i, _fp, i, _fp, i, i, i, i, i, _fp, i, i, _fp])
     _sig(lib, "sgl_op_gemm_tn_ws", i, [i, _fp, i, _fp, i, i, i, i, i, _fp, i, i, _fp, sz, _fp])
+    _sig(lib, "sgl_op_gemm_tn_ws_ln_bwd", i, [i, _fp, i, _fp, i, i, i, i, i, _fp, i, i, _fp, sz,
+                                              _fp, _fp, _fp, _fp, _fp, _fp, _fp, _fp, _fp, sz, i, i, i, _fp])
     _sig(lib, "sgl_op_attn_fwd", i, [i, _fp, _fp, _fp, _fp, _fp, i, i, i, i, i, i, _fp])
     _sig(lib, "sgl_op_attn_bwd", i, [i, _fp, _fp, _fp, _fp, _fp, _fp, _fp, _fp, i, i, i, i, i, i, _fp])
     _sig(lib, "sgl_op_colsum", i, [i, _fp, i, i, i, _fp, i, _fp, sz, _fp])
diff --git a/include/siglip_hip.h b/include/siglip_hip.h
--- a/include/siglip_hip.h
+++ b/include/siglip_hip.h
@@ -145,6 +145,11 @@
                    float* out, int ldo, int accumulate, sgl_stream stream);
 int sgl_op_gemm_tn_ws(int dtype, const void* A, int lda, const void* B, int ldb, int Mred, int N1, int N2, int splits,
                       float* out, int ldo, int accumulate, float* scratch, size_t scratch_bytes, sgl_stream stream);
+int sgl_op_gemm_tn_ws_ln_bwd(int dtype, const void* A, int lda, const void* B, int ldb, int Mred, int N1, int N2,
+                             int splits, float* out, int ldo, int accumulate, float* scratch, size_t scratch_bytes,
+                             const void* dy, const float* x, const float* mean, const float* rstd, const float* gamma,
+                             const float* dres, float* dx, void* dx_lp, float* partial, size_t partial_bytes, int M, int D,
+                             int vb_split, sgl_stream stream);
 int sgl_op_attn_fwd(int dtype, const void* q, const void* k, const void* v, void* out, float* lse, int B, int H, int N,
                     int head_dim, int head_dim_pad, int ld_qkv, sgl_stream stream);
 int sgl_op_attn_bwd(int dtype, const void* q, const void* k, const void* v, const void* out, const void* dout,
```

After: 438.9 images/sec (median of 2 runs). Within noise of the previous version (+0.0%).
